# WangSimiao2000/MinecraftSkin_Raytracer

Hardware: NVIDIA B200
Metric: Mrays/s (higher is better)
Workload: dtype f32

## Files before the change

### include/mcskin_cuda.h

```cpp
#ifndef MCSKIN_CUDA_H
#define MCSKIN_CUDA_H

#include <stdint.h>

#ifdef __cplusplus
extern "C" {
#endif

#define MCSKIN_ABI_VERSION 2

enum {
    MC_OK = 0,
    MC_ERR_INVALID = -1,
    MC_ERR_NO_DEVICE = -2,
    MC_ERR_CUDA = -3,
    MC_ERR_LIMIT = -4
};

typedef struct McFaceTex {
    int32_t texel_offset;
    int32_t width;
    int32_t height;
} McFaceTex;

// ... 53 lines not shown
    x ^= x >> 16; x *= 0x7feb352du; x ^= x >> 15; x *= 0x846ca68bu; x ^= x >> 16;
    return x;
}
static inline uint32_t mc_rng_counter_key(uint32_t seed) { return mc_rng_lowbias32(seed ^ 0x9e3779b9u); }
static inline uint32_t mc_rng_counter_word(uint32_t seed, uint32_t k) { return mc_rng_lowbias32(mc_rng_counter_key(seed) + k); }
uint32_t mcskin_counter_word(uint32_t seed, uint32_t k);

void mcskin_config_defaults(McConfig* cfg);

typedef struct McTile {
    int32_t x, y, width, height;
} McTile;

int32_t mcskin_generate_tiles(int32_t image_width, int32_t image_height, int32_t tile_size,
                              McTile* out, int32_t capacity);

typedef void (*McProgressFn)(int32_t done, int32_t total, void* user);

typedef struct McRenderStats {
    int32_t n_tiles;
    int32_t n_active_pixels;
    int64_t n_samples;
    float ms_device;
    int32_t n_kernel_launches;
    float ms_primary;
    float ms_shade;
} McRenderStats;

int32_t mcskin_cuda_device_count(void);
const char* mcskin_cuda_last_error(void);
int32_t mcskin_cuda_abi_version(void);
void mcskin_cuda_abi_sizes(int32_t* out8);

int32_t mcskin_cuda_render(const McScene* scene, const McConfig* cfg, int32_t device,
                           float* out_rgba_f32, uint8_t* out_rgba_u8,
                           McProgressFn progress, void* user, McRenderStats* stats);

typedef struct McAovTargets {
    float* coverage;
    float* depth;
    int32_t* tri_id;
} McAovTargets;

int32_t mcskin_cuda_render_aovs(const McScene* scene, const McConfig* cfg, int32_t device,
                                float* out_rgba_f32, uint8_t* out_rgba_u8, const McAovTargets* aov,
                                McRenderStats* stats);

int32_t mcskin_cuda_render_tile(const McScene* scene, const McConfig* cfg, int32_t device,
                                const McTile* tile, float* image_rgba_f32, uint8_t* image_rgba_u8);

int32_t mcskin_cuda_render_multi(const McScene* scene, const McConfig* cfg, int32_t n_devices,
                                 float* out_rgba_f32, uint8_t* out_rgba_u8, McRenderStats* stats);

typedef struct McContext McContext;

int32_t mcskin_cuda_context_create(int32_t device, McContext** out);
void mcskin_cuda_context_destroy(McContext* ctx);
int32_t mcskin_cuda_context_set_scene(McContext* ctx, const McScene* scene, const McConfig* cfg);
int32_t mcskin_cuda_context_render_bands(McContext* ctx, int32_t first_tile_row, int32_t tile_row_stride,
                                         void* d_out_f32, void* d_out_u8, void* stream);
int32_t mcskin_cuda_band_rows(const McConfig* cfg, int32_t first_tile_row, int32_t tile_row_stride);
int32_t mcskin_cuda_context_render_rows_into_frame(McContext* ctx, int32_t first_tile_row, int32_t stride,
                                                    void* d_frame_f32, void* d_frame_u8, void* stream);
int32_t mcskin_cuda_context_render_tiles_into_frame(McContext* ctx, const int32_t* tiles, int32_t n_tiles,
                                                     void* d_frame_f32, void* d_frame_u8, void* stream);
int32_t mcskin_cuda_context_render_scene_tiles(McContext* ctx, const McScene* scene, const McConfig* cfg,
                                                const int32_t* tiles, int32_t n_tiles, float* host_frame_f32,
                                                uint8_t* host_frame_u8, float* ms_device);
int32_t mcskin_partition_tiles(const McScene* scene, const McConfig* cfg, int32_t n_parts, int32_t part,
                               int32_t root_part, int32_t* out_tiles, int32_t capacity);
int32_t mcskin_host_copy_rows(void* dst, const void* src, uint64_t dst_pitch, uint64_t src_pitch, uint64_t row_bytes,
                              uint64_t rows, int32_t pieces);
int32_t mcskin_cuda_host_register(void* host_ptr, uint64_t bytes, void** d_ptr);
int32_t mcskin_cuda_host_unregister(void* host_ptr);
int32_t mcskin_cuda_device_alloc(int32_t device, uint64_t bytes, void** out_ptr);
int32_t mcskin_cuda_device_free(int32_t device, void* ptr);
int32_t mcskin_cuda_ipc_export(int32_t device, void* ptr, uint8_t handle_out[64]);
int32_t mcskin_cuda_ipc_open(int32_t device, const uint8_t handle[64], void** out_ptr);
int32_t mcskin_cuda_ipc_close(int32_t device, void* ptr);
int32_t mcskin_cuda_peer_signal(int32_t device, void* d_flag, uint32_t value, void* stream);
int32_t mcskin_cuda_enable_peer_access(int32_t device, int32_t peer);
int32_t mcskin_cuda_peer_wait(int32_t device, const void* d_flags, int32_t n, uint32_t value, void* d_timeout, void* stream);
int32_t mcskin_cuda_context_debug_block_times(McContext* ctx, uint64_t* out, int32_t capacity);
int32_t mcskin_cuda_context_set_aov_targets(McContext* ctx, const McAovTargets* d_targets);
int32_t mcskin_cuda_context_sync(McContext* ctx, McRenderStats* stats);
int32_t mcskin_cuda_context_set_option(McContext* ctx, const char* name, int64_t value);

int32_t mcskin_cuda_context_render_batch(McContext* ctx, const McScene* scenes, int32_t n_scenes,
                                         const McConfig* cfg, void* d_out_f32, void* d_out_u8, void* stream);
int32_t mcskin_skin_layout(const uint8_t* atlas_rgba8, int32_t atlas_w, int32_t atlas_h, const float* pose12, McBox* boxes_out,
                           int32_t* faces_out, int32_t* n_faces_out, uint8_t* box_opaque_out, McScene* scene_out);
int32_t mcskin_cuda_context_render_skin_batch(McContext* ctx, const uint8_t* atlases_rgba8, int32_t atlas_w, int32_t atlas_h,
                                              int32_t n_skins, const float* poses12, int32_t pose_stride, const McConfig* cfg,
                                              void* d_out_f32, void* d_out_u8, void* stream);
int32_t mcskin_cuda_render_batch_multi(const McScene* scenes, int32_t n_scenes, const McConfig* cfg, int32_t n_devices,
                                       float* out_rgba_f32, uint8_t* out_rgba_u8);

typedef struct McRay {
    float origin[3];
    float dir[3];
} McRay;

typedef struct McHit {
    int32_t hit;
    float t;
    float point[3];
    float normal[3];
    float tex_color[4];
    int32_t is_outer_layer;
    int32_t box;
    int32_t face;
} McHit;

int32_t mcskin_cuda_intersect(const McScene* scene, int32_t device, int32_t box,
                              const McRay* rays, int32_t n, McHit* out);
int32_t mcskin_cuda_trace(const McScene* scene, const McConfig* cfg, int32_t device, int32_t use_config,
                          int32_t depth, const McRay* rays, int32_t n, float* out_rgba);
int32_t mcskin_cuda_shade(const McScene* scene, const McConfig* cfg, int32_t device,
                          const McHit* hits, const float* view_dirs , const float* shadow_factors ,
                          int32_t n, float* out_rgba);
int32_t mcskin_cuda_in_shadow(const McScene* scene, int32_t device, const float* points, const float* normals,
                              const float* light_positions, int32_t n, int32_t* out);
int32_t mcskin_cuda_soft_shadow(const McScene* scene, int32_t device, const float* points, const float* normals,
                                const uint32_t* seeds, int32_t samples, int32_t n, float* out);
int32_t mcskin_cuda_ambient_occlusion(const McScene* scene, int32_t device, const float* points,
                                      const float* normals, const uint32_t* seeds, int32_t samples,
                                      float radius, int32_t n, float* out);
int32_t mcskin_cuda_generate_rays(const McScene* scene, int32_t device, float aspect, const float* uv,
                                  int32_t n, McRay* out);
int32_t mcskin_cuda_background(const McScene* scene, const McConfig* cfg, int32_t device, int32_t use_config,
                               const float* uv, int32_t n, float* out_rgba);
int32_t mcskin_cuda_sincos(int32_t device, const float* angles, int32_t n, float* out_sin, float* out_cos);
void mcskin_sincos_model(const float* angles, int32_t n, float* out_sin, float* out_cos);
int32_t mcskin_cuda_powf(int32_t device, const float* x, const float* y, int32_t n, float* out);
void mcskin_powf_model(const float* x, const float* y, int32_t n, float* out);
int32_t mcskin_primary_launch_order(const McScene* scene, const McConfig* cfg, int32_t first_tile_row, int32_t stride,
                                    int32_t parts_heavy, int32_t parts_light, int32_t* out_tile, int32_t* out_part,
                                    int32_t* out_parts, int32_t capacity);
int32_t mcskin_cuda_fp32_issue_peak(int32_t device, double* out_lane_ops_per_second);
int32_t mcskin_cuda_aov(const McScene* scene, const McConfig* cfg, int32_t device, int32_t* out_tri_id);

#define MCSKIN_MAX_SKIN_BOXES 12
#define MCSKIN_MAX_SKIN_TEXELS 4096
int32_t mcskin_build_skin_scene(const uint8_t* atlas_rgba8, int32_t atlas_w, int32_t atlas_h,
                                const float* pose12, McBox* boxes_out, float* texels_out,
                                McScene* scene_out);

#ifdef __cplusplus
}
#endif
#endif
```

### minecraftskin_raytracer_b200/csrc/batch.cu

```cuda
#include <cstring>
#include <thread>
#include "capi_internal.hpp"

namespace {

struct SkinBatchSrc {
    const uint8_t* atlases;
    int w, h;
    const float* poses;
    int poseStride;
};

int render_batch_grouped(McContext* ctx, const McScene* scenes, const SkinBatchSrc* skins, int nScenes, const McConfig* cfg,
                         float4* outF32, uchar4* outU8, cudaStream_t stream, bool* handled) {
    *handled = false;
    if (!ctx->batchMode || ctx->shadeMode != 0 || ctx->forceAllActive || nScenes < 2) return MC_OK;
    if (cfg->width <= 0 || cfg->height <= 0 || cfg->tile_size <= 0 || cfg->width > 65535 || cfg->height > 65535) return MC_OK;
    const int spp = std::max(1, cfg->samples_per_pixel);
    if (spp > kBlockThreads) return MC_OK;
    const size_t pixels = static_cast<size_t>(cfg->width) * cfg->height;
    std::string err;
    for (int i = 0; i < 2; ++i)
        if (!ctx->evStage[i]) CU_TRY(cudaEventCreateWithFlags(&ctx->evStage[i], cudaEventDisableTiming));

// ... 123 lines not shown
                    groupOf[i] = static_cast<int>(g);
            }
            if (groupOf[i] < 0) {
                groupOf[i] = static_cast<int>(groups.size());
                groups.emplace_back();
            }
            groups[groupOf[i]].push_back(i);
        }
        unsigned char* stage = static_cast<unsigned char*>(ctx->batchStage[stageSlot].p);
        BatchSlice* stageSlices = reinterpret_cast<BatchSlice*>(stage + sliceOffset);
        AovView* stageAovs = reinterpret_cast<AovView*>(stage + aovOffset);
        int sliceAt = 0;
        std::vector<int> groupFirstSlice(groups.size(), 0);
        for (size_t g = 0; g < groups.size(); ++g) {
            groupFirstSlice[g] = sliceAt;
            for (int i : groups[g]) {
                const PreparedFrame& pf = ctx->batchPreps[i];
                unsigned char* dst = stage + static_cast<size_t>(i) * sceneStride;
                const size_t blobBytes = (pf.blob.size() + 255) & ~size_t(255);
                std::memcpy(dst, pf.blob.data(), pf.blob.size());
                if (!skins) std::memcpy(dst + blobBytes, pf.texels.data(), pf.texels.size() * sizeof(float4h));
                BatchSlice sl{};
                sl.fp.blob = devScenes + static_cast<size_t>(i) * sceneStride;
                sl.fp.texels = reinterpret_cast<const float4*>(devScenes + static_cast<size_t>(i) * sceneStride + blobBytes);
                sl.fp.blob_bytes = static_cast<unsigned int>(pf.blob.size());
                sl.band.first_tile_row = 0;
                sl.band.tile_row_stride = 1;
                sl.band.n_tile_rows = pf.frame.tiles_y;
                sl.band.out_first_row = 0;
                sl.band.out_row_stride = 1;
                sl.band.out_f32 = outF32 ? outF32 + static_cast<size_t>(c0 + i) * pixels : nullptr;
                sl.band.out_u8 = outU8 ? outU8 + static_cast<size_t>(c0 + i) * pixels : nullptr;
                AovView av{};
                av.planes = aov_at(ctx->aov, static_cast<size_t>(c0 + i) * pixels);
                sl.list.count = static_cast<unsigned int*>(ctx->batchCounts.p) + i;
                sl.list.slot_pixel = static_cast<uint2*>(ctx->batchSlots.p) + static_cast<size_t>(i) * slotCap;
                sl.list.records = reinterpret_cast<float*>(static_cast<unsigned char*>(ctx->batchRecords.p) + static_cast<size_t>(i) * recordBytes);
                sl.list.capacity = static_cast<unsigned int>(slotCap);
                sl.list.count_host = nullptr;
                const int gridX = std::max(2, (ctx->smCount * ctx->shadeBlocksPerSm + nC - 1) / nC);
                if (!wavefront_carve(pf.frame, static_cast<unsigned char*>(ctx->batchWave.p) + static_cast<size_t>(i) * waveBytes,
                                     waveBytes, static_cast<unsigned int>(paths), static_cast<unsigned int>(entries), gridX, &sl.wave, aov ? &av : nullptr))
                    return MC_OK;
                sl.wave.seedMemo = batchSeedMemo;
                stageAovs[sliceAt] = av;
                stageSlices[sliceAt++] = sl;
            }
        }
        const size_t usedScenes = static_cast<size_t>(nC) * sceneStride;
        if (skins) {
            const size_t blobMax = (SceneBlobLayout(kSkinMaxBoxes).bytes() + 255) & ~size_t(255);
            CU_TRY(cudaMemcpy2DAsync(devScenes, sceneStride, stage, sceneStride, blobMax, nC, cudaMemcpyHostToDevice, stream));
            CU_TRY(cudaMemcpyAsync(devSkin, skinStage, static_cast<size_t>(nC) * skinRecord, cudaMemcpyHostToDevice, stream));
            launch_slice_skins(devSkin, skinRecord, atlasBytes + kSkinMaxFaces * sizeof(SkinFaceSource), nC, stream);
        } else {
            CU_TRY(cudaMemcpyAsync(devScenes, stage, usedScenes, cudaMemcpyHostToDevice, stream));
        }
        CU_TRY(cudaMemcpyAsync(devScenes + sliceOffset, stage + sliceOffset, static_cast<size_t>(nC) * sizeof(BatchSlice),
                               cudaMemcpyHostToDevice, stream));
        if (aov)
            CU_TRY(cudaMemcpyAsync(devScenes + aovOffset, stage + aovOffset, static_cast<size_t>(nC) * sizeof(AovView),
                                   cudaMemcpyHostToDevice, stream));
        CU_TRY(cudaEventRecord(ctx->evStage[stageSlot], stream));
        stageSlot ^= 1;
        const BatchSlice* devSlices = reinterpret_cast<const BatchSlice*>(devScenes + sliceOffset);
        const AovView* devAovs = aov ? reinterpret_cast<const AovView*>(devScenes + aovOffset) : nullptr;
        for (size_t g = 0; g < groups.size(); ++g) {
            const int nS = static_cast<int>(groups[g].size());
            const BatchSlice* gs = devSlices + groupFirstSlice[g];
            const AovView* gAov = devAovs ? devAovs + groupFirstSlice[g] : nullptr;
            const BatchSlice& first = stageSlices[groupFirstSlice[g]];
            const DevFrame& f = ctx->batchPreps[groups[g][0]].frame;
            launch_batch_reset(gs, nS, stream);
            if (gAov) launch_aov_defaults(f, first.band, McAovTargets{}, gAov, nS, stream);
            const KernelBuild& build = kernels_for(f);
            const int primaryTarget = ctx->smCount * ctx->primaryBlocksPerSm;
            const int statesPerTile = primary_states_per_tile(f, f.tiles_x * f.tiles_y, nS, primaryTarget, 0);
            const bool seedNow = !seeded || statesPerTile != seededStatesPerTile;
            uint32_t* const states = static_cast<uint32_t*>(ctx->tileStates.p);
            if (!build.launch_primary_batch(f, first.band, states, seedNow, gs, nS, first.fp.blob_bytes, primaryTarget, stream)) return MC_OK;
            seeded = true;
            seededStatesPerTile = statesPerTile;
            int launches = 0;
            build.launch_wavefront(f, first.fp, first.band, first.list, first.wave, nullptr, stream, &launches, gs, nS, nullptr, gAov);
        }
        CU_TRY(cudaGetLastError());
    }
    *handled = true;
    return MC_OK;
}

}

extern "C" {

int32_t mcskin_cuda_context_render_batch(McContext* ctx, const McScene* scenes, int32_t nScenes, const McConfig* cfg,
                                         void* dOutF32, void* dOutU8, void* stream) {
    if (!ctx || !scenes || !cfg || nScenes < 0) return fail(MC_ERR_INVALID, "render_batch: bad argument");
    if (nScenes == 0) return MC_OK;
    CU_TRY(cudaSetDevice(ctx->device));
    const size_t pixels = static_cast<size_t>(std::max(cfg->width, 0)) * std::max(cfg->height, 0);
    cudaStream_t caller = stream ? static_cast<cudaStream_t>(stream) : ctx->stream;
    {
        bool handled = false;
        const int rc = render_batch_grouped(ctx, scenes, nullptr, nScenes, cfg, static_cast<float4*>(dOutF32), static_cast<uchar4*>(dOutU8),
                                            caller, &handled);
        if (rc != MC_OK) return rc;
        if (handled) {
            ctx->stats = McRenderStats{};
            ctx->statsPending = false;
            return MC_OK;
        }
    }
    const int nLanes = std::min<int>(ctx->batchLanes, nScenes);
    {
        const int rc = ensure_lanes(ctx, nLanes);
        if (rc != MC_OK) return rc;
    }
    CU_TRY(cudaEventRecord(ctx->evCopy, caller));
    for (int k = 0; k < nLanes; ++k) {
        McContext* lane = ctx->lanes[k];
        inherit_options(lane, ctx);
        lane->shadeBlocksPerSm = std::max(1, ctx->shadeBlocksPerSm / 2);
        CU_TRY(cudaStreamWaitEvent(lane->stream, ctx->evCopy, 0));
    }
    for (int i = 0; i < nScenes; ++i) {
        McContext* lane = ctx->lanes[i % nLanes];
        int rc = mcskin_cuda_context_set_scene(lane, &scenes[i], cfg);
        if (rc != MC_OK) return rc;
        lane->aov = aov_at(ctx->aov, static_cast<size_t>(i) * pixels);
        rc = render_bands(lane, 0, 1, dOutF32 ? static_cast<float4*>(dOutF32) + i * pixels : nullptr,
                          dOutU8 ? static_cast<uchar4*>(dOutU8) + i * pixels : nullptr, lane->stream);
        if (rc != MC_OK) return rc;
    }
    for (int k = 0; k < nLanes; ++k) {
        CU_TRY(cudaEventRecord(ctx->lanes[k]->evCopy, ctx->lanes[k]->stream));
        CU_TRY(cudaStreamWaitEvent(caller, ctx->lanes[k]->evCopy, 0));
    }
    ctx->stats = McRenderStats{};
    ctx->statsPending = false;
    return MC_OK;
}

int32_t mcskin_cuda_context_render_skin_batch(McContext* ctx, const uint8_t* atlases, int32_t atlasW, int32_t atlasH,
                                              int32_t nSkins, const float* poses12, int32_t poseStride, const McConfig* cfg,
                                              void* dOutF32, void* dOutU8, void* stream) {
    if (!ctx || !atlases || !cfg || nSkins < 0 || poseStride < 0) return fail(MC_ERR_INVALID, "render_skin_batch: bad argument");
    if (!((atlasW == 64 && atlasH == 64) || (atlasW == 64 && atlasH == 32)))
        return fail(MC_ERR_INVALID, "Invalid skin dimensions: " + std::to_string(atlasW) + "x" + std::to_string(atlasH) +
                                        " (expected 64x64 or 64x32)");
    if (nSkins == 0) return MC_OK;
    CU_TRY(cudaSetDevice(ctx->device));
    cudaStream_t caller = stream ? static_cast<cudaStream_t>(stream) : ctx->stream;
    const SkinBatchSrc src{atlases, atlasW, atlasH, poses12, poses12 ? poseStride : 0};
    bool handled = false;
    int rc = render_batch_grouped(ctx, nullptr, &src, nSkins, cfg, static_cast<float4*>(dOutF32), static_cast<uchar4*>(dOutU8),
                                  caller, &handled);
    if (rc != MC_OK) return rc;
    if (handled) {
        ctx->stats = McRenderStats{};
        ctx->statsPending = false;
        return MC_OK;
    }
    const size_t atlasBytes = static_cast<size_t>(atlasW) * atlasH * 4;
    const int chunk = 64;
    std::vector<McBox> boxes(static_cast<size_t>(chunk) * kSkinMaxBoxes);
    std::vector<float> texels(static_cast<size_t>(chunk) * (kSkinMaxTexels + 16) * 4);
// ... 99 lines not shown
```

### minecraftskin_raytracer_b200/csrc/capi.cu

```cuda
#include <cstring>
#include "capi_internal.hpp"

namespace {

struct Staged {
    McContext* ctx;
    std::vector<void*> temps;
    ~Staged() {
        for (void* p : temps) cudaFree(p);
    }
    int up(const void* host, size_t bytes, void** dev) {
        *dev = nullptr;
        if (bytes == 0) return MC_OK;
        CU_TRY(cudaMalloc(dev, bytes));
        temps.push_back(*dev);
        if (host) CU_TRY(cudaMemcpyAsync(*dev, host, bytes, cudaMemcpyHostToDevice, ctx->stream));
        return MC_OK;
    }
    int down(void* host, const void* dev, size_t bytes) {
        if (bytes == 0) return MC_OK;
        CU_TRY(cudaMemcpyAsync(host, dev, bytes, cudaMemcpyDeviceToHost, ctx->stream));
        CU_TRY(cudaStreamSynchronize(ctx->stream));
        CU_TRY(cudaGetLastError());
        return MC_OK;
// ... 251 lines not shown
    if (rc != MC_OK) return rc;
    Staged st{ctx, {}};
    void *dU, *dO;
    if ((rc = st.up(uv, sizeof(float) * 2 * n, &dU)) != MC_OK) return rc;
    if ((rc = st.up(nullptr, sizeof(float4) * n, &dO)) != MC_OK) return rc;
    launch_background(ctx->prep.frame, static_cast<float*>(dU), n, static_cast<float4*>(dO), ctx->stream);
    return st.down(out, dO, sizeof(float4) * n);
}

int32_t mcskin_primary_launch_order(const McScene* scene, const McConfig* cfg, int32_t first, int32_t stride,
                                    int32_t partsHeavy, int32_t partsLight, int32_t* outTile, int32_t* outPart,
                                    int32_t* outParts, int32_t capacity) {
    if (!scene || !cfg || capacity < 0) return fail(MC_ERR_INVALID, "primary_launch_order: bad argument");
    PreparedFrame pf;
    std::string err;
    const int rc = prepare_frame(scene, cfg, 1, 0.0f, pf, err);
    if (rc != MC_OK) return fail(rc, err);
    return primary_launch_order(pf.frame, first, stride, partsHeavy, partsLight, outTile, outPart, outParts, capacity);
}

int32_t mcskin_cuda_fp32_issue_peak(int32_t device, double* out) {
    if (!out) return fail(MC_ERR_INVALID, "fp32_issue_peak: out is null");
    *out = 0.0;
    std::lock_guard<std::mutex> lock(g_ctxMutex);
    McContext* ctx = nullptr;
    int rc = shared_context(device, &ctx);
    if (rc != MC_OK) return rc;
    float* sink = nullptr;
    CU_TRY(cudaMalloc(&sink, sizeof(float)));
    const int blocks = ctx->smCount * 8, iters = 1 << 15;
    cudaEvent_t e0, e1;
    CU_TRY(cudaEventCreate(&e0));
    CU_TRY(cudaEventCreate(&e1));
    double best = 0.0;
    for (int rep = 0; rep < 6; ++rep) {
        CU_TRY(cudaEventRecord(e0, ctx->stream));
        launch_fp32_peak(blocks, iters, sink, ctx->stream);
        CU_TRY(cudaEventRecord(e1, ctx->stream));
        CU_TRY(cudaEventSynchronize(e1));
        float ms = 0.0f;
        CU_TRY(cudaEventElapsedTime(&ms, e0, e1));
        const double ops = static_cast<double>(blocks) * kBlockThreads * iters * 16.0;
        if (ms > 0.0f) best = std::max(best, ops / (ms * 1e-3));
    }
    cudaEventDestroy(e0);
    cudaEventDestroy(e1);
    cudaFree(sink);
    CU_TRY(cudaGetLastError());
    *out = best;
    return MC_OK;
}

int32_t mcskin_cuda_powf(int32_t device, const float* x, const float* y, int32_t n, float* out) {
    if (n < 0 || (n > 0 && (!x || !y || !out))) return fail(MC_ERR_INVALID, "powf: bad argument");
    std::lock_guard<std::mutex> lock(g_ctxMutex);
    McContext* ctx = nullptr;
    int rc = shared_context(device, &ctx);
    if (rc != MC_OK) return rc;
    Staged st{ctx, {}};
    void *dX, *dY, *dO;
    if ((rc = st.up(x, sizeof(float) * n, &dX)) != MC_OK) return rc;
    if ((rc = st.up(y, sizeof(float) * n, &dY)) != MC_OK) return rc;
    if ((rc = st.up(nullptr, sizeof(float) * n, &dO)) != MC_OK) return rc;
    launch_powf(static_cast<float*>(dX), static_cast<float*>(dY), n, static_cast<float*>(dO), ctx->stream);
    return st.down(out, dO, sizeof(float) * n);
}

int32_t mcskin_cuda_sincos(int32_t device, const float* angles, int32_t n, float* outSin, float* outCos) {
    if (n < 0 || (n > 0 && (!angles || !outSin || !outCos))) return fail(MC_ERR_INVALID, "sincos: bad argument");
    std::lock_guard<std::mutex> lock(g_ctxMutex);
    McContext* ctx = nullptr;
    int rc = shared_context(device, &ctx);
    if (rc != MC_OK) return rc;
    Staged st{ctx, {}};
    void *dA, *dS, *dC;
    if ((rc = st.up(angles, sizeof(float) * n, &dA)) != MC_OK) return rc;
    if ((rc = st.up(nullptr, sizeof(float) * n, &dS)) != MC_OK) return rc;
    if ((rc = st.up(nullptr, sizeof(float) * n, &dC)) != MC_OK) return rc;
    launch_sincos(static_cast<float*>(dA), n, static_cast<float*>(dS), static_cast<float*>(dC), ctx->stream);
    if ((rc = st.down(outSin, dS, sizeof(float) * n)) != MC_OK) return rc;
    return st.down(outCos, dC, sizeof(float) * n);
}

int32_t mcskin_cuda_aov(const McScene* scene, const McConfig* cfg, int32_t device, int32_t* outTriId) {
    if (!cfg || !outTriId) return fail(MC_ERR_INVALID, "aov: bad argument");
    if (cfg->width <= 0 || cfg->height <= 0) return MC_OK;
    std::lock_guard<std::mutex> lock(g_ctxMutex);
    McContext* ctx = nullptr;
    int rc = query_setup(scene, cfg, device, 1, 0.0f, &ctx);
    if (rc != MC_OK) return rc;
    Staged st{ctx, {}};
    void* dO;
    const size_t bytes = sizeof(int32_t) * static_cast<size_t>(cfg->width) * cfg->height;
    if ((rc = st.up(nullptr, bytes, &dO)) != MC_OK) return rc;
    launch_aov(ctx->prep.frame, frame_pointers(ctx), static_cast<int*>(dO), ctx->stream);
    return st.down(outTriId, dO, bytes);
}

void mcskin_cuda_abi_sizes(int32_t* out8) {
    if (!out8) return;
    out8[0] = sizeof(McFaceTex);
    out8[1] = sizeof(McBox);
    out8[2] = sizeof(McScene);
    out8[3] = sizeof(McConfig);
    out8[4] = sizeof(McTile);
    out8[5] = sizeof(McRenderStats);
    out8[6] = sizeof(McRay);
    out8[7] = sizeof(McHit);
}

}
```

### minecraftskin_raytracer_b200/csrc/capi_internal.hpp

```cpp
#pragma once
#include <algorithm>
#include <atomic>
#include <cstdlib>
#include <cstring>
#include <memory>
#include <mutex>
#include <string>
#include <thread>
#include <vector>

#include <cuda_runtime.h>

#include "host_copy.hpp"
#include "host_prep.hpp"
#include "kernels.cuh"
#include "wavefront.cuh"
#include "mcskin_cuda.h"

using namespace mcskin;

inline int fail(int code, const std::string& msg) {
    set_last_error(msg);
    return code;
}
inline int cuda_fail(cudaError_t e, const char* what) {
    return fail(e == cudaErrorNoDevice || e == cudaErrorInsufficientDriver ? MC_ERR_NO_DEVICE : MC_ERR_CUDA,
                std::string(what) + ": " + cudaGetErrorString(e));
}
#define CU_TRY(expr)                                     \
    do {                                                 \
        cudaError_t e__ = (expr);                        \
        if (e__ != cudaSuccess) return cuda_fail(e__, #expr); \
    } while (0)

extern std::atomic<unsigned long long> g_allocEpoch;

template <bool kPinned>
struct GrowBuf {
    void* p = nullptr;
    size_t cap = 0;
    GrowBuf() = default;
    GrowBuf(const GrowBuf&) = delete;
    GrowBuf& operator=(const GrowBuf&) = delete;
    ~GrowBuf() { release(); }
    cudaError_t reserve(size_t bytes) {
        if (bytes <= cap) return cudaSuccess;
        if (!kPinned) g_allocEpoch.fetch_add(1);
        release();
        cudaError_t e = kPinned ? cudaMallocHost(&p, bytes) : cudaMalloc(&p, bytes);
        if (e == cudaSuccess) cap = bytes;
        return e;
    }
    void release() {
        if (p) (kPinned ? cudaFreeHost : cudaFree)(p);
        p = nullptr;
        cap = 0;
    }
};
using DevBuf = GrowBuf<false>;
using PinnedBuf = GrowBuf<true>;

struct PixelRect {
    int x, y, w, h;
};

struct McOptions {
    int forceAllActive = 0;
    long long recordBudgetBytes = 1ll << 31;
    int shadeBlocksPerSm = 8;
    int softBlocksPerSm = 4;
    int heavyTilesPerSm = 16;
    int primaryBlocksPerSm = 8;
    int waveQueuePct = 0;
    int frameLanes = 2;
    int cacheTileSeeds = 1;
    int overlapCopyOut = 2;
    int useGraphs = 1;
    int shadeMode = 0;
    long long waveBudgetBytes = 12ll << 30;
    int shadowSeedMemo = 1;
    int stagedCopyOut = 1;
    int batchLanes = 4;
    int batchGroup = 128;
    int batchMode = 1;
    int debugPrimaryTiming = 0;
};
constexpr size_t kOptionCount = 19;

struct McContext : McOptions {
    int device = 0;
    int smCount = 148;
    cudaStream_t stream = nullptr;
    cudaEvent_t ev0 = nullptr, ev1 = nullptr, evCopy = nullptr;
    std::vector<cudaEvent_t> passEvents;
    bool hasScene = false;
    PreparedFrame prep;
    DevBuf boxes, texels;
    DevBuf slotPixel, records;
    DevBuf imgF32, imgU8;
    DevBuf tileStates;
    DevBuf blockTimes;
    int blockTimesCount = 0;
    DevBuf tileMap;
    std::vector<int32_t> tileMapHost, tileMapOrdered;
    std::vector<PixelRect> tileMapLightRects;
    unsigned long long tileMapVersion = 0;
    int tileMapHeavy = 0;
    DevFrame tileMapFrame{};
    DevBuf wave;
    PinnedBuf pinned;
    bool isChild = false;
    struct TileSeedKey {
        int width = 0, tile_size = 0, first = 0, stride = 0, rows = 0;
        const void* buf = nullptr;
        cudaStream_t stream = nullptr;
        const void* map = nullptr;
        unsigned long long mapVersion = 0;
        int wordsPerPixel = 0, statesPerTile = 0;
        bool operator==(const TileSeedKey& o) const {
            return width == o.width && tile_size == o.tile_size && first == o.first && stride == o.stride &&
                   rows == o.rows && buf == o.buf && stream == o.stream && map == o.map && mapVersion == o.mapVersion &&
                   wordsPerPixel == o.wordsPerPixel && statesPerTile == o.statesPerTile;
        }
    } tileSeedKey;
    bool tileSeedValid = false;
    int splitLastRender = 0;
    cudaEvent_t evPrimaryDone = nullptr;
    cudaStream_t copyStream = nullptr;
    cudaEvent_t evFrameDone = nullptr;
    cudaEvent_t evUpload = nullptr;
    unsigned long long seedGen = 0;
    bool capturing = false;
    struct GraphKey {
        DevFrame frame;
        const void *blob, *texels, *outF32, *outU8;
        unsigned int blobBytes;
        int first, stride, lanes;
        const void* tileMap;
        unsigned long long mapVersion;
        int nTiles, nHeavy;
        const void *hotF32, *hotU8;
        const void *aovCoverage, *aovDepth, *aovTriId;
        long long optionBits[kOptionCount];
        unsigned long long allocEpoch;
        bool operator==(const GraphKey& o) const { return std::memcmp(this, &o, sizeof(GraphKey)) == 0; }
    };
    GraphKey graphKey{}, graphCandidate{};
    bool hasCandidate = false;
    cudaGraph_t graph = nullptr;
    cudaGraphExec_t graphExec = nullptr;
    std::vector<unsigned long long> graphSeedGens;
    std::vector<int> graphLaneLaunches, graphLaneChunks, graphLaneTiles;
    bool graphLastRender = false;
    McRenderStats stats{};
    bool statsPending = false;
    bool uploadQueued = false;
    DevBuf countLog;
    PinnedBuf countHost;
    unsigned int* countAlias = nullptr;
    PinnedBuf sceneStage;
    DevBuf seedMemo;
    PinnedBuf stageF32, stageU8;
    std::vector<cudaEvent_t> pieceEvents;
    std::vector<std::pair<const void*, bool>> farCache;
    int chunksLastRender = 0;
    DevBuf batchScenes, batchSlots, batchRecords, batchWave, batchCounts;
    DevBuf batchSkinSrc;
    PinnedBuf batchSkinStage[2];
    std::vector<McBox> batchSkinBoxes;
    PinnedBuf batchStage[2];
    cudaEvent_t evStage[2] = {nullptr, nullptr};
    std::vector<PreparedFrame> batchPreps;
    std::vector<McContext*> lanes;
    McAovTargets aov{};
    DevBuf aovPlanes;
};

struct KernelBuild {
    decltype(&mcskin::launch_primary) launch_primary;
    decltype(&mcskin::launch_shade) launch_shade;
    decltype(&mcskin::launch_wavefront) launch_wavefront;
    decltype(&mcskin::launch_primary_batch) launch_primary_batch;
};
constexpr KernelBuild kGeneralBuild{&launch_primary, &launch_shade, &launch_wavefront, &launch_primary_batch};
constexpr KernelBuild kPlainBuild{&plain::launch_primary, &plain::launch_shade, &plain::launch_wavefront, &plain::launch_primary_batch};
// ... 50 lines not shown
```

### minecraftskin_raytracer_b200/csrc/context.cu

```cuda
#include <cstdlib>
#include "capi_internal.hpp"

std::atomic<unsigned long long> g_allocEpoch{1};

namespace {

using IntOption = int McOptions::*;
using LongOption = long long McOptions::*;
struct OptionSpec {
    const char* name;
    const char* env;
    IntOption i;
    LongOption ll;
    long long lo, hi;
    bool inherited, launch;
};
constexpr OptionSpec kOptions[] = {
    {"force_all_active", "MCSKIN_FORCE_ALL_ACTIVE", &McOptions::forceAllActive, nullptr, 0, 1, true, true},
    {"record_budget_bytes", nullptr, nullptr, &McOptions::recordBudgetBytes, 1, INT64_MAX, true, true},
    {"shade_blocks_per_sm", "MCSKIN_SHADE_BLOCKS", &McOptions::shadeBlocksPerSm, nullptr, 1, INT32_MAX, true, true},
    {"soft_blocks_per_sm", "MCSKIN_SOFT_BLOCKS", &McOptions::softBlocksPerSm, nullptr, 1, INT32_MAX, true, true},
    {"primary_blocks_per_sm", "MCSKIN_PRIMARY_BLOCKS", &McOptions::primaryBlocksPerSm, nullptr, 0, INT32_MAX, true, true},
    {"heavy_tiles_per_sm", "MCSKIN_HEAVY_TILES", &McOptions::heavyTilesPerSm, nullptr, 0, INT32_MAX, true, true},
    {"batch_lanes", nullptr, &McOptions::batchLanes, nullptr, 1, 16, false, false},
    {"batch_group", "MCSKIN_BATCH_GROUP", &McOptions::batchGroup, nullptr, 1, 4096, false, false},
    {"batch_mode", "MCSKIN_BATCH_MODE", &McOptions::batchMode, nullptr, 0, 1, false, false},
    {"shade_mode", "MCSKIN_SHADE_MODE", &McOptions::shadeMode, nullptr, 0, 2, true, true},
    {"debug_primary_timing", nullptr, &McOptions::debugPrimaryTiming, nullptr, 0, 1, false, true},
    {"wave_queue_pct", "MCSKIN_WAVE_QUEUE_PCT", &McOptions::waveQueuePct, nullptr, 0, 100000, true, true},
    {"frame_lanes", "MCSKIN_FRAME_LANES", &McOptions::frameLanes, nullptr, 1, 8, false, true},
    {"cache_tile_seeds", "MCSKIN_CACHE_TILE_SEEDS", &McOptions::cacheTileSeeds, nullptr, 0, 1, true, true},
    {"use_graphs", "MCSKIN_GRAPHS", &McOptions::useGraphs, nullptr, 0, 1, false, false},
    {"overlap_copy_out", "MCSKIN_OVERLAP_COPY", &McOptions::overlapCopyOut, nullptr, 0, 2, false, false},
    {"wave_budget_bytes", nullptr, nullptr, &McOptions::waveBudgetBytes, 1 << 20, INT64_MAX, true, true},
    {"staged_copy_out", "MCSKIN_STAGED_COPY", &McOptions::stagedCopyOut, nullptr, 0, 1, false, false},
    {"shadow_seed_memo", "MCSKIN_SEED_MEMO", &McOptions::shadowSeedMemo, nullptr, 0, 1, false, true},
};
static_assert(sizeof(kOptions) / sizeof(kOptions[0]) == kOptionCount, "kOptionCount counts the rows of kOptions");

long long option_value(const McOptions& o, const OptionSpec& spec) { return spec.i ? o.*spec.i : o.*spec.ll; }

void set_option_value(McOptions& o, const OptionSpec& spec, long long value) {
    const long long v = spec.lo == 0 && spec.hi == 1 ? value != 0 : std::min(spec.hi, std::max(spec.lo, value));
    if (spec.i) o.*spec.i = static_cast<int>(v);
    else o.*spec.ll = v;
}

}

void inherit_options(McContext* lane, const McContext* ctx) {
    for (const OptionSpec& spec : kOptions)
        if (spec.inherited) set_option_value(*lane, spec, option_value(*ctx, spec));
    lane->aov = ctx->aov;
    lane->useGraphs = 0;
}

void launch_option_bits(const McContext* ctx, long long* bits) {
    for (size_t i = 0; i < kOptionCount; ++i) bits[i] = kOptions[i].launch ? option_value(*ctx, kOptions[i]) : 0;
}

int upload_scene(McContext* ctx) {
    const PreparedFrame& pf = ctx->prep;
    if (pf.blob.size() > kMaxSceneSmemBytes)
        return fail(MC_ERR_LIMIT, "scene has too many meshes for the shared-memory staging area (" +
                                      std::to_string(pf.boxes.size()) + " boxes)");
    CU_TRY(ctx->boxes.reserve(pf.blob.size()));
    CU_TRY(ctx->texels.reserve(pf.texels.size() * sizeof(float4h)));
    const size_t blobBytes = (pf.blob.size() + 255) & ~size_t(255), texelBytes = pf.texels.size() * sizeof(float4h);
    if (ctx->uploadQueued) CU_TRY(cudaEventSynchronize(ctx->evUpload));
    CU_TRY(ctx->sceneStage.reserve(blobBytes + texelBytes + 256));
    unsigned char* stage = static_cast<unsigned char*>(ctx->sceneStage.p);
    std::memcpy(stage, pf.blob.data(), pf.blob.size());
    if (texelBytes) std::memcpy(stage + blobBytes, pf.texels.data(), texelBytes);
    CU_TRY(cudaMemcpyAsync(ctx->boxes.p, stage, pf.blob.size(), cudaMemcpyHostToDevice, ctx->stream));
    if (texelBytes) CU_TRY(cudaMemcpyAsync(ctx->texels.p, stage + blobBytes, texelBytes, cudaMemcpyHostToDevice, ctx->stream));
    CU_TRY(cudaEventRecord(ctx->evUpload, ctx->stream));
    ctx->uploadQueued = true;
    return MC_OK;
}

int finish_stats(McContext* ctx, McRenderStats* out) {
    if (ctx->statsPending) {
        float ms = 0.0f;
        if (!(ctx->isChild && ctx->graphLastRender)) {
            CU_TRY(cudaEventSynchronize(ctx->ev1));
            CU_TRY(cudaEventElapsedTime(&ms, ctx->ev0, ctx->ev1));
        }
        ctx->stats.ms_device = ms;
        ctx->stats.ms_primary = ctx->stats.ms_shade = 0.0f;
        for (int c = 0; c < ctx->chunksLastRender && !ctx->graphLastRender; ++c) {
            float a = 0.0f, b = 0.0f;
            CU_TRY(cudaEventElapsedTime(&a, ctx->passEvents[3 * c], ctx->passEvents[3 * c + 1]));
            CU_TRY(cudaEventElapsedTime(&b, ctx->passEvents[3 * c + 1], ctx->passEvents[3 * c + 2]));
            ctx->stats.ms_primary += a;
            ctx->stats.ms_shade += b;
        }
        long long active = 0;
        const unsigned int* counts = static_cast<const unsigned int*>(ctx->countHost.p);
        for (int c = 0; c < ctx->chunksLastRender && counts; ++c) active += counts[c];
        ctx->stats.n_active_pixels = static_cast<int32_t>(std::min<long long>(active, 0x7fffffff));
        ctx->statsPending = false;
        for (int k = 0; k < ctx->splitLastRender; ++k) {
            McRenderStats s{};
            const int rc = finish_stats(ctx->lanes[k], &s);
            if (rc != MC_OK) return rc;
            ctx->stats.n_tiles += s.n_tiles;
            ctx->stats.n_active_pixels += s.n_active_pixels;
            ctx->stats.n_kernel_launches += s.n_kernel_launches;
            ctx->stats.ms_primary = std::max(ctx->stats.ms_primary, s.ms_primary);
            ctx->stats.ms_shade = std::max(ctx->stats.ms_shade, s.ms_shade);
        }
    }
    if (out) *out = ctx->stats;
    return MC_OK;
}

std::mutex g_ctxMutex;
std::vector<McContext*> g_ctxByDevice;

// ... 116 lines not shown
```

### minecraftskin_raytracer_b200/csrc/dev_intersect.cuh

```cuda
#pragma once
#include "dev_math.cuh"
#include "dev_types.cuh"

namespace mcskin {

struct Ray {
    V3 o, d;
};

struct Hit {
    float t;
    V3 p;
    int box;
    int face;
    int texel;
    bool flip;
};

struct SceneView {
    const float4* __restrict__ lo;
    const float4* __restrict__ hi;
    const int4* __restrict__ rect;
    const DevBox* __restrict__ boxes;
    const float4* __restrict__ texels;
// ... 73 lines not shown
}
__device__ __forceinline__ int face_texel(const DevBox& bx, V3 p, int axis, bool negSide, int face) {
    const float pa = (axis == 0) ? p.z : p.x;
    const float la0 = (axis == 0) ? bx.lo[2] : bx.lo[0];
    const float sa = (axis == 0) ? bx.size[2] : bx.size[0];
    const float ra = (axis == 0) ? bx.inv_size_z : bx.inv_size_x;
    const float pb = (axis == 1) ? p.z : p.y;
    const float lb0 = (axis == 1) ? bx.lo[2] : bx.lo[1];
    const float sb = (axis == 1) ? bx.size[2] : bx.size[1];
    const float rb = (axis == 1) ? bx.inv_size_z : bx.inv_size_y;
    float la, lb;
    if (bx.flags & kBoxRecip) {
        la = div_exact(pa - la0, sa, ra);
        lb = div_exact(pb - lb0, sb, rb);
    } else {
        la = (pa - la0) / sa;
        lb = (pb - lb0) / sb;
    }
    float u, v;
    if (axis == 2) {
        u = negSide ? 1.0f - la : la;
        v = 1.0f - lb;
    } else if (axis == 0) {
        u = !negSide ? 1.0f - la : la;
        v = 1.0f - lb;
    } else {
        u = la;
        v = !negSide ? lb : 1.0f - lb;
    }
    u = clamp01(u);
    v = clamp01(v);
    const int2 ft = bx.face[face];
    const int w = ft.y & 0xffff;
    const int h = ft.y >> 16;
    int x = __float2int_rz(u * static_cast<float>(w));
    int y = __float2int_rz(v * static_cast<float>(h));
    x = max(0, min(x, w - 1));
    y = max(0, min(y, h - 1));
    return ft.x + y * w + x;
}

struct RayPre {
    V3 inv;
    bool parallel;
};
__device__ __forceinline__ RayPre ray_pre(const Ray& r) {
    RayPre p;
    p.parallel = fabsf(r.d.x) < 1e-8f || fabsf(r.d.y) < 1e-8f || fabsf(r.d.z) < 1e-8f;
    p.inv = mk3(1.0f / r.d.x, 1.0f / r.d.y, 1.0f / r.d.z);
    return p;
}

struct BoxHit {
    float t;
    V3 p;
    int face, texel;
    bool flip;
};

__device__ __forceinline__ float rcp_fast(float x) {
    float r;
    asm("rcp.approx.ftz.f32 %0, %1;" : "=f"(r) : "f"(x));
    return r;
}

__device__ __forceinline__ V3 to_box_space(const DevBox& bx, V3 p, bool isPoint) {
    const V3 pivot = isPoint ? ld3(bx.pivot) : mk3(0.0f, 0.0f, 0.0f);
    V3 q = p - pivot;
    if (bx.flags & kBoxRotZ) {
        const float nx = q.x * bx.inv_cz - q.y * bx.inv_sz, ny = q.x * bx.inv_sz + q.y * bx.inv_cz;
        q.x = nx;
        q.y = ny;
    }
    if (bx.flags & kBoxRotX) {
        const float ny = q.y * bx.inv_cx - q.z * bx.inv_sx, nz = q.y * bx.inv_sx + q.z * bx.inv_cx;
        q.y = ny;
        q.z = nz;
    }
    return q + pivot;
}

enum : int { kPosedUnknown = 0, kPosedMissed = 1, kPosedHitBeforeLimit = 2 };
template <bool LIMITED>
__device__ __forceinline__ int posed_box_verdict(const DevBox& bx, const Ray& ray, float limit, bool opaque) {
    constexpr float kPad = 1e-2f;
    const V3 o = to_box_space(bx, ray.o, true);
    const V3 d = to_box_space(bx, ray.d, false);
    float tmin = -FLT_MAX, tmax = FLT_MAX;
    float smin = -FLT_MAX, smax = FLT_MAX;
    bool sure = LIMITED && opaque;
    const float os[3] = {o.x, o.y, o.z}, ds[3] = {d.x, d.y, d.z};
#pragma unroll
    for (int k = 0; k < 3; ++k) {
        const float lo = bx.lo[k] - kPad, hi = bx.hi[k] + kPad;
        if (fabsf(ds[k]) < 1e-6f) {
            if (os[k] < lo || os[k] > hi) return kPosedMissed;
            sure = sure && os[k] > lo + 2.0f * kPad && os[k] < hi - 2.0f * kPad;
            continue;
        }
        const float inv = rcp_fast(ds[k]);
        const float a = (lo - os[k]) * inv, b = (hi - os[k]) * inv;
        tmin = fmaxf(tmin, fminf(a, b));
        tmax = fminf(tmax, fmaxf(a, b));
        if (LIMITED) {
            const float shift = 2.0f * kPad * fabsf(inv);
            smin = fmaxf(smin, fminf(a, b) + shift);
            smax = fminf(smax, fmaxf(a, b) - shift);
        }
    }
    const float slack = 1e-4f * (fabsf(tmin) + fabsf(tmax)) + 1e-3f;
    if (fmaxf(tmin, 0.0f) > tmax + slack) return kPosedMissed;
    if (LIMITED && !(tmin - slack < limit)) return kPosedMissed;
    if (LIMITED && sure && fmaxf(smin, 0.0f) + slack < smax && tmax + slack < limit) return kPosedHitBeforeLimit;
    return kPosedUnknown;
}
template <bool LIMITED>
__device__ __forceinline__ bool posed_box_missed(const DevBox& bx, const Ray& ray, float limit) {
    return posed_box_verdict<LIMITED>(bx, ray, limit, false) == kPosedMissed;
}

template <bool LIMITED>
__device__ __forceinline__ uint32_t drop_missed_posed(const SceneView& sc, const Ray& ray, uint32_t mask, float limit) {
    if (!kPosedScenes) return mask;
    uint32_t todo = mask & sc.rotated_mask;
    while (todo) {
        const int i = __ffs(todo) - 1;
        todo &= todo - 1u;
        if (posed_box_missed<LIMITED>(sc.boxes[i], ray, limit)) mask &= ~(1u << i);
    }
    return mask;
}


__device__ __forceinline__ bool box_test(const SceneView& sc, const DevBox& bx, V3 o, V3 d, V3 inv, BoxHit& out) {
    Slab s;
    s.tmin = -FLT_MAX;
    s.tmax = FLT_MAX;
    s.axis = 0;
    s.exitAxis = 0;
    s.neg = false;
    s.exitNeg = false;
    if (!slab_axis<0>(s, o.x, d.x, inv.x, bx.lo[0], bx.hi[0])) return false;
    if (!slab_axis<1>(s, o.y, d.y, inv.y, bx.lo[1], bx.hi[1])) return false;
    if (!slab_axis<2>(s, o.z, d.z, inv.z, bx.lo[2], bx.hi[2])) return false;
    if (s.tmin > s.tmax || s.tmax < 0.0f) return false;

    float tHit = s.tmin;
    int axis = s.axis;
    bool negSide = s.neg;
    if (tHit < 0.0f) {
        tHit = s.tmax;
        axis = s.exitAxis;
        negSide = s.exitNeg;
    }
    bool flip = false;
    for (;;) {
        const V3 p = o + d * tHit;
        const int face = face_index(axis, negSide);
        const int texel = face_texel(bx, p, axis, negSide, face);
        const float alpha = __ldg(&sc.texels[texel].w);
        const bool opaque = flip ? (alpha > 0.0f) : !(alpha == 0.0f);
        if (opaque) {
            out.t = tHit;
            out.p = p;
            out.face = face;
            out.texel = texel;
            out.flip = flip;
            return true;
// ... 177 lines not shown
    best.p = mk3(0.0f, 0.0f, 0.0f);
    BoxHit h;
    const RayPre pre = ray_pre(ray);
    if (b >= 0 && b < sc.n_boxes && mesh_test(sc, b, ray, pre, h)) {
        best.t = h.t;
        best.p = h.p;
        best.box = b;
        best.face = h.face;
        best.texel = h.texel;
        best.flip = h.flip;
    }
    return best;
}

__device__ __forceinline__ bool any_hit(const SceneView& sc, const Ray& ray) {
    const RayPre pre = ray_pre(ray);
    for (int base = 0; base < sc.n_boxes; base += 32) {
        uint32_t mask = candidate_mask<false>(sc, ray, pre, base, FLT_MAX);
        while (mask) {
            const int b = base + __ffs(mask) - 1;
            mask &= mask - 1u;
            BoxHit h;
            if (mesh_test(sc, b, ray, pre, h)) return true;
        }
    }
    return false;
}

__device__ __forceinline__ bool occluded_among(const SceneView& sc, const Ray& ray, const float dist, const uint32_t allow) {
    const RayPre pre = ray_pre(ray);
    for (int base = 0; base < sc.n_boxes; base += 32) {
        uint32_t mask;
        if (base == 0 && allow != 0xffffffffu) {
            uint32_t todo = allow & sc.usable_mask;
            if (sc.n_boxes < 32) todo &= (1u << sc.n_boxes) - 1u;
            mask = todo;
            if (!pre.parallel) {
                uint32_t rejected = 0u;
                while (todo) {
                    const int i = __ffs(todo) - 1;
                    todo &= todo - 1u;
                    const float4 L = sc.lo[i];
                    const float4 H = sc.hi[i];
                    const float ax = (L.x - ray.o.x) * pre.inv.x, bx = (H.x - ray.o.x) * pre.inv.x;
                    const float ay = (L.y - ray.o.y) * pre.inv.y, by = (H.y - ray.o.y) * pre.inv.y;
                    const float az = (L.z - ray.o.z) * pre.inv.z, bz = (H.z - ray.o.z) * pre.inv.z;
                    const float tmin = fmaxf(fmaxf(fminf(ax, bx), fminf(ay, by)), fminf(az, bz));
                    const float tmax = fminf(fminf(fmaxf(ax, bx), fmaxf(ay, by)), fmaxf(az, bz));
                    if (fmaxf(tmin, 0.0f) > tmax || !(tmin < dist)) {
                        rejected |= 1u << i;
                    } else if ((sc.opaque_mask >> i) & 1u) {
                        if ((tmin < 0.0f ? tmax : tmin) < dist) return true;
                        rejected |= 1u << i;
                    }
                }
                mask &= ~rejected | sc.posed_mask;
                if (kPosedScenes) {
                    uint32_t posedTodo = mask & sc.rotated_mask;
                    while (posedTodo) {
                        const int i = __ffs(posedTodo) - 1;
                        posedTodo &= posedTodo - 1u;
                        const int verdict = posed_box_verdict<true>(sc.boxes[i], ray, dist, (sc.opaque_posed_mask >> i) & 1u);
                        if (verdict == kPosedHitBeforeLimit) return true;
                        if (verdict == kPosedMissed) mask &= ~(1u << i);
                    }
                }
            }
        } else {
            mask = candidate_mask<true>(sc, ray, pre, base, dist);
        }
        while (mask) {
            const int b = base + __ffs(mask) - 1;
            mask &= mask - 1u;
            BoxHit h;
            if (mesh_test(sc, b, ray, pre, h) && h.t < dist) return true;
        }
    }
    return false;
}
__device__ __forceinline__ bool occluded(const SceneView& sc, const Ray& ray, float dist) {
    return occluded_among(sc, ray, dist, 0xffffffffu);
}

__device__ __forceinline__ bool bundle_clip(V3 a, V3 d, V3 inv, V3 lo, V3 hi, float grow, float* sEnd) {
    const float ax0 = (lo.x - grow - a.x) * inv.x, ax1 = (hi.x + grow - a.x) * inv.x;
    const float ay0 = (lo.y - grow - a.y) * inv.y, ay1 = (hi.y + grow - a.y) * inv.y;
    const float az0 = (lo.z - grow - a.z) * inv.z, az1 = (hi.z + grow - a.z) * inv.z;
    const bool px = fabsf(d.x) < 1e-6f, py = fabsf(d.y) < 1e-6f, pz = fabsf(d.z) < 1e-6f;
    const bool outX = px && (a.x < lo.x - grow || a.x > hi.x + grow);
    const bool outY = py && (a.y < lo.y - grow || a.y > hi.y + grow);
    const bool outZ = pz && (a.z < lo.z - grow || a.z > hi.z + grow);
    float s0 = 0.0f, s1 = 1.0f;
    if (!px) { s0 = fmaxf(s0, fminf(ax0, ax1)); s1 = fminf(s1, fmaxf(ax0, ax1)); }
    if (!py) { s0 = fmaxf(s0, fminf(ay0, ay1)); s1 = fminf(s1, fmaxf(ay0, ay1)); }
    if (!pz) { s0 = fmaxf(s0, fminf(az0, az1)); s1 = fminf(s1, fmaxf(az0, az1)); }
    *sEnd = s1;
    return !(outX || outY || outZ) && s0 <= s1 + 1e-3f;
}

__device__ __forceinline__ bool bundle_reaches(V3 from, V3 d, V3 lo, V3 hi, float radius, float pad) {
    const float growFull = radius * 1.01f + 0.01f + pad;
    const V3 inv = mk3(rcp_fast(d.x), rcp_fast(d.y), rcp_fast(d.z));
    if (fabsf(d.x) < 1e-6f || fabsf(d.y) < 1e-6f || fabsf(d.z) < 1e-6f) {
        float sEnd;
        if (!bundle_clip(from, d, inv, lo, hi, growFull, &sEnd)) return false;
        const float reach = fminf(fmaxf(sEnd + 1e-3f, 0.0f), 1.0f);
        float unused;
        return bundle_clip(from, d, inv, lo, hi, reach * radius * 1.01f + 0.01f + pad, &unused);
    }
    if ((from.x > hi.x + pad && d.x > growFull) || (from.x < lo.x - pad && d.x < -growFull) ||
        (from.y > hi.y + pad && d.y > growFull) || (from.y < lo.y - pad && d.y < -growFull) ||
        (from.z > hi.z + pad && d.z > growFull) || (from.z < lo.z - pad && d.z < -growFull))
        return false;
    const V3 ainv = mk3(fabsf(inv.x), fabsf(inv.y), fabsf(inv.z));
    const V3 g1 = ainv * growFull;
    const float ax = (lo.x - from.x) * inv.x, bx = (hi.x - from.x) * inv.x;
    const float ay = (lo.y - from.y) * inv.y, by = (hi.y - from.y) * inv.y;
    const float az = (lo.z - from.z) * inv.z, bz = (hi.z - from.z) * inv.z;
    const float nx = fminf(ax, bx), fx = fmaxf(ax, bx);
    const float ny = fminf(ay, by), fy = fmaxf(ay, by);
    const float nz = fminf(az, bz), fz = fmaxf(az, bz);
    const float s0 = fmaxf(fmaxf(nx - g1.x, ny - g1.y), fmaxf(nz - g1.z, 0.0f));
    const float s1 = fminf(fminf(fx + g1.x, fy + g1.y), fminf(fz + g1.z, 1.0f));
    if (!(s0 <= s1 + 1e-3f)) return false;
    const float reach = fminf(fmaxf(s1 + 1e-3f, 0.0f), 1.0f);
    const V3 g2 = ainv * (reach * radius * 1.01f + 0.01f + pad);
    const float t0 = fmaxf(fmaxf(nx - g2.x, ny - g2.y), fmaxf(nz - g2.z, 0.0f));
    const float t1 = fminf(fminf(fx + g2.x, fy + g2.y), fminf(fz + g2.z, 1.0f));
    return t0 <= t1 + 1e-3f;
}

__device__ __forceinline__ bool posed_bundle_reaches(const DevBox& pb, V3 from, V3 d, float radius) {
    return bundle_reaches(to_box_space(pb, from, true), to_box_space(pb, d, false), ld3(pb.lo), ld3(pb.hi), radius, 1e-4f);
}

__device__ __forceinline__ uint32_t drop_unreached_posed(const SceneView& sc, V3 from, V3 d, float radius, uint32_t mask) {
    if (!kPosedScenes) return mask;
    uint32_t todo = mask & sc.rotated_mask;
    while (todo) {
        const int i = __ffs(todo) - 1;
        todo &= todo - 1u;
        if (!posed_bundle_reaches(sc.boxes[i], from, d, radius)) mask &= ~(1u << i);
    }
    return mask;
}


__device__ __forceinline__ uint32_t bundle_box_mask(const SceneView& sc, V3 from, V3 to, float radius) {
    const int n = min(32, sc.n_boxes);
    const V3 d = to - from;
    const V3 inv = mk3(rcp_fast(d.x), rcp_fast(d.y), rcp_fast(d.z));
    const float growFull = radius * 1.01f + 0.01f;
    uint32_t mask = 0u;
    if (fabsf(d.x) < 1e-6f || fabsf(d.y) < 1e-6f || fabsf(d.z) < 1e-6f) {
        for (int i = 0; i < n; ++i) {
            const float4 L = sc.lo[i];
            const float4 H = sc.hi[i];
            if (__float_as_uint(L.w) & kBoxEmpty) continue;
            const V3 lo = mk3(L.x, L.y, L.z), hi = mk3(H.x, H.y, H.z);
            float sEnd;
            if (!bundle_clip(from, d, inv, lo, hi, growFull, &sEnd)) continue;
            const float reach = fminf(fmaxf(sEnd + 1e-3f, 0.0f), 1.0f);
            float unused;
            if (!bundle_clip(from, d, inv, lo, hi, reach * radius * 1.01f + 0.01f, &unused)) continue;
            mask |= 1u << i;
        }
// ... 85 lines not shown
```

### minecraftskin_raytracer_b200/csrc/dev_shade.cuh

```cuda
#pragma once
#include "dev_intersect.cuh"
#include "dev_mt19937.cuh"

namespace mcskin {

constexpr float kShadowEpsilon = 1e-3f;
constexpr float kReflectEpsilon = 1e-3f;
constexpr float kReflectivity = 0.1f;
constexpr int kMaxStackDepth = 64;
#define MCSKIN_TWO_PI_F (2.0f * 3.14159274101257324219f)

__device__ __forceinline__ Ray camera_ray(const DevFrame& fr, float u, float v) {
    const float su = (2.0f * u - 1.0f) * fr.half_w;
    const float sv = (2.0f * (1.0f - v) - 1.0f) * fr.half_h;
    const V3 fwd = ld3(fr.cam_fwd), right = ld3(fr.cam_right), up = ld3(fr.cam_up);
    Ray r;
    r.o = ld3(fr.cam_pos);
    r.d = normalize3((fwd + right * su) + up * sv);
    return r;
}

__device__ __forceinline__ void sincos_ref(float a, float* sn, float* cs) {
    const uint32_t top12 = (__float_as_uint(a) >> 20) & 0x7ffu;
    if (top12 > 0x42eu) {
// ... 171 lines not shown
}

static __device__ __noinline__ float soft_shadow_large(const SceneView& sc, const DevFrame& fr, V3 point, V3 normal,
                                                int samples, uint32_t seed) {
    if (samples <= 1 || fr.light_radius < 1e-4f) return in_shadow(sc, point, normal, ld3(fr.light_pos)) ? 0.0f : 1.0f;
    LocalEngine rng;
    rng.seed(seed);
    return static_cast<float>(soft_shadow_count(sc, fr, point, normal, samples, rng, 0xffffffffu)) / static_cast<float>(samples);
}
__device__ __forceinline__ float soft_shadow(const SceneView& sc, const DevFrame& fr, V3 point, V3 normal,
                                             int samples, uint32_t seed) {
    if (samples <= 1 || fr.light_radius < 1e-4f || 2 * samples > kFreshStreamMaxDraws)
        return soft_shadow_large(sc, fr, point, normal, samples, seed);
    const uint32_t allow = bundle_box_mask(sc, point + normal * kShadowEpsilon, ld3(fr.light_pos), fr.light_radius);
    if (allow == 0u && sc.n_boxes <= 32) return 1.0f;
    FreshStream rng;
    rng.seed(seed);
    return static_cast<float>(soft_shadow_count(sc, fr, point, normal, samples, rng, allow)) / static_cast<float>(samples);
}

template <class Engine>
__device__ __forceinline__ int ao_count(const SceneView& sc, V3 point, V3 normal, int samples, float radius,
                                        Engine& rng) {
    const V3 N = normalize3(normal);
    V3 T, B;
    frame_about(N, &T, &B);
    Ray r;
    r.o = point + N * 1e-3f;
    int occludedCount = 0;
    for (int i = 0; i < samples; ++i) {
        const float r1 = rng.next();
        const float r2 = rng.next();
        const float sinT = sqrtf(1.0f - r1);
        const float cosT = sqrtf(r1);
        const float phi = MCSKIN_TWO_PI_F * r2;
        float sn, cs;
        sincos_ref(phi, &sn, &cs);
        const V3 l = mk3(sinT * cs, cosT, sinT * sn);
        r.d = normalize3((T * l.x + N * l.y) + B * l.z);
        if (occluded(sc, r, radius)) ++occludedCount;
    }
    return occludedCount;
}
static __device__ __noinline__ float ambient_occlusion_large(const SceneView& sc, V3 point, V3 normal, int samples,
                                                      float radius, uint32_t seed) {
    LocalEngine rng;
    rng.seed(seed);
    return 1.0f - static_cast<float>(ao_count(sc, point, normal, samples, radius, rng)) / static_cast<float>(samples);
}
static __device__ __noinline__ float ambient_occlusion(const SceneView& sc, V3 point, V3 normal, int samples,
                                                   float radius, uint32_t seed) {
    if (2 * samples > kFreshStreamMaxDraws) return ambient_occlusion_large(sc, point, normal, samples, radius, seed);
    FreshStream rng;
    rng.seed(seed);
    return 1.0f - static_cast<float>(ao_count(sc, point, normal, samples, radius, rng)) / static_cast<float>(samples);
}

__device__ __forceinline__ float4 shade_lit(const DevFrame& fr, V3 P, V3 normal, float4 tex, V3 viewDir, float vis) {
    const V3 lp = ld3(fr.light_pos);
    const V3 L = normalize3(lp - P);
    const V3 N = normalize3(normal);
    const V3 V = normalize3(viewDir);
    const float ndl = fmaxf(0.0f, dot3(N, L));
    const float kdiff = fr.kd * ndl * vis;
    const V3 H = normalize3(L + V);
    const float ndh = fmaxf(0.0f, dot3(N, H));
    const float spec = powf_ref(ndh, fr.shininess);
    const float kspec = fr.ks * spec * vis;
    float4 out;
    out.x = (tex.x * fr.ambient + tex.x * fr.light_color[0] * kdiff) + fr.light_color[0] * kspec;
    out.y = (tex.y * fr.ambient + tex.y * fr.light_color[1] * kdiff) + fr.light_color[1] * kspec;
    out.z = (tex.z * fr.ambient + tex.z * fr.light_color[2] * kdiff) + fr.light_color[2] * kspec;
    out.w = tex.w;
    return clamp4(out);
}

__device__ __forceinline__ float4 shade_hit(const SceneView& sc, const DevFrame& fr, V3 P, V3 normal, float4 tex,
                                            V3 viewDir, float shadowFactor) {
    float vis = shadowFactor;
    if (vis < 0.0f) vis = in_shadow(sc, P, normalize3(normal), ld3(fr.light_pos)) ? 0.0f : 1.0f;
    return shade_lit(fr, P, normal, tex, viewDir, vis);
}

template <class Engine>
__device__ __forceinline__ void soft_shadow_positions(const DevFrame& fr, V3 point, int samples, Engine& rng,
                                                      float* out ) {
    const V3 lp = ld3(fr.light_pos);
    const V3 toPoint = normalize3(point - lp);
    V3 tangent, bitangent;
    frame_about(toPoint, &tangent, &bitangent);
    for (int i = 0; i < samples; ++i) {
        const float angle = MCSKIN_TWO_PI_F * rng.next();
        const float r = fr.light_radius * sqrtf(rng.next());
        float sn, cs;
        sincos_ref(angle, &sn, &cs);
        const V3 offset = tangent * (r * cs) + bitangent * (r * sn);
        const V3 samplePos = lp + offset;
        out[3 * i] = samplePos.x;
        out[3 * i + 1] = samplePos.y;
        out[3 * i + 2] = samplePos.z;
    }
}

__device__ __forceinline__ uint32_t shadow_seed(V3 P, int depth) {
    return seed_cast(P.x * 12345.0f + P.y * 67890.0f + P.z * 11111.0f + static_cast<float>(depth) * 99999.0f);
}
__device__ __forceinline__ uint32_t ao_seed(V3 P) {
    return seed_cast(P.x * 73856093.0f + P.y * 19349663.0f + P.z * 83492791.0f);
}

struct TraceOptions {
    int start_depth;
    bool primary_uv;
    float u, v;
};

__device__ __forceinline__ float4 trace_path(const SceneView& sc, const DevFrame& fr, Ray ray,
                                             const TraceOptions& opt) {
    const bool cfg = fr.use_config != 0;
    const int maxB = fr.max_bounces;
    int depth = opt.start_depth;

    if (depth > maxB) {
        float4 c = cfg ? config_background(fr, 0.5f, 0.5f) : flat_background(fr);
        if (opt.primary_uv && closest_hit(sc, ray).box < 0) c = config_background(fr, opt.u, opt.v);
        return c;
    }

    float stack[kMaxStackDepth][3];
    float alpha0 = 1.0f;
    int top = 0;
    float4 tail;
    for (;;) {
        const Hit hit = closest_hit(sc, ray);
        if (hit.box < 0) {
            if (depth == 0 && opt.primary_uv) tail = config_background(fr, opt.u, opt.v);
            else if (depth == 0 && cfg) tail = config_background(fr, 0.5f, 0.5f);
            else tail = flat_background(fr);
            break;
        }
        const V3 P = hit.p;
        const V3 nrm = hit_normal(sc, hit);
        const float4 tex = hit_texel(sc, hit);
        const V3 viewDir = normalize3(ray.o - P);
        float shadowFactor = -1.0f;
        if (cfg && fr.soft_on) {
            const uint32_t seed = shadow_seed(P, depth);
            shadowFactor = soft_shadow(sc, fr, P, nrm, fr.shadow_samples, seed);
        }
        float4 shaded = shade_hit(sc, fr, P, nrm, tex, viewDir, shadowFactor);
        const float alpha = shaded.w;
        if (cfg && fr.ao_on && depth == 0) {
            const uint32_t seed = ao_seed(P);
            const float ao = ambient_occlusion(sc, P, nrm, fr.ao_samples, fr.ao_radius, seed);
            const float f = 1.0f - fr.ao_intensity * (1.0f - ao);
            shaded.x *= f;
            shaded.y *= f;
            shaded.z *= f;
        }
        if (depth < maxB && top < kMaxStackDepth) {
            stack[top][0] = shaded.x;
            stack[top][1] = shaded.y;
            stack[top][2] = shaded.z;
            if (top == 0) alpha0 = alpha;
            ++top;
            const V3 N = normalize3(nrm);
            const V3 D = normalize3(ray.d);
            V3 R = D - N * (2.0f * dot3(D, N));
            R = normalize3(R);
            ray.o = P + N * kReflectEpsilon;
            ray.d = R;
            ++depth;
            continue;
        }
        shaded.w = alpha;
        tail = clamp4(shaded);
        break;
    }
    const float keep = 1.0f - kReflectivity;
    while (top > 0) {
        --top;
        float4 c;
        c.x = stack[top][0] * keep + tail.x * kReflectivity;
        c.y = stack[top][1] * keep + tail.y * kReflectivity;
// ... 9 lines not shown
```

### minecraftskin_raytracer_b200/csrc/frame.cu

```cuda
#include <cstring>
#include "capi_internal.hpp"

FramePointers frame_pointers(const McContext* ctx) {
    return FramePointers{static_cast<const unsigned char*>(ctx->boxes.p), static_cast<const float4*>(ctx->texels.p),
                         static_cast<unsigned int>(ctx->prep.blob.size())};
}

namespace {

int local_tile_rows(const DevFrame& f, int first, int stride) {
    if (f.tiles_y <= 0 || first < 0 || stride <= 0 || first >= f.tiles_y) return 0;
    return (f.tiles_y - first + stride - 1) / stride;
}

int band_pixel_rows(const DevFrame& f, int first, int stride) {
    const int n = local_tile_rows(f, first, stride);
    if (n == 0) return 0;
    const int lastTileRow = first + (n - 1) * stride;
    const int lastHeight = std::min(f.tile_size, f.height - lastTileRow * f.tile_size);
    return (n - 1) * f.tile_size + lastHeight;
}

}

// ... 81 lines not shown
        paths = std::max<size_t>(paths, static_cast<size_t>(f.spp));
        size_t entries = paths * hitsMax;
        if (ctx.waveQueuePct > 0) entries = std::min(entries, std::max<size_t>(32, paths * static_cast<size_t>(ctx.waveQueuePct) / 100));
        const size_t room = budget > paths * perPath ? (budget - paths * perPath) / perEntry : 0;
        entries = std::min(entries, std::max(room, paths + paths / 4));
        entries = std::min<size_t>(entries, 0xffffff00u);
        p.wavePaths = paths;
        p.waveEntries = entries;
        p.waveBytes = paths * perPath + entries * perEntry + wavefront_fixed_bytes(f) + 16 * 256;
    }
    return p;
}

int render_bands_lane(McContext* ctx, const McContext* scn, const BandSpec& spec, float4* outF32, uchar4* outU8,
                      cudaStream_t stream, int lanesInFlight = 1) {
    const DevFrame& f = scn->prep.frame;
    const long long nTilesAll = band_tiles(f, spec);
    ctx->chunksLastRender = 0;
    ctx->graphLastRender = false;
    ctx->stats = McRenderStats{};
    ctx->stats.n_samples = static_cast<int64_t>(std::max(f.width, 0)) * std::max(f.height, 0) * f.spp;
    ctx->stats.n_tiles = nTilesAll;
    if (nTilesAll == 0) return MC_OK;
    if (f.width > 65535 || f.height > 65535) return fail(MC_ERR_LIMIT, "image larger than 65535 pixels on a side");
    if (static_cast<long long>(f.tile_size) * f.tile_size > (1ll << 30))
        return fail(MC_ERR_LIMIT, "tile_size too large");
    const BandPlan plan = plan_band(f, spec, *ctx, lanesInFlight);
    if (plan.slotCap > 0x7fffffffull) return fail(MC_ERR_LIMIT, "one tile row holds more than 2^31 pixels");
    const int nChunks = plan.nChunks;

    CU_TRY(ctx->countLog.reserve(sizeof(unsigned int) * 2 * nChunks));
    if (ctx->countHost.cap < sizeof(unsigned int) * nChunks) {
        g_allocEpoch.fetch_add(1);
        CU_TRY(ctx->countHost.reserve(sizeof(unsigned int) * std::max(1024, 2 * nChunks)));
        void* alias = nullptr;
        if (cudaHostGetDevicePointer(&alias, ctx->countHost.p, 0) != cudaSuccess) {
            cudaGetLastError();
            alias = nullptr;
        }
        ctx->countAlias = static_cast<unsigned int*>(alias);
    }
    unsigned int* const countAlias = ctx->countAlias;
    CU_TRY(ctx->slotPixel.reserve(plan.slotCap * sizeof(uint2)));
    CU_TRY(ctx->records.reserve(std::max<size_t>(16, plan.slotCap * plan.recordBytesPerSlot)));
    CU_TRY(ctx->tileStates.reserve(
        std::max<size_t>(16, plan.unitsPerChunk * plan.tilesPerUnit * plan.statesPerTile * 624 * sizeof(uint32_t))));
    CU_TRY(cudaMemsetAsync(ctx->countLog.p, 0, sizeof(unsigned int) * 2 * nChunks, stream));

    while (ctx->passEvents.size() < static_cast<size_t>(3 * nChunks)) {
        cudaEvent_t e;
        CU_TRY(cudaEventCreate(&e));
        ctx->passEvents.push_back(e);
    }
    WaveView wave{};
    const bool aov = aov_on(ctx);
    AovView aovView{};
    aovView.planes = ctx->aov;
    if (ctx->shadeMode == 0) {
        CU_TRY(ctx->wave.reserve(plan.waveBytes));
        if (!wavefront_carve(f, ctx->wave.p, ctx->wave.cap, static_cast<unsigned int>(plan.wavePaths),
                             static_cast<unsigned int>(plan.waveEntries), ctx->smCount * ctx->shadeBlocksPerSm, &wave,
                             aov ? &aovView : nullptr))
            return fail(MC_ERR_CUDA, "wavefront buffer carve failed");
        wave.softGrid = ctx->smCount * ctx->softBlocksPerSm;
        wave.seedMemo = static_cast<uint2*>(scn->seedMemo.p);
        if (!scn->shadowSeedMemo) wave.seedMemo = nullptr;
    }
    if (!ctx->capturing) CU_TRY(cudaEventRecord(ctx->ev0, stream));
    const FramePointers fp = frame_pointers(scn);
    const KernelBuild& build = kernels_for(f);
    const bool mapped = spec.map != nullptr, classify = plan.classify;
    int launches = 0;
    McContext::TileSeedKey seedKey;
    seedKey.width = f.width; seedKey.tile_size = f.tile_size; seedKey.first = spec.first; seedKey.stride = spec.stride;
    seedKey.rows = static_cast<int>(plan.nUnits); seedKey.buf = ctx->tileStates.p; seedKey.stream = stream;
    seedKey.map = spec.map; seedKey.mapVersion = spec.mapVersion;
    seedKey.wordsPerPixel = f.spp * f.draws_per_sample; seedKey.statesPerTile = static_cast<int>(plan.statesPerTile) | (f.rng_mode << 16);
    const bool seedsCacheable = ctx->cacheTileSeeds && nChunks == 1 && f.draws_per_sample > 0;
    const bool seedTiles = !(seedsCacheable && ctx->tileSeedValid && seedKey == ctx->tileSeedKey);
    ctx->tileSeedKey = seedKey;
    ctx->tileSeedValid = false;
    if (seedTiles) ++ctx->seedGen;
    const bool farOutput = spec.hotF32 || spec.hotU8 || is_far_memory(ctx, outF32) || is_far_memory(ctx, outU8);
    for (int c = 0; c < nChunks; ++c) {
        const size_t unit0 = static_cast<size_t>(c) * plan.unitsPerChunk;
        const size_t units = std::min<size_t>(plan.unitsPerChunk, plan.nUnits - unit0);
        BandView band{};
        band.out_f32 = outF32;
        band.out_u8 = outU8;
        band.hot_f32 = spec.hotF32;
        band.hot_u8 = spec.hotU8;
        band.far_output = farOutput ? 1 : 0;
        if (ctx->debugPrimaryTiming && nChunks == 1) {
            const size_t tilePixels = static_cast<size_t>(f.tile_size) * f.tile_size;
            const size_t blocks = static_cast<size_t>(nTilesAll) * ((tilePixels + kBlockThreads - 1) / kBlockThreads);
            CU_TRY(ctx->blockTimes.reserve(blocks * 4 * sizeof(unsigned long long)));
            CU_TRY(cudaMemsetAsync(ctx->blockTimes.p, 0, blocks * 4 * sizeof(unsigned long long), stream));
            band.block_times = static_cast<unsigned long long*>(ctx->blockTimes.p);
            ctx->blockTimesCount = static_cast<int>(blocks);
        }
        size_t listing = units;
        if (mapped) {
            band.tile_map = spec.map + unit0;
            band.n_tiles = static_cast<int>(units);
            band.n_heavy = static_cast<int>(unit0 >= static_cast<size_t>(spec.nHeavy) ? 0 : std::min<size_t>(units, spec.nHeavy - unit0));
            if (classify && f.rect_valid) listing = static_cast<size_t>(band.n_heavy);
        } else {
            band.first_tile_row = spec.first + static_cast<int>(unit0) * spec.stride;
            band.tile_row_stride = spec.stride;
            band.n_tile_rows = static_cast<int>(units);
            band.out_first_row = spec.outFirst + static_cast<int>(unit0) * spec.outStride;
            band.out_row_stride = spec.outStride;
        }
        ActiveList list;
        list.count = static_cast<unsigned int*>(ctx->countLog.p) + c;
        list.slot_pixel = static_cast<uint2*>(ctx->slotPixel.p);
        list.records = static_cast<float*>(ctx->records.p);
        list.capacity = static_cast<unsigned int>(std::min(plan.slotCap, std::max<size_t>(1, listing * plan.slotsPerUnit)));
        list.count_host = (ctx->shadeMode == 0 && countAlias) ? countAlias + c : nullptr;
        if (!classify) {
            CU_TRY(cudaMemsetAsync(list.slot_pixel, 0xff, static_cast<size_t>(list.capacity) * sizeof(uint2), stream));
            CU_TRY(cudaMemcpyAsync(list.count, &list.capacity, sizeof(unsigned int), cudaMemcpyHostToDevice, stream));
        }
        if (!ctx->capturing) CU_TRY(cudaEventRecord(ctx->passEvents[3 * c], stream));
        if (aov) {
            launch_aov_defaults(f, band, ctx->aov, nullptr, 1, stream);
            ++launches;
        }
        const bool seeded = build.launch_primary(f, fp, band, list, classify ? 1 : 0, static_cast<uint32_t*>(ctx->tileStates.p),
                                                 seedTiles, plan.primaryTarget, plan.heavyTarget, stream);
        ctx->tileSeedValid = seedsCacheable && seeded;
        if (c == nChunks - 1)
            CU_TRY(cudaEventRecordWithFlags(ctx->evPrimaryDone, stream, ctx->capturing ? cudaEventRecordExternal : cudaEventRecordDefault));
        if (!ctx->capturing) CU_TRY(cudaEventRecord(ctx->passEvents[3 * c + 1], stream));
        unsigned int* groupCounter = static_cast<unsigned int*>(ctx->countLog.p) + nChunks + c;
        const int shadeGrid = ctx->smCount * ctx->shadeBlocksPerSm;
        if (ctx->shadeMode == 0)
            build.launch_wavefront(f, fp, band, list, wave, groupCounter, stream, &launches, nullptr, 1, aov ? &aovView : nullptr, nullptr);
        else
            launches += build.launch_shade(f, fp, band, list, shadeGrid, groupCounter, 0u, stream, ctx->shadeMode, &ctx->aov);
        if (!ctx->capturing) CU_TRY(cudaEventRecord(ctx->passEvents[3 * c + 2], stream));
        ++launches;
    }
    if (!(ctx->shadeMode == 0 && countAlias))
        CU_TRY(cudaMemcpyAsync(ctx->countHost.p, ctx->countLog.p, sizeof(unsigned int) * nChunks, cudaMemcpyDeviceToHost, stream));
    if (!ctx->capturing) CU_TRY(cudaEventRecord(ctx->ev1, stream));
    CU_TRY(cudaGetLastError());
    ctx->chunksLastRender = nChunks;
    ctx->stats.n_kernel_launches = launches;
    ctx->statsPending = true;
    return MC_OK;
}

}

int ensure_lanes(McContext* ctx, int n) {
    while (static_cast<int>(ctx->lanes.size()) < n) {
        McContext* lane = nullptr;
        const int rc = mcskin_cuda_context_create(ctx->device, &lane);
        if (rc != MC_OK) return rc;
        lane->isChild = true;
        ctx->lanes.push_back(lane);
    }
    return MC_OK;
}

namespace {

int launch_frame_lanes(McContext* ctx, int first, int stride, int L, float4* outF32, uchar4* outU8, cudaStream_t stream,
                       bool frameLayout, const BandSpec* tiles, float4* hotF32, uchar4* hotU8) {
    if (tiles) {
        BandSpec t = *tiles;
        t.hotF32 = hotF32; t.hotU8 = hotU8;
        return render_bands_lane(ctx, ctx, t, outF32, outU8, stream);
    }
    auto rows = [&](int f0, int st, int out0, int outSt) {
        BandSpec b;
        b.first = f0; b.stride = st; b.outFirst = out0; b.outStride = outSt;
        b.hotF32 = hotF32; b.hotU8 = hotU8;
        return b;
    };
    if (L <= 1)
        return render_bands_lane(ctx, ctx, rows(first, stride, frameLayout ? first : 0, frameLayout ? stride : 1), outF32, outU8, stream);
    CU_TRY(cudaEventRecord(ctx->evCopy, stream));
    int rc = render_bands_lane(ctx, ctx, rows(first, stride * L, frameLayout ? first : 0, frameLayout ? stride * L : L), outF32, outU8, stream, L);
    if (rc != MC_OK) return rc;
    for (int k = 1; k < L; ++k) {
        McContext* lane = ctx->lanes[k - 1];
        CU_TRY(cudaStreamWaitEvent(lane->stream, ctx->evCopy, 0));
        rc = render_bands_lane(lane, ctx, rows(first + k * stride, stride * L, frameLayout ? first + k * stride : k,
                                               frameLayout ? stride * L : L), outF32, outU8, lane->stream, L);
        if (rc != MC_OK) return rc;
        CU_TRY(cudaEventRecord(lane->evCopy, lane->stream));
    }
    for (int k = 1; k < L; ++k) CU_TRY(cudaStreamWaitEvent(stream, ctx->lanes[k - 1]->evCopy, 0));
    return MC_OK;
}

void drop_graph(McContext* ctx) {
    if (ctx->graphExec) cudaGraphExecDestroy(ctx->graphExec);
    if (ctx->graph) cudaGraphDestroy(ctx->graph);
    ctx->graphExec = nullptr;
    ctx->graph = nullptr;
}

}

int render_bands(McContext* ctx, int first, int stride, float4* outF32, uchar4* outU8, cudaStream_t stream,
                 bool frameLayout, const BandSpec* tiles, float4* hotF32, uchar4* hotU8) {
    const DevFrame& f = ctx->prep.frame;
    const int nRows = tiles ? (tiles->nTiles > 0 ? 1 : 0) : local_tile_rows(f, first, stride);
    const int L = (ctx->isChild || tiles) ? 1 : std::max(1, std::min(ctx->frameLanes, nRows / 2));
    ctx->splitLastRender = 0;
    ctx->graphLastRender = false;
    if (!ctx->isChild && f.soft_on) seed_memo_of(ctx);
    if (stream != ctx->stream && ctx->evUpload) CU_TRY(cudaStreamWaitEvent(stream, ctx->evUpload, 0));
    if (L > 1) {
        const int rc = ensure_lanes(ctx, L - 1);
        if (rc != MC_OK) return rc;
        for (int k = 1; k < L; ++k) inherit_options(ctx->lanes[k - 1], ctx);
    }
// ... 143 lines not shown
            const int x = tx * f.tile_size, y = ty * f.tile_size;
            const int w = std::min(f.tile_size, f.width - x), h = std::min(f.tile_size, f.height - y);
            const bool canHit = !f.rect_valid || !(x > f.rect_x1 || x + w - 1 < f.rect_x0 || y > f.rect_y1 || y + h - 1 < f.rect_y0);
            (canHit ? heavy : light).push_back(id);
        }
        ctx->tileMapHost.assign(tiles, tiles + nTiles);
        ctx->tileMapHeavy = static_cast<int>(heavy.size());
        ctx->tileMapOrdered = heavy;
        ctx->tileMapOrdered.insert(ctx->tileMapOrdered.end(), light.begin(), light.end());
        ctx->tileMapLightRects = tile_rects(f, light);
        ctx->tileMapFrame = f;
        if (nTiles > 0) {
            CU_TRY(ctx->tileMap.reserve(sizeof(int32_t) * static_cast<size_t>(nTiles)));
            CU_TRY(cudaMemcpyAsync(ctx->tileMap.p, ctx->tileMapOrdered.data(), sizeof(int32_t) * nTiles, cudaMemcpyHostToDevice, s));
        }
        ++ctx->tileMapVersion;
    }
    *empty = nTiles == 0;
    if (nTiles == 0) {
        ctx->stats = McRenderStats{};
        ctx->statsPending = false;
        return MC_OK;
    }
    spec->map = static_cast<const int*>(ctx->tileMap.p);
    spec->nTiles = nTiles;
    spec->nHeavy = ctx->tileMapHeavy;
    spec->mapVersion = ctx->tileMapVersion;
    return MC_OK;
}

extern "C" {

int32_t mcskin_cuda_band_rows(const McConfig* cfg, int32_t first, int32_t stride) {
    if (!cfg || cfg->width <= 0 || cfg->height <= 0 || cfg->tile_size <= 0) return 0;
    DevFrame f{};
    f.width = cfg->width;
    f.height = cfg->height;
    f.tile_size = cfg->tile_size;
    f.tiles_x = (cfg->width + cfg->tile_size - 1) / cfg->tile_size;
    f.tiles_y = (cfg->height + cfg->tile_size - 1) / cfg->tile_size;
    return band_pixel_rows(f, first, stride);
}

int32_t mcskin_cuda_context_render_bands(McContext* ctx, int32_t first, int32_t stride, void* dOutF32, void* dOutU8,
                                         void* stream) {
    if (!ctx || !ctx->hasScene) return fail(MC_ERR_INVALID, "render_bands: no scene set");
    if (stride <= 0 || first < 0) return fail(MC_ERR_INVALID, "render_bands: bad partition");
    CU_TRY(cudaSetDevice(ctx->device));
    cudaStream_t s = stream ? static_cast<cudaStream_t>(stream) : ctx->stream;
    return render_bands(ctx, first, stride, static_cast<float4*>(dOutF32), static_cast<uchar4*>(dOutU8), s);
}

int32_t mcskin_cuda_context_render_rows_into_frame(McContext* ctx, int32_t first, int32_t stride, void* dFrameF32,
                                                    void* dFrameU8, void* stream) {
    if (!ctx || !ctx->hasScene) return fail(MC_ERR_INVALID, "render_rows_into_frame: no scene set");
    if (stride <= 0 || first < 0) return fail(MC_ERR_INVALID, "render_rows_into_frame: bad partition");
    CU_TRY(cudaSetDevice(ctx->device));
    cudaStream_t s = stream ? static_cast<cudaStream_t>(stream) : ctx->stream;
    return render_bands(ctx, first, stride, static_cast<float4*>(dFrameF32), static_cast<uchar4*>(dFrameU8), s, true);
}

int32_t mcskin_cuda_context_render_tiles_into_frame(McContext* ctx, const int32_t* tiles, int32_t nTiles, void* dFrameF32,
                                                     void* dFrameU8, void* stream) {
    if (!ctx || !ctx->hasScene) return fail(MC_ERR_INVALID, "render_tiles_into_frame: no scene set");
    if (nTiles < 0 || (nTiles > 0 && !tiles)) return fail(MC_ERR_INVALID, "render_tiles_into_frame: bad tile list");
    CU_TRY(cudaSetDevice(ctx->device));
    cudaStream_t s = stream ? static_cast<cudaStream_t>(stream) : ctx->stream;
    BandSpec spec;
    bool empty = false;
    const int rc = prepare_tile_map(ctx, tiles, nTiles, s, &spec, &empty);
    if (rc != MC_OK || empty) return rc;
    return render_bands(ctx, 0, 1, static_cast<float4*>(dFrameF32), static_cast<uchar4*>(dFrameU8), s, true, &spec);
}

int32_t mcskin_cuda_context_debug_block_times(McContext* ctx, uint64_t* out, int32_t capacity) {
    if (!ctx || capacity < 0) return fail(MC_ERR_INVALID, "debug_block_times: bad argument");
    CU_TRY(cudaSetDevice(ctx->device));
    CU_TRY(cudaDeviceSynchronize());
    const int n = std::min(ctx->blockTimesCount, capacity);
    if (out && n > 0) CU_TRY(cudaMemcpy(out, ctx->blockTimes.p, static_cast<size_t>(n) * 4 * sizeof(uint64_t), cudaMemcpyDeviceToHost));
    return ctx->blockTimesCount;
}

}
```

### minecraftskin_raytracer_b200/csrc/kernels.cu

```cuda
#include "kernels.cuh"
#include "wavefront.cuh"

#include "dev_shade.cuh"
#include "dev_stage.cuh"
#include "dev_sample.cuh"

namespace mcskin {
MCSKIN_VARIANT_BEGIN

namespace {

struct TileGeom {
    int x, y, w, h;
    int bandRow0;
    int localIndex;
};

__device__ __forceinline__ TileGeom tile_geom(const DevFrame& fr, const BandView& band, int localTile) {
    TileGeom g;
    int tx, ty, outRow;
    if (band.tile_map) {
        const int id = __ldg(band.tile_map + localTile);
        ty = id / fr.tiles_x;
        tx = id - ty * fr.tiles_x;
// ... 1043 lines not shown

__global__ void k_soft_shadow(const DevFrame fr, const FramePointers fp, const float* points, const float* normals,
                              const uint32_t* seeds, int samples, int n, float* out) {
    const int i = blockIdx.x * blockDim.x + threadIdx.x;
    if (i >= n) return;
    const SceneView sc = scene_view(fp.blob, fp.texels, fr);
    out[i] = soft_shadow(sc, fr, ld3(points + 3 * i), ld3(normals + 3 * i), samples, seeds[i]);
}

__global__ void k_ambient_occlusion(const DevFrame fr, const FramePointers fp, const float* points,
                                    const float* normals, const uint32_t* seeds, int samples, float radius, int n,
                                    float* out) {
    const int i = blockIdx.x * blockDim.x + threadIdx.x;
    if (i >= n) return;
    const SceneView sc = scene_view(fp.blob, fp.texels, fr);
    out[i] = ambient_occlusion(sc, ld3(points + 3 * i), ld3(normals + 3 * i), samples, radius, seeds[i]);
}

__global__ void k_generate_rays(const DevFrame fr, const float* uv, int n, McRay* out) {
    const int i = blockIdx.x * blockDim.x + threadIdx.x;
    if (i >= n) return;
    const Ray r = camera_ray(fr, uv[2 * i], uv[2 * i + 1]);
    out[i].origin[0] = r.o.x; out[i].origin[1] = r.o.y; out[i].origin[2] = r.o.z;
    out[i].dir[0] = r.d.x; out[i].dir[1] = r.d.y; out[i].dir[2] = r.d.z;
}

__global__ void k_background(const DevFrame fr, const float* uv, int n, float4* out) {
    const int i = blockIdx.x * blockDim.x + threadIdx.x;
    if (i >= n) return;
    out[i] = fr.use_config ? config_background(fr, uv[2 * i], uv[2 * i + 1]) : flat_background(fr);
}

__global__ void k_peer_signal(unsigned int* flag, const unsigned int value) {
    __threadfence_system();
    asm volatile("st.release.sys.global.u32 [%0], %1;" ::"l"(flag), "r"(value) : "memory");
}
__global__ void k_peer_wait(const unsigned int* flags, const int n, const unsigned int value, unsigned int* timedOut) {
    const int i = threadIdx.x;
    if (i < n) {
        const long long t0 = clock64();
        for (;;) {
            unsigned int v;
            asm volatile("ld.relaxed.sys.global.u32 %0, [%1];" : "=r"(v) : "l"(flags + i) : "memory");
            if (static_cast<int>(v - value) >= 0) {
                asm volatile("ld.acquire.sys.global.u32 %0, [%1];" : "=r"(v) : "l"(flags + i) : "memory");
                break;
            }
            if (clock64() - t0 > 4000000000ll) {
                if (timedOut) *timedOut = 1u;
                break;
            }
            __nanosleep(100);
        }
    }
}

__global__ void __launch_bounds__(kBlockThreads) k_fp32_peak(const int iters, float* sink) {
    float x0 = threadIdx.x * 1e-3f, x1 = x0 + 0.1f, x2 = x0 + 0.2f, x3 = x0 + 0.3f;
    float x4 = x0 + 0.4f, x5 = x0 + 0.5f, x6 = x0 + 0.6f, x7 = x0 + 0.7f;
    const float a = 0.999f + blockIdx.x * 1e-9f, b = 1e-3f;
#pragma unroll 4
    for (int i = 0; i < iters; ++i) {
        x0 = x0 * a + b; x1 = x1 * a + b; x2 = x2 * a + b; x3 = x3 * a + b;
        x4 = x4 * a + b; x5 = x5 * a + b; x6 = x6 * a + b; x7 = x7 * a + b;
    }
    const float s = ((x0 + x1) + (x2 + x3)) + ((x4 + x5) + (x6 + x7));
    if (s == 123.456f) sink[0] = s;
}

__global__ void k_powf(const float* x, const float* y, int n, float* out) {
    const int i = blockIdx.x * blockDim.x + threadIdx.x;
    if (i < n) out[i] = powf_ref(x[i], y[i]);
}

__global__ void k_sincos(const float* angles, int n, float* outSin, float* outCos) {
    const int i = blockIdx.x * blockDim.x + threadIdx.x;
    if (i >= n) return;
    float sn, cs;
    sincos_ref(angles[i], &sn, &cs);
    outSin[i] = sn;
    outCos[i] = cs;
}

__global__ void k_aov(const DevFrame fr, const FramePointers fp, int* outTriId) {
    const int px = blockIdx.x * blockDim.x + threadIdx.x;
    const int py = blockIdx.y * blockDim.y + threadIdx.y;
    if (px >= fr.width || py >= fr.height) return;
    const SceneView sc = scene_view(fp.blob, fp.texels, fr);
    const float u = (static_cast<float>(px) + 0.5f) / fr.width_f;
    const float v = (static_cast<float>(py) + 0.5f) / fr.height_f;
    const Hit h = closest_hit(sc, camera_ray(fr, u, v));
    outTriId[py * fr.width + px] = h.box >= 0 ? h.box * 12 + h.face * 2 : -1;
}

__global__ void k_slice_skins(const unsigned char* records, const size_t recordStride, const size_t jobOffset) {
    const SkinSliceJob job = *reinterpret_cast<const SkinSliceJob*>(records + blockIdx.y * recordStride + jobOffset);
    const int f = blockIdx.x;
    if (f == 0 && threadIdx.x == 0) {
        job.texels[job.nTexels] = make_float4(1.0f, 0.0f, 1.0f, 1.0f);
        job.texels[job.nTexels + 1] = make_float4(0.0f, 0.0f, 0.0f, 1.0f);
    }
    if (f >= job.nFaces) return;
    const SkinFaceSource src = job.faces[f];
    const int n = src.w * src.h;
    for (int i = threadIdx.x; i < n; i += blockDim.x) {
        const int row = i / src.w, col = i - row * src.w;
        const int sx = src.x + (src.mirror ? src.w - 1 - col : col), sy = src.y + row;
        float4 t = make_float4(0.0f, 0.0f, 0.0f, 1.0f);
        if (sx >= 0 && sx < job.atlasW && sy >= 0 && sy < job.atlasH) {
            const uchar4 b = job.atlas[sy * job.atlasW + sx];
            t = make_float4(static_cast<float>(b.x) / 255.0f, static_cast<float>(b.y) / 255.0f, static_cast<float>(b.z) / 255.0f,
                            static_cast<float>(b.w) / 255.0f);
        }
        job.texels[src.dst + i] = t;
    }
}

inline int blocks_for(int n) { return (n + kBlockThreads - 1) / kBlockThreads; }

}

static int log2_if_warp_spp(int spp) {
    for (int lg = 0; lg <= 5; ++lg)
        if (spp == (1 << lg)) return lg;
    return -1;
}

static size_t pix_smem_limit() {
    static SmemOptIn optIn;
    static const void* const fns[] = {
        reinterpret_cast<const void*>(k_primary_pix<false>), reinterpret_cast<const void*>(k_primary_pix<true>),
        reinterpret_cast<const void*>(k_primary_pix_fixed<16, true, false>), reinterpret_cast<const void*>(k_primary_pix_fixed<16, false, false>),
        reinterpret_cast<const void*>(k_primary_pix_fixed<4, true, false>), reinterpret_cast<const void*>(k_primary_pix_fixed<4, false, false>),
        reinterpret_cast<const void*>(k_primary_pix_fixed<16, true, true>), reinterpret_cast<const void*>(k_primary_pix_fixed<16, false, true>),
        reinterpret_cast<const void*>(k_primary_pix_fixed<4, true, true>), reinterpret_cast<const void*>(k_primary_pix_fixed<4, false, true>)};
    return optIn.limit(fns, static_cast<int>(sizeof(fns) / sizeof(fns[0])));
}

static void launch_primary_pix(const DevFrame& fr, const FramePointers& fp, const BandView& band, const ActiveList& list,
                               uint32_t* tileStates, bool seedTiles, int primaryTargetBlocks, int heavyTargetTiles,
                               const BatchSlice* batch, int nScenes, unsigned int blobBytes, cudaStream_t stream) {
    const int nTiles = band_tile_count(band, fr.tiles_x);
    const size_t pixSmem = ((sizeof(PixStreamSmem) + 15) & ~size_t(15)) + blobBytes;
    const int roundsPerTile = (fr.tile_size * fr.tile_size + kBlockThreads - 1) / kBlockThreads;
    const int allTiles = nTiles * (batch ? nScenes : 1);
    int parts = (primaryTargetBlocks + allTiles - 1) / allTiles;
    parts = parts < 1 ? 1 : (parts > roundsPerTile ? roundsPerTile : parts);
    while (roundsPerTile % parts) --parts;
    int partsHeavy = (heavyTargetTiles + allTiles - 1) / allTiles;
    partsHeavy = partsHeavy < parts ? parts : (partsHeavy > roundsPerTile ? roundsPerTile : partsHeavy);
    while (roundsPerTile % partsHeavy) --partsHeavy;
    TileOrder order = make_tile_order(fr, band, partsHeavy, parts);
    const int statesPerTile = primary_states_per_tile(fr, nTiles, batch ? nScenes : 1, primaryTargetBlocks, heavyTargetTiles);
    order.round_states = statesPerTile > 1 ? statesPerTile : 0;
    if (fr.draws_per_sample > 0 && seedTiles) {
        k_tile_seed<<<(nTiles + 63) / 64, 64, 0, stream>>>(fr, band, tileStates, statesPerTile);
        if (statesPerTile > 1)
            k_tile_rounds<<<nTiles, kBlockThreads, 0, stream>>>(tileStates, statesPerTile,
                                                                static_cast<unsigned int>(kBlockThreads * fr.spp * fr.draws_per_sample));
    }
    const dim3 grid(order.n_heavy * order.parts_heavy + (nTiles - order.n_heavy) * order.parts_light, batch ? nScenes : 1);
    const bool fixedForm = fr.draws_per_sample == 2 && fr.spp > 1 && !fr.dof_on && fr.uv_recip;
#define MCSKIN_LAUNCH_PIX(KERNEL)                                                                                \
    do {                                                                                                        \
        if (batch) KERNEL<true><<<grid, kBlockThreads, pixSmem, stream>>>(fr, fp, band, list, tileStates, order, batch);   \
        else KERNEL<false><<<grid, kBlockThreads, pixSmem, stream>>>(fr, fp, band, list, tileStates, order, batch);        \
// ... 59 lines not shown
    else
        k_shade_cta<<<gridBlocks, kBlockThreads, fp.blob_bytes, stream>>>(fr, fp, band, list, firstSlot);
    if (!aov_any(aov)) return 1;
    k_aov_listed<<<gridBlocks, kBlockThreads, 0, stream>>>(fr, fp, list, firstSlot, *aov);
    return 2;
}

void launch_aov_defaults(const DevFrame& fr, const BandView& band, const McAovTargets& planes, const AovView* aovBatch, int nScenes,
                         cudaStream_t stream) {
    const int nTiles = band_tile_count(band, fr.tiles_x);
    if (nTiles <= 0 || nScenes <= 0) return;
    if (aovBatch) k_aov_defaults<true><<<dim3(nTiles, nScenes), kBlockThreads, 0, stream>>>(fr, band, planes, aovBatch);
    else k_aov_defaults<false><<<nTiles, kBlockThreads, 0, stream>>>(fr, band, planes, aovBatch);
}

void launch_intersect(const DevFrame& fr, const FramePointers& fp, int box, const McRay* rays, int n, McHit* out,
                      cudaStream_t stream) {
    if (n > 0) k_intersect<<<blocks_for(n), kBlockThreads, 0, stream>>>(fr, fp, box, rays, n, out);
}
void launch_trace(const DevFrame& fr, const FramePointers& fp, int depth, const McRay* rays, int n, float4* out,
                  cudaStream_t stream) {
    if (n > 0) k_trace<<<blocks_for(n), kBlockThreads, 0, stream>>>(fr, fp, depth, rays, n, out);
}
void launch_shade_hits(const DevFrame& fr, const FramePointers& fp, const McHit* hits, const float* viewDirs,
                       const float* shadowFactors, int n, float4* out, cudaStream_t stream) {
    if (n > 0) k_shade_hits<<<blocks_for(n), kBlockThreads, 0, stream>>>(fr, fp, hits, viewDirs, shadowFactors, n, out);
}
void launch_in_shadow(const DevFrame& fr, const FramePointers& fp, const float* points, const float* normals,
                      const float* lights, int n, int* out, cudaStream_t stream) {
    if (n > 0) k_in_shadow<<<blocks_for(n), kBlockThreads, 0, stream>>>(fr, fp, points, normals, lights, n, out);
}
void launch_soft_shadow(const DevFrame& fr, const FramePointers& fp, const float* points, const float* normals,
                        const uint32_t* seeds, int samples, int n, float* out, cudaStream_t stream) {
    if (n > 0)
        k_soft_shadow<<<blocks_for(n), kBlockThreads, 0, stream>>>(fr, fp, points, normals, seeds, samples, n, out);
}
void launch_ambient_occlusion(const DevFrame& fr, const FramePointers& fp, const float* points, const float* normals,
                              const uint32_t* seeds, int samples, float radius, int n, float* out,
                              cudaStream_t stream) {
    if (n > 0)
        k_ambient_occlusion<<<blocks_for(n), kBlockThreads, 0, stream>>>(fr, fp, points, normals, seeds, samples,
                                                                         radius, n, out);
}
void launch_generate_rays(const DevFrame& fr, const float* uv, int n, McRay* out, cudaStream_t stream) {
    if (n > 0) k_generate_rays<<<blocks_for(n), kBlockThreads, 0, stream>>>(fr, uv, n, out);
}
void launch_background(const DevFrame& fr, const float* uv, int n, float4* out, cudaStream_t stream) {
    if (n > 0) k_background<<<blocks_for(n), kBlockThreads, 0, stream>>>(fr, uv, n, out);
}
int primary_launch_order(const DevFrame& fr, int first, int stride, int partsHeavy, int partsLight, int* outTile,
                         int* outPart, int* outParts, int capacity) {
    BandView band{};
    band.first_tile_row = first;
    band.tile_row_stride = stride;
    band.n_tile_rows = (fr.tiles_y <= 0 || first < 0 || stride <= 0 || first >= fr.tiles_y) ? 0 : (fr.tiles_y - first + stride - 1) / stride;
    const int nTiles = band.n_tile_rows * fr.tiles_x;
    if (nTiles <= 0) return 0;
    partsLight = partsLight < 1 ? 1 : partsLight;
    partsHeavy = partsHeavy < partsLight ? partsLight : partsHeavy;
    const TileOrder order = make_tile_order(fr, band, partsHeavy, partsLight);
    const int blocks = order.n_heavy * order.parts_heavy + (nTiles - order.n_heavy) * order.parts_light;
    for (int b = 0; b < blocks && b < capacity; ++b) {
        int slot, part, parts;
        block_to_slot(order, b, &slot, &part, &parts);
        if (outTile) outTile[b] = ordered_tile(order, fr.tiles_x, slot);
        if (outPart) outPart[b] = part;
        if (outParts) outParts[b] = parts;
    }
    return blocks;
}

void launch_fp32_peak(int blocks, int iters, float* sink, cudaStream_t stream) {
    k_fp32_peak<<<blocks, kBlockThreads, 0, stream>>>(iters, sink);
}
void launch_peer_signal(unsigned int* flag, unsigned int value, cudaStream_t stream) {
    k_peer_signal<<<1, 1, 0, stream>>>(flag, value);
}
void launch_peer_wait(const unsigned int* flags, int n, unsigned int value, unsigned int* timedOut, cudaStream_t stream) {
    if (n > 0) k_peer_wait<<<1, ((n + 31) / 32) * 32, 0, stream>>>(flags, n, value, timedOut);
}
void launch_powf(const float* x, const float* y, int n, float* out, cudaStream_t stream) {
    if (n > 0) k_powf<<<blocks_for(n), kBlockThreads, 0, stream>>>(x, y, n, out);
}
void launch_sincos(const float* angles, int n, float* outSin, float* outCos, cudaStream_t stream) {
    if (n > 0) k_sincos<<<blocks_for(n), kBlockThreads, 0, stream>>>(angles, n, outSin, outCos);
}
void launch_slice_skins(const unsigned char* records, size_t recordStride, size_t jobOffset, int nSkins, cudaStream_t stream) {
    if (nSkins > 0) k_slice_skins<<<dim3(kSkinMaxFaces, nSkins), 96, 0, stream>>>(records, recordStride, jobOffset);
}
void launch_aov(const DevFrame& fr, const FramePointers& fp, int* outTriId, cudaStream_t stream) {
    if (fr.width <= 0 || fr.height <= 0) return;
    dim3 block(32, 8);
    dim3 grid((fr.width + 31) / 32, (fr.height + 7) / 8);
    k_aov<<<grid, block, 0, stream>>>(fr, fp, outTriId);
}

MCSKIN_VARIANT_END
}
```

### minecraftskin_raytracer_b200/csrc/kernels.cuh

```cuda
#pragma once
#include <cuda_runtime.h>
#include <stdint.h>

#include <algorithm>
#include <mutex>

#include "dev_types.cuh"
#include "host_prep.hpp"
#include "mcskin_cuda.h"

namespace mcskin {

constexpr int kBlockThreads = 256;
constexpr unsigned int kMaxSceneSmemBytes = 40u * 1024u;

class SmemOptIn {
public:
    size_t limit(const void* const* fns, int nFns) {
        int dev = 0;
        if (cudaGetDevice(&dev) != cudaSuccess || dev < 0 || dev >= kMaxDevices) return 0;
        std::lock_guard<std::mutex> lock(mu_);
        if (known_[dev]) return limit_[dev];
        int optin = 0;
        if (cudaDeviceGetAttribute(&optin, cudaDevAttrMaxSharedMemoryPerBlockOptin, dev) != cudaSuccess) optin = 0;
// ... 16 lines not shown
private:
    static constexpr int kMaxDevices = 64;
    std::mutex mu_;
    size_t limit_[kMaxDevices] = {};
    bool known_[kMaxDevices] = {};
};

struct BandView {
    int first_tile_row, tile_row_stride, n_tile_rows;
    int out_first_row, out_row_stride;
    float4* out_f32;
    uchar4* out_u8;
    float4* hot_f32;
    uchar4* hot_u8;
    const int* tile_map;
    int n_tiles, n_heavy;
    int far_output;
    unsigned long long* block_times;
};
__host__ __device__ inline int band_tile_count(const BandView& band, int tilesX) {
    return band.tile_map ? band.n_tiles : band.n_tile_rows * tilesX;
}
__host__ __device__ inline bool aov_any(const McAovTargets* a) { return a && (a->coverage || a->depth || a->tri_id); }

struct ActiveList {
    unsigned int* count;
    uint2* slot_pixel;
    float* records;
    unsigned int capacity;
    unsigned int* count_host;
};

struct FramePointers {
    const unsigned char* blob;
    const float4* texels;
    unsigned int blob_bytes;
};

#define MCSKIN_HOT_KERNEL_LAUNCHERS                                                                                      \
    bool launch_primary(const DevFrame& fr, const FramePointers& fp, const BandView& band, const ActiveList& list,      \
                        int classify, uint32_t* tileStates, bool seedTiles, int primaryTargetBlocks, int heavyTargetTiles, \
                        cudaStream_t stream);                                                                           \
    int launch_shade(const DevFrame& fr, const FramePointers& fp, const BandView& band, const ActiveList& list,         \
                     int gridBlocks, unsigned int* groupCounter, unsigned int firstSlot, cudaStream_t stream,           \
                     int variant = 1, const McAovTargets* aov = nullptr);
MCSKIN_HOT_KERNEL_LAUNCHERS
namespace plain {
MCSKIN_HOT_KERNEL_LAUNCHERS
}
namespace counter {
MCSKIN_HOT_KERNEL_LAUNCHERS
}

inline int primary_states_per_tile(const DevFrame& fr, int nTiles, int nScenes, int primaryTargetBlocks, int heavyTargetTiles) {
    if (nTiles <= 0 || fr.draws_per_sample <= 0) return 1;
    const int roundsPerTile = (fr.tile_size * fr.tile_size + kBlockThreads - 1) / kBlockThreads;
    const long long allTiles = static_cast<long long>(nTiles) * std::max(1, nScenes);
    const bool split = primaryTargetBlocks > allTiles || heavyTargetTiles > allTiles;
    return split && roundsPerTile > 1 ? roundsPerTile : 1;
}

void launch_intersect(const DevFrame& fr, const FramePointers& fp, int box, const McRay* rays, int n, McHit* out,
                      cudaStream_t stream);
void launch_trace(const DevFrame& fr, const FramePointers& fp, int depth, const McRay* rays, int n, float4* out,
                  cudaStream_t stream);
void launch_shade_hits(const DevFrame& fr, const FramePointers& fp, const McHit* hits, const float* viewDirs,
                       const float* shadowFactors, int n, float4* out, cudaStream_t stream);
void launch_in_shadow(const DevFrame& fr, const FramePointers& fp, const float* points, const float* normals,
                      const float* lights, int n, int* out, cudaStream_t stream);
void launch_soft_shadow(const DevFrame& fr, const FramePointers& fp, const float* points, const float* normals,
                        const uint32_t* seeds, int samples, int n, float* out, cudaStream_t stream);
void launch_ambient_occlusion(const DevFrame& fr, const FramePointers& fp, const float* points, const float* normals,
                              const uint32_t* seeds, int samples, float radius, int n, float* out,
                              cudaStream_t stream);
void launch_generate_rays(const DevFrame& fr, const float* uv, int n, McRay* out, cudaStream_t stream);
void launch_background(const DevFrame& fr, const float* uv, int n, float4* out, cudaStream_t stream);
int primary_launch_order(const DevFrame& fr, int first, int stride, int partsHeavy, int partsLight, int* outTile,
                         int* outPart, int* outParts, int capacity);
void launch_fp32_peak(int blocks, int iters, float* sink, cudaStream_t stream);
void launch_peer_signal(unsigned int* flag, unsigned int value, cudaStream_t stream);
void launch_peer_wait(const unsigned int* flags, int n, unsigned int value, unsigned int* timedOut, cudaStream_t stream);
void launch_powf(const float* x, const float* y, int n, float* out, cudaStream_t stream);
void launch_sincos(const float* angles, int n, float* outSin, float* outCos, cudaStream_t stream);
void launch_aov(const DevFrame& fr, const FramePointers& fp, int* outTriId, cudaStream_t stream);

struct SkinSliceJob {
    const uchar4* atlas;
    const SkinFaceSource* faces;
    float4* texels;
    int atlasW, atlasH, nFaces, nTexels;
};
void launch_slice_skins(const unsigned char* records, size_t recordStride, size_t jobOffset, int nSkins, cudaStream_t stream);

}
```

### minecraftskin_raytracer_b200/csrc/wavefront.cu

```cuda
#include "wavefront.cuh"

#include <algorithm>

#include "dev_sample.cuh"

namespace mcskin {
MCSKIN_VARIANT_BEGIN

namespace {

constexpr int kWfThreads = 256;
#ifndef MCSKIN_WF_HIT0_MIN_BLOCKS
#define MCSKIN_WF_HIT0_MIN_BLOCKS 3
#endif
#ifndef MCSKIN_WF_SHADE_MIN_BLOCKS
#define MCSKIN_WF_SHADE_MIN_BLOCKS 4
#endif
#define WF_HIT0_BOUNDS __launch_bounds__(kWfThreads, MCSKIN_WF_HIT0_MIN_BLOCKS)
#ifdef MCSKIN_WF_SHADOW_MIN_BLOCKS
#define WF_SHADOW_BOUNDS __launch_bounds__(kWfThreads, MCSKIN_WF_SHADOW_MIN_BLOCKS)
#else
#define WF_SHADOW_BOUNDS __launch_bounds__(kWfThreads)
#endif
#define WF_SHADE_BOUNDS __launch_bounds__(kWfThreads, QUEUED ? MCSKIN_WF_SHADE_MIN_BLOCKS : 2)
// ... 92 lines not shown
                }
                if (fr.max_bounces < 0) {
                    wv.tail[p] = hit.box < 0 ? config_background(fr, u, v) : config_background(fr, 0.5f, 0.5f);
                    wv.top[p] = 0;
                } else if (hit.box < 0) {
                    wv.tail[p] = config_background(fr, u, v);
                    wv.top[p] = 0;
                } else {
                    alive = true;
                }
            } else {
                wv.top[p] = -1;
            }
        }
        for (int depth = 0; __any_sync(0xffffffffu, alive); ++depth) {
            const bool queued = enqueue_hit(wv.q, &wv.qCount[0], wv.qCapacity, alive, hit, ray, static_cast<unsigned int>(p), depth);
            if (!alive) continue;
            if (!queued) {
                wv.top[p] = kPathOverflow;
                alive = false;
            } else if (depth < lastBounce) {
                const V3 N = normalize3(hit_normal(sc, hit));
                const V3 D = normalize3(ray.d);
                V3 Rd = D - N * (2.0f * dot3(D, N));
                Rd = normalize3(Rd);
                ray.o = hit.p + N * kReflectEpsilon;
                ray.d = Rd;
                hit = closest_hit(sc, ray);
                if (hit.box < 0) {
                    wv.tail[p] = flat_background(fr);
                    wv.top[p] = depth + 1;
                    alive = false;
                }
            } else {
                alive = false;
            }
        }
    }
}

template <bool BATCH>
__global__ void __launch_bounds__(kWfThreads)
k_wf_overflow(const DevFrame fr, const FramePointers fp_, const ActiveList list_, const WaveView wv_,
              const BatchSlice* __restrict__ batch) {
    __shared__ __align__(8) uint64_t stageBar;
    const FramePointers& fp = BATCH ? batch[blockIdx.y].fp : fp_;
    const ActiveList& list = BATCH ? batch[blockIdx.y].list : list_;
    const WaveView& wv = BATCH ? batch[blockIdx.y].wave : wv_;
    if (wv.qCount[0] <= wv.qCapacity) return;
    unsigned int count = *list.count;
    if (count > list.capacity) count = list.capacity;
    if (count > wv.slotCapacity) count = wv.slotCapacity;
    const unsigned long long nPaths = static_cast<unsigned long long>(count) * fr.spp;
    stage_bulk(g_sceneSmem, fp.blob, fp.blob_bytes, &stageBar);
    const SceneView sc = scene_view(g_sceneSmem, fp.texels, fr);
    const int spp = fr.spp, dps = fr.draws_per_sample;
    for (unsigned long long p = static_cast<unsigned long long>(blockIdx.x) * kWfThreads + threadIdx.x; p < nPaths;
         p += static_cast<unsigned long long>(gridDim.x) * kWfThreads) {
        if (wv.top[p] != kPathOverflow) continue;
        const unsigned int slot = static_cast<unsigned int>(p / spp);
        const int s = static_cast<int>(p - static_cast<unsigned long long>(slot) * spp);
        const uint2 sp = list.slot_pixel[slot];
        const int px = static_cast<int>(sp.y & 0xffffu), py = static_cast<int>(sp.y >> 16);
        float d0 = 0.0f, d1 = 0.0f, d2 = 0.0f, d3 = 0.0f;
        const float* rec = list.records + (static_cast<size_t>(slot) * spp + s) * dps;
        if (dps == 2) {
            const float2 r = *reinterpret_cast<const float2*>(rec);
            d0 = r.x; d1 = r.y;
        } else if (dps == 4) {
            const float4 r = *reinterpret_cast<const float4*>(rec);
            d0 = r.x; d1 = r.y; d2 = r.z; d3 = r.w;
        }
        const SampleDraws sd = assign_draws(fr, d0, d1, d2, d3);
        TraceOptions opt;
        opt.start_depth = 0;
        opt.primary_uv = true;
        sample_uv(fr, px, py, sd, &opt.u, &opt.v);
        wv.tail[p] = trace_path(sc, fr, primary_ray(fr, opt.u, opt.v, sd), opt);
        wv.top[p] = 0;
    }
}

constexpr int kPendCap = 2 * kWfThreads;
constexpr int kShadowRound = 8;
constexpr int kPtStride = kShadowRound * 3 + 1;
struct ShadowSmem {
    float4 pendP[kPendCap];
    float4 pendO[kPendCap];
    unsigned int pendI[kPendCap];
    float pts[kWfThreads * kPtStride];
    uint4 engine[kWfThreads];
    unsigned int lit[kWfThreads];
    unsigned int head, tail;
    unsigned int chunk;
};
static_assert((kPendCap & (kPendCap - 1)) == 0, "ring size must be a power of two");

#ifndef MCSKIN_WF_SOFT_MIN_BLOCKS
#define MCSKIN_WF_SOFT_MIN_BLOCKS 4
#endif
template <bool BATCH>
__global__ void __launch_bounds__(kWfThreads, MCSKIN_WF_SOFT_MIN_BLOCKS)
k_wf_softshadow(const DevFrame fr, const FramePointers fp_, const WaveView wv_, const BatchSlice* __restrict__ batch) {
    __shared__ __align__(8) uint64_t stageBar;
    const FramePointers& fp = BATCH ? batch[blockIdx.y].fp : fp_;
    const WaveView& wv = BATCH ? batch[blockIdx.y].wave : wv_;
    unsigned int n = wv.qCount[0];
    if (n > wv.qCapacity) n = wv.qCapacity;
    const unsigned int nChunks = (n + kWfThreads - 1) / kWfThreads;
    if (blockIdx.x >= nChunks) return;
    stage_bulk(g_sceneSmem, fp.blob, fp.blob_bytes, &stageBar);
    const SceneView sc = scene_view(g_sceneSmem, fp.texels, fr);
    ShadowSmem* sm = reinterpret_cast<ShadowSmem*>(g_sceneSmem + ((fp.blob_bytes + 15u) & ~15u));
    const int tid = threadIdx.x, lane = tid & 31;
    const HitQueueView q = wv.q;
    const int N = fr.shadow_samples;
    const int rounds = (N + kShadowRound - 1) / kShadowRound;
    const V3 lightCentre = ld3(fr.light_pos);
    const uint32_t one = fr.spp > 0 ? 1u : 0u;
    unsigned int* chunkCounter = wv.qCount + 1;
    if (tid == 0) {
        sm->head = 0u;
        sm->tail = 0u;
    }
    for (;;) {
        __syncthreads();
        if (tid == 0) sm->chunk = atomicAdd(chunkCounter, 1u);
        __syncthreads();
        const unsigned int c = sm->chunk;
        const bool last = c >= nChunks;
        if (!last) {
            const unsigned int i = c * kWfThreads + tid;
            bool pend = false;
            float4 eP = make_float4(0.f, 0.f, 0.f, 0.f), eO = eP;
            if (i < n) {
                const float4 g = q.geo[i];
                const Hit h = unpack_hit(g, make_float4(0.f, 0.f, 0.f, 0.f));
                const V3 origin = h.p + hit_normal(sc, h) * kShadowEpsilon;
                const uint32_t allow = bundle_box_mask(sc, origin, lightCentre, fr.light_radius);
                if (allow == 0u && sc.n_boxes <= 32) {
                    wv.lit[i] = static_cast<unsigned int>(N);
                } else {
                    pend = true;
                    eP = make_float4(h.p.x, h.p.y, h.p.z, __uint_as_float(shadow_seed(h.p, unpack_depth(g))));
                    eO = make_float4(origin.x, origin.y, origin.z, __uint_as_float(allow));
                }
            }
            const unsigned int m = __ballot_sync(0xffffffffu, pend);
            if (m) {
                unsigned int base = 0u;
                if (lane == 0) base = atomicAdd(&sm->tail, static_cast<unsigned int>(__popc(m)));
                base = __shfl_sync(0xffffffffu, base, 0);
                if (pend) {
                    const unsigned int pos = (base + __popc(m & ((1u << lane) - 1u))) & (kPendCap - 1);
                    sm->pendP[pos] = eP;
                    sm->pendO[pos] = eO;
                    sm->pendI[pos] = i;
                }
            }
            __syncthreads();
        }
        for (;;) {
            const unsigned int head = sm->head;
            const unsigned int avail = sm->tail - head;
            if (avail == 0u || (!last && avail < static_cast<unsigned int>(kWfThreads))) break;
            const unsigned int cnt = avail < static_cast<unsigned int>(kWfThreads) ? avail : static_cast<unsigned int>(kWfThreads);
            const bool mine = static_cast<unsigned int>(tid) < cnt;
            if (mine) sm->lit[tid] = 0u;
            for (int round = 0; round < rounds; ++round) {
                const int ns = min(kShadowRound, N - round * kShadowRound);
                if (mine) {
                    const float4 eP = sm->pendP[(head + tid) & (kPendCap - 1)];
                    const V3 P = mk3(eP.x, eP.y, eP.z);
                    FreshStream rng;
                    if (round == 0) {
                        rng.seed_memo(__float_as_uint(eP.w), one, wv.seedMemo);
                    } else {
                        const uint4 e = sm->engine[tid];
                        rng.cur = e.x; rng.nxt = e.y; rng.far = e.z; rng.j = e.w;
                    }
                    soft_shadow_positions(fr, P, ns, rng, sm->pts + tid * kPtStride);
                    if (round + 1 < rounds) sm->engine[tid] = make_uint4(rng.cur, rng.nxt, rng.far, rng.j);
                }
                __syncthreads();
                const unsigned int nRays = cnt * static_cast<unsigned int>(ns);
                for (unsigned int r = tid; r < nRays; r += kWfThreads) {
                    const unsigned int e = ns == kShadowRound ? r >> 3 : r / static_cast<unsigned int>(ns);
                    const unsigned int k = r - e * static_cast<unsigned int>(ns);
                    const float4 eO = sm->pendO[(head + e) & (kPendCap - 1)];
                    const float* pt = sm->pts + e * kPtStride + k * 3u;
                    if (!in_shadow_from(sc, mk3(eO.x, eO.y, eO.z), mk3(pt[0], pt[1], pt[2]), __float_as_uint(eO.w)))
                        atomicAdd(&sm->lit[e], 1u);
                }
                __syncthreads();
            }
            if (mine) wv.lit[sm->pendI[(head + tid) & (kPendCap - 1)]] = sm->lit[tid];
            __syncthreads();
            if (tid == 0) sm->head = head + cnt;
            __syncthreads();
        }
        if (last) break;
    }
}

template <bool BATCH>
__global__ void __launch_bounds__(kWfThreads)
k_wf_hardshadow(const DevFrame fr, const FramePointers fp_, const WaveView wv_, const BatchSlice* __restrict__ batch) {
    __shared__ __align__(8) uint64_t stageBar;
    const FramePointers& fp = BATCH ? batch[blockIdx.y].fp : fp_;
    const WaveView& wv = BATCH ? batch[blockIdx.y].wave : wv_;
    unsigned int n = wv.qCount[0];
    if (n > wv.qCapacity) n = wv.qCapacity;
    if (blockIdx.x * kWfThreads >= n) return;
    stage_bulk(g_sceneSmem, fp.blob, fp.blob_bytes, &stageBar);
    const SceneView sc = scene_view(g_sceneSmem, fp.texels, fr);
    const HitQueueView q = wv.q;
    const V3 lightCentre = ld3(fr.light_pos);
    for (unsigned int i = blockIdx.x * kWfThreads + threadIdx.x; i < n; i += gridDim.x * kWfThreads) {
        const Hit h = unpack_hit(q.geo[i], make_float4(0.f, 0.f, 0.f, 0.f));
        wv.lit[i] = in_shadow(sc, h.p, normalize3(hit_normal(sc, h)), lightCentre) ? 0u : 1u;
    }
}

template <bool QUEUED, bool BATCH>
__global__ void WF_SHADE_BOUNDS
k_wf_shade(const DevFrame fr, const FramePointers fp_, const WaveView wv_, const BatchSlice* __restrict__ batch) {
    const FramePointers& fp = BATCH ? batch[blockIdx.y].fp : fp_;
    const WaveView& wv = BATCH ? batch[blockIdx.y].wave : wv_;
    __shared__ __align__(8) uint64_t stageBar;
    unsigned int n = wv.qCount[0];
    if (n > wv.qCapacity) n = wv.qCapacity;
    if (blockIdx.x * kWfThreads >= n) return;
    stage_bulk(g_sceneSmem, fp.blob, fp.blob_bytes, &stageBar);
    const SceneView sc = scene_view(g_sceneSmem, fp.texels, fr);
    const HitQueueView q = wv.q;
    const bool cfg = fr.use_config != 0;
    const size_t cap = wv.pathCapacity;
    const int lastBounce = min(fr.max_bounces, wv.levels);

    for (unsigned int i = blockIdx.x * kWfThreads + threadIdx.x; i < n; i += gridDim.x * kWfThreads) {
        const float4 g = q.geo[i], o = q.org[i], dd = q.dir[i];
        const Hit h = unpack_hit(g, o);
        const int d = unpack_depth(g);
        const unsigned int path = __float_as_uint(dd.w);
        const V3 P = h.p;
        const V3 nrm = hit_normal(sc, h);
        const float4 tex = hit_texel(sc, h);
        const V3 viewDir = normalize3(mk3(o.x, o.y, o.z) - P);
        float vis;
        if (QUEUED) {
            vis = static_cast<float>(wv.lit[i]) / static_cast<float>(wv.shadowRays);
            if (wv.shadowMode == kShadowHard) vis = wv.lit[i] ? 1.0f : 0.0f;
        } else if (cfg && fr.soft_on) {
            vis = soft_shadow(sc, fr, P, nrm, fr.shadow_samples, shadow_seed(P, d));
        } else {
            vis = in_shadow(sc, P, normalize3(nrm), ld3(fr.light_pos)) ? 0.0f : 1.0f;
        }
        float4 shaded = shade_lit(fr, P, nrm, tex, viewDir, vis);
        const float alpha = shaded.w;
        if (cfg && fr.ao_on && d == 0) {
            const float ao = ambient_occlusion(sc, P, nrm, fr.ao_samples, fr.ao_radius, ao_seed(P));
            const float f = 1.0f - fr.ao_intensity * (1.0f - ao);
            shaded.x *= f;
            shaded.y *= f;
            shaded.z *= f;
        }
        if (d < lastBounce) {
            wv.stack[static_cast<size_t>(d) * cap + path] = make_float4(shaded.x, shaded.y, shaded.z, alpha);
        } else {
            shaded.w = alpha;
            wv.tail[path] = clamp4(shaded);
            wv.top[path] = d;
        }
    }
}

__device__ __forceinline__ float4 fold_path(const WaveView& wv, size_t path) {
    float4 c = wv.tail[path];
    const int top = wv.top[path];
    if (top > 0) {
        const size_t cap = wv.pathCapacity;
        const float alpha0 = wv.stack[path].w;
        const float keep = 1.0f - kReflectivity;
        for (int k = top - 1; k >= 0; --k) {
// ... 104 lines not shown
    }
}

__global__ void k_batch_reset(const BatchSlice* __restrict__ batch, const int nScenes, const int nQueueCounters) {
    const int s = blockIdx.x * blockDim.x + threadIdx.x;
    if (s >= nScenes) return;
    *batch[s].list.count = 0u;
    for (int i = 0; i < nQueueCounters; ++i) batch[s].wave.qCount[i] = 0u;
}

int log2_pow2_le32(int v) {
    for (int lg = 0; lg <= 5; ++lg)
        if (v == (1 << lg)) return lg;
    return -1;
}

size_t align256(size_t v) { return (v + 255) & ~static_cast<size_t>(255); }

int shadow_mode_of(const DevFrame& fr) {
    if (!(fr.use_config && fr.soft_on)) return kShadowHard;
    if (fr.shadow_samples <= 1 || fr.light_radius < 1e-4f || 2 * fr.shadow_samples > kFreshStreamMaxDraws)
        return kShadowInThread;
    return kShadowSoft;
}
int stack_levels_of(const DevFrame& fr) {
    return fr.max_bounces < 0 ? 0 : (fr.max_bounces > kMaxStackDepth ? kMaxStackDepth : fr.max_bounces);
}
constexpr size_t kEntryBytes = 3 * sizeof(float4) + sizeof(unsigned int);
constexpr int kQueueCounters = 4;

}

int wavefront_max_hits_per_path(const DevFrame& fr) { return stack_levels_of(fr) + 1; }
size_t wavefront_bytes_per_path(const DevFrame& fr, bool aov) {
    return sizeof(float4) + sizeof(int) + sizeof(float4) * stack_levels_of(fr) + (aov ? sizeof(float) + sizeof(int) : 0);
}
size_t wavefront_bytes_per_entry() { return kEntryBytes; }
size_t wavefront_fixed_bytes(const DevFrame&) { return 256 * 16 + sizeof(unsigned int) * kQueueCounters; }

bool wavefront_carve(const DevFrame& fr, void* base, size_t bytes, unsigned int pathCapacity, unsigned int entryCapacity,
                     int gridBlocks, WaveView* out, AovView* aov) {
    WaveView w{};
    w.pathCapacity = pathCapacity;
    w.slotCapacity = pathCapacity / static_cast<unsigned int>(fr.spp);
    w.qCapacity = entryCapacity;
    w.levels = stack_levels_of(fr);
    w.shadowMode = shadow_mode_of(fr);
    w.shadowRays = w.shadowMode == kShadowSoft ? fr.shadow_samples : (w.shadowMode == kShadowHard ? 1 : 0);
    w.gridBlocks = gridBlocks;
    w.softGrid = gridBlocks;
    unsigned char* p = static_cast<unsigned char*>(base);
    size_t off = 0;
    auto take = [&](size_t n) {
        void* r = p + off;
        off = align256(off + n);
        return r;
    };
    const size_t cap = pathCapacity, ents = entryCapacity;
    w.q.geo = static_cast<float4*>(take(ents * sizeof(float4)));
    w.q.org = static_cast<float4*>(take(ents * sizeof(float4)));
    w.q.dir = static_cast<float4*>(take(ents * sizeof(float4)));
    w.lit = static_cast<unsigned int*>(take(ents * sizeof(unsigned int)));
    w.tail = static_cast<float4*>(take(cap * sizeof(float4)));
    w.top = static_cast<int*>(take(cap * sizeof(int)));
    w.stack = static_cast<float4*>(take(std::max<size_t>(16, cap * sizeof(float4) * w.levels)));
    w.qCount = static_cast<unsigned int*>(take(sizeof(unsigned int) * kQueueCounters));
    float* aovT = aov ? static_cast<float*>(take(cap * sizeof(float))) : nullptr;
    int* aovId = aov ? static_cast<int*>(take(cap * sizeof(int))) : nullptr;
    if (off > bytes) return false;
    if (aov) {
        aov->t = aovT;
        aov->id = aovId;
    }
    *out = w;
    return true;
}

void launch_batch_reset(const BatchSlice* batch, int nScenes, cudaStream_t stream) {
    if (nScenes > 0) k_batch_reset<<<(nScenes + 127) / 128, 128, 0, stream>>>(batch, nScenes, kQueueCounters);
}

void launch_wavefront(const DevFrame& fr, const FramePointers& fp, const BandView& band, const ActiveList& list,
                      const WaveView& wv, unsigned int* groupCounter, cudaStream_t stream, int* launches,
                      const BatchSlice* batch, int nScenes, const AovView* aovView, const AovView* aovBatch) {
    int n = 0;
    const AovView av = aovView ? *aovView : AovView{};
    const int grid = wv.gridBlocks;
    const unsigned int ny = batch ? static_cast<unsigned int>(nScenes) : 1u;
    const dim3 g(grid, ny);
    const size_t blob = fp.blob_bytes;
#define MCSKIN_WF_LAUNCH(KERNEL, GRID, SMEM, ...)                                                   \
    do {                                                                                            \
        if (batch) KERNEL<true><<<GRID, kWfThreads, SMEM, stream>>>(__VA_ARGS__, batch);            \
        else KERNEL<false><<<GRID, kWfThreads, SMEM, stream>>>(__VA_ARGS__, batch);                 \
        ++n;                                                                                        \
    } while (0)
    if (wv.shadowMode == kShadowSoft) {
        static SmemOptIn optIn;
        static const void* const fns[] = {reinterpret_cast<const void*>(k_wf_softshadow<false>),
                                          reinterpret_cast<const void*>(k_wf_softshadow<true>)};
        optIn.limit(fns, 2);
    }
    if (!batch) cudaMemsetAsync(wv.qCount, 0, sizeof(unsigned int) * kQueueCounters, stream);
    const bool aov = batch ? aovBatch != nullptr : av.t != nullptr;
    if (batch) {
        if (aov) k_wf_trace<true, true><<<g, kWfThreads, blob, stream>>>(fr, fp, list, wv, av, aovBatch, batch);
        else k_wf_trace<true, false><<<g, kWfThreads, blob, stream>>>(fr, fp, list, wv, av, aovBatch, batch);
    } else {
        if (aov) k_wf_trace<false, true><<<g, kWfThreads, blob, stream>>>(fr, fp, list, wv, av, aovBatch, batch);
        else k_wf_trace<false, false><<<g, kWfThreads, blob, stream>>>(fr, fp, list, wv, av, aovBatch, batch);
    }
    ++n;
    if (fr.max_bounces >= 0) {
        if (wv.shadowMode == kShadowSoft) {
            const dim3 gs(std::max(1, std::min<int>(grid, wv.softGrid)), ny);
            const size_t smem = ((blob + 15u) & ~size_t(15)) + sizeof(ShadowSmem);
            MCSKIN_WF_LAUNCH(k_wf_softshadow, gs, smem, fr, fp, wv);
        } else if (wv.shadowMode == kShadowHard) {
            MCSKIN_WF_LAUNCH(k_wf_hardshadow, g, blob, fr, fp, wv);
        }
        if (wv.shadowMode != kShadowInThread) {
            if (batch) k_wf_shade<true, true><<<g, kWfThreads, blob, stream>>>(fr, fp, wv, batch);
            else k_wf_shade<true, false><<<g, kWfThreads, blob, stream>>>(fr, fp, wv, batch);
        } else {
            if (batch) k_wf_shade<false, true><<<g, kWfThreads, blob, stream>>>(fr, fp, wv, batch);
            else k_wf_shade<false, false><<<g, kWfThreads, blob, stream>>>(fr, fp, wv, batch);
        }
        ++n;
        if (static_cast<unsigned long long>(wv.qCapacity) < static_cast<unsigned long long>(wv.pathCapacity) * (wv.levels + 1))
            MCSKIN_WF_LAUNCH(k_wf_overflow, g, blob, fr, fp, list, wv);
    }
    const int lg = log2_pow2_le32(fr.spp);
    if (lg >= 0) {
        const bool farImage = !batch && band.far_output != 0;
        if (aov) {
            if (batch) k_wf_resolve_warp<true, false, true><<<g, kWfThreads, 0, stream>>>(fr, band, list, wv, lg, av, aovBatch, batch);
            else if (farImage) k_wf_resolve_warp<false, true, true><<<g, kWfThreads, 0, stream>>>(fr, band, list, wv, lg, av, aovBatch, batch);
            else k_wf_resolve_warp<false, false, true><<<g, kWfThreads, 0, stream>>>(fr, band, list, wv, lg, av, aovBatch, batch);
        } else {
            if (batch) k_wf_resolve_warp<true, false, false><<<g, kWfThreads, 0, stream>>>(fr, band, list, wv, lg, av, aovBatch, batch);
            else if (farImage) k_wf_resolve_warp<false, true, false><<<g, kWfThreads, 0, stream>>>(fr, band, list, wv, lg, av, aovBatch, batch);
            else k_wf_resolve_warp<false, false, false><<<g, kWfThreads, 0, stream>>>(fr, band, list, wv, lg, av, aovBatch, batch);
        }
        ++n;
    } else {
        if (batch && aov) k_wf_resolve_pixel<true, true><<<g, kWfThreads, 0, stream>>>(fr, band, list, wv, av, aovBatch, batch);
        else if (batch) k_wf_resolve_pixel<true, false><<<g, kWfThreads, 0, stream>>>(fr, band, list, wv, av, aovBatch, batch);
        else if (aov) k_wf_resolve_pixel<false, true><<<g, kWfThreads, 0, stream>>>(fr, band, list, wv, av, aovBatch, batch);
        else k_wf_resolve_pixel<false, false><<<g, kWfThreads, 0, stream>>>(fr, band, list, wv, av, aovBatch, batch);
        ++n;
    }
#undef MCSKIN_WF_LAUNCH
    if (!batch && wv.slotCapacity < list.capacity) {
        n += MCSKIN_VARIANT_NS::launch_shade(fr, fp, band, list, grid, groupCounter, wv.slotCapacity, stream, 1, aov ? &av.planes : nullptr);
    }
    if (launches) *launches += n;
}

MCSKIN_VARIANT_END
}
```

### minecraftskin_raytracer_b200/csrc/wavefront.cuh

```cuda
#pragma once
#include "kernels.cuh"

namespace mcskin {

struct HitQueueView {
    float4* geo;
    float4* org;
    float4* dir;
};

struct WaveView {
    HitQueueView q;
    unsigned int* lit;
    float4* tail;
    float4* stack;
    int* top;
    unsigned int* qCount;
    unsigned int pathCapacity;
    unsigned int slotCapacity;
    unsigned int qCapacity;
    int levels;
    int shadowMode;
    int shadowRays;
    int gridBlocks;
    int softGrid;
    uint2* seedMemo;
};

struct AovView {
    McAovTargets planes;
    float* t;
    int* id;
};

enum : int {
    kShadowHard = 0,
    kShadowSoft = 1,
    kShadowInThread = 2
};

struct BatchSlice {
    FramePointers fp;
    BandView band;
    ActiveList list;
    WaveView wave;
};
static_assert(sizeof(BatchSlice) == 256, "a BatchSlice is indexed by blockIdx.y: keep its stride a power of two");

size_t wavefront_bytes_per_path(const DevFrame& fr, bool aov = false);
size_t wavefront_bytes_per_entry();
size_t wavefront_fixed_bytes(const DevFrame& fr);
int wavefront_max_hits_per_path(const DevFrame& fr);
bool wavefront_carve(const DevFrame& fr, void* base, size_t bytes, unsigned int pathCapacity, unsigned int entryCapacity,
                     int gridBlocks, WaveView* out, AovView* aov = nullptr);

void launch_aov_defaults(const DevFrame& fr, const BandView& band, const McAovTargets& planes, const AovView* aovBatch, int nScenes,
                         cudaStream_t stream);

#define MCSKIN_HOT_WAVEFRONT_LAUNCHERS                                                                                   \
    void launch_wavefront(const DevFrame& fr, const FramePointers& fp, const BandView& band, const ActiveList& list,    \
                          const WaveView& wave, unsigned int* groupCounter, cudaStream_t stream, int* launches,         \
                          const BatchSlice* batch = nullptr, int nScenes = 1, const AovView* aov = nullptr,             \
                          const AovView* aovBatch = nullptr);                                                          \
    void launch_batch_reset(const BatchSlice* batch, int nScenes, cudaStream_t stream);                                 \
    bool launch_primary_batch(const DevFrame& fr, const BandView& band, uint32_t* tileStates, bool seedTiles,           \
                              const BatchSlice* batch, int nScenes, unsigned int blobBytes, int primaryTargetBlocks,    \
                              cudaStream_t stream);
MCSKIN_HOT_WAVEFRONT_LAUNCHERS
namespace plain {
MCSKIN_HOT_WAVEFRONT_LAUNCHERS
}
namespace counter {
MCSKIN_HOT_WAVEFRONT_LAUNCHERS
}

}
```

### minecraftskin_raytracer_b200/lib.py

```python
from __future__ import annotations

import ctypes as C
from pathlib import Path

import numpy as np

from . import _abi
from ._abi import McConfig, McContext_p, McHit, McRay, McRenderStats, McScene, McTile
from .scene import FlatScene, pose_array

import os

LIB_PATH = Path(os.environ.get("MCSKIN_LIB") or (Path(__file__).resolve().parent / "_lib" / "libmcskin_cuda.so"))

DEFAULT_FRAME_LANES = 2

EXPORTS = [
    "mcskin_config_defaults", "mcskin_counter_word", "mcskin_host_copy_rows", "mcskin_generate_tiles", "mcskin_cuda_device_count", "mcskin_cuda_last_error",
    "mcskin_cuda_abi_version", "mcskin_cuda_abi_sizes", "mcskin_cuda_render", "mcskin_cuda_render_tile",
    "mcskin_cuda_render_multi", "mcskin_cuda_context_create", "mcskin_cuda_context_destroy",
    "mcskin_cuda_context_set_scene", "mcskin_cuda_context_render_bands", "mcskin_cuda_band_rows",
    "mcskin_cuda_context_sync", "mcskin_cuda_context_set_option", "mcskin_cuda_context_render_batch",
    "mcskin_cuda_intersect", "mcskin_cuda_trace", "mcskin_cuda_shade", "mcskin_cuda_in_shadow",
    "mcskin_cuda_soft_shadow", "mcskin_cuda_ambient_occlusion", "mcskin_cuda_generate_rays",
    "mcskin_cuda_background", "mcskin_cuda_aov", "mcskin_build_skin_scene", "mcskin_cuda_sincos",
    "mcskin_sincos_model", "mcskin_cuda_powf", "mcskin_powf_model", "mcskin_cuda_context_render_rows_into_frame",
    "mcskin_cuda_device_alloc", "mcskin_cuda_device_free", "mcskin_cuda_ipc_export", "mcskin_cuda_ipc_open",
    "mcskin_cuda_ipc_close", "mcskin_cuda_fp32_issue_peak", "mcskin_cuda_peer_signal", "mcskin_cuda_peer_wait",
    "mcskin_primary_launch_order", "mcskin_cuda_context_render_tiles_into_frame", "mcskin_partition_tiles",
    "mcskin_cuda_host_register", "mcskin_cuda_host_unregister", "mcskin_cuda_render_batch_multi",
    "mcskin_cuda_enable_peer_access", "mcskin_cuda_context_render_scene_tiles",
    "mcskin_cuda_context_debug_block_times", "mcskin_cuda_context_render_skin_batch",
    "mcskin_skin_layout", "mcskin_cuda_render_aovs", "mcskin_cuda_context_set_aov_targets",
]


class McSkinError(RuntimeError):
    def __init__(self, code: int, message: str):
        super().__init__(f"mcskin_cuda error {code}: {message}")
        self.code = code
        self.message = message


def _load() -> C.CDLL:
    if not LIB_PATH.exists():
        raise ImportError(
            f"{LIB_PATH} is missing: build the CUDA extension first "
            "(python -c 'import __graft_entry__ as g; g.build()').  There is no CPU fallback.")
    lib = C.CDLL(str(LIB_PATH))
    lib.mcskin_cuda_last_error.restype = C.c_char_p
    for name in EXPORTS:
        fn = getattr(lib, name)
        if name not in ("mcskin_cuda_last_error", "mcskin_config_defaults", "mcskin_cuda_context_destroy",
                        "mcskin_cuda_abi_sizes"):
            fn.restype = C.c_int32
    lib.mcskin_config_defaults.restype = None
    lib.mcskin_cuda_context_destroy.restype = None
    lib.mcskin_cuda_abi_sizes.restype = None
    lib.mcskin_counter_word.restype = C.c_uint32
    lib.mcskin_counter_word.argtypes = [C.c_uint32, C.c_uint32]
    return lib


_lib = _load()


def raw() -> C.CDLL:
    return _lib


def last_error() -> str:
    return (_lib.mcskin_cuda_last_error() or b"").decode("utf-8", "replace")


def _check(rc: int):
    if rc != 0:
        raise McSkinError(rc, last_error())


def _ptr(a: np.ndarray, ctype):
    return a.ctypes.data_as(C.POINTER(ctype))


def _f32(a, shape=None):
    a = np.ascontiguousarray(a, dtype=np.float32)
    return a.reshape(shape) if shape is not None else a


def device_count() -> int:
    return int(_lib.mcskin_cuda_device_count())


def abi_sizes() -> list[int]:
    out = (C.c_int32 * 8)()
    _lib.mcskin_cuda_abi_sizes(out)
    return list(out)


def config_defaults() -> McConfig:
    cfg = McConfig()
    _lib.mcskin_config_defaults(C.byref(cfg))
    return cfg


def counter_word(seed: int, k: int) -> int:
    return int(_lib.mcskin_counter_word(seed & 0xFFFFFFFF, k & 0xFFFFFFFF))


def host_copy_rows(dst: np.ndarray, src: np.ndarray, row_bytes: int, rows: int, pieces: int = 8,
                   dst_pitch: int | None = None, src_pitch: int | None = None):
    _check(_lib.mcskin_host_copy_rows(C.c_void_p(dst.ctypes.data), C.c_void_p(src.ctypes.data),
                                      C.c_uint64(row_bytes if dst_pitch is None else dst_pitch),
                                      C.c_uint64(row_bytes if src_pitch is None else src_pitch),
                                      C.c_uint64(row_bytes), C.c_uint64(rows), C.c_int32(pieces)))

# ... 195 lines not shown
    def __del__(self):
        try:
            self.close()
        except Exception:
            pass

    def set_option(self, name: str, value: int):
        _check(_lib.mcskin_cuda_context_set_option(self._h, name.encode(), C.c_int64(value)))

    def set_aov_targets(self, coverage: int = 0, depth: int = 0, tri_id: int = 0):
        t = _abi.McAovTargets(coverage or None, depth or None, tri_id or None)
        _check(_lib.mcskin_cuda_context_set_aov_targets(self._h, C.byref(t)))

    def set_scene(self, scene: FlatScene, cfg: McConfig):
        cs = scene.as_c()
        _check(_lib.mcskin_cuda_context_set_scene(self._h, C.byref(cs), C.byref(cfg)))
        self.cfg = _abi.copy_config(cfg)

    def band_rows(self, first_tile_row: int = 0, stride: int = 1) -> int:
        return int(_lib.mcskin_cuda_band_rows(C.byref(self.cfg), C.c_int32(first_tile_row), C.c_int32(stride)))

    def render_bands(self, first_tile_row: int, stride: int, d_out_f32: int = 0, d_out_u8: int = 0, stream: int = 0):
        _check(_lib.mcskin_cuda_context_render_bands(self._h, C.c_int32(first_tile_row), C.c_int32(stride),
                                                     C.c_void_p(d_out_f32 or None), C.c_void_p(d_out_u8 or None),
                                                     C.c_void_p(stream or None)))

    def render_rows_into_frame(self, first_tile_row: int, stride: int, d_frame_f32: int = 0, d_frame_u8: int = 0, stream: int = 0):
        _check(_lib.mcskin_cuda_context_render_rows_into_frame(self._h, C.c_int32(first_tile_row), C.c_int32(stride),
                                                               C.c_void_p(d_frame_f32 or None), C.c_void_p(d_frame_u8 or None),
                                                               C.c_void_p(stream or None)))

    def render_tiles_into_frame(self, tiles: np.ndarray, d_frame_f32: int = 0, d_frame_u8: int = 0, stream: int = 0):
        tiles = np.ascontiguousarray(tiles, dtype=np.int32)
        _check(_lib.mcskin_cuda_context_render_tiles_into_frame(self._h, _ptr(tiles, C.c_int32), C.c_int32(len(tiles)),
                                                                C.c_void_p(d_frame_f32 or None), C.c_void_p(d_frame_u8 or None),
                                                                C.c_void_p(stream or None)))

    def render_scene_tiles(self, scene, cfg: McConfig, tiles: np.ndarray, host_f32: np.ndarray | None = None,
                           host_u8: np.ndarray | None = None) -> float:
        cs = scene.as_c() if isinstance(scene, FlatScene) else scene
        ms = C.c_float(0.0)
        _check(_lib.mcskin_cuda_context_render_scene_tiles(
            self._h, C.byref(cs), C.byref(cfg), _ptr(tiles, C.c_int32), C.c_int32(len(tiles)),
            None if host_f32 is None else C.cast(C.c_void_p(host_f32.ctypes.data), C.POINTER(C.c_float)),
            None if host_u8 is None else C.cast(C.c_void_p(host_u8.ctypes.data), C.POINTER(C.c_uint8)), C.byref(ms)))
        self.cfg = cfg
        return float(ms.value)

    def render_batch(self, scenes: list[FlatScene], cfg: McConfig, d_out_f32: int = 0, d_out_u8: int = 0, stream: int = 0):
        arr = (McScene * len(scenes))(*[s.as_c() for s in scenes])
        self._keep = (arr, scenes)
        _check(_lib.mcskin_cuda_context_render_batch(self._h, arr, C.c_int32(len(scenes)), C.byref(cfg),
                                                     C.c_void_p(d_out_f32 or None), C.c_void_p(d_out_u8 or None),
                                                     C.c_void_p(stream or None)))
        self.cfg = _abi.copy_config(cfg)

    def render_skin_batch(self, atlases: np.ndarray, cfg: McConfig, poses=None, d_out_f32: int = 0, d_out_u8: int = 0, stream: int = 0):
        atlases = np.ascontiguousarray(atlases, dtype=np.uint8)
        if atlases.ndim != 4 or atlases.shape[3] != 4:
            raise ValueError("atlases must be uint8 [n, H, W, 4]")
        n, h, w = atlases.shape[:3]
        p, stride = None, 0
        if poses is not None:
            arr = np.asarray(poses, dtype=np.float32) if not isinstance(poses, (str, int)) else None
            if arr is not None and arr.ndim == 2:
                p, stride = np.ascontiguousarray(arr.reshape(n, 12)), 12
            else:
                p = pose_array(poses)
        self._keep = (atlases, p)
        _check(_lib.mcskin_cuda_context_render_skin_batch(self._h, _ptr(atlases, C.c_uint8), C.c_int32(w), C.c_int32(h), C.c_int32(n),
                                                          None if p is None else _ptr(p, C.c_float), C.c_int32(stride), C.byref(cfg),
                                                          C.c_void_p(d_out_f32 or None), C.c_void_p(d_out_u8 or None),
                                                          C.c_void_p(stream or None)))
        self.cfg = _abi.copy_config(cfg)

    def debug_block_times(self) -> np.ndarray:
        n = _lib.mcskin_cuda_context_debug_block_times(self._h, None, C.c_int32(0))
        _check(min(n, 0))
        out = np.zeros((n, 4), dtype=np.uint64)
        if n:
            _check(min(_lib.mcskin_cuda_context_debug_block_times(self._h, _ptr(out, C.c_uint64), C.c_int32(n)), 0))
        return out

    def sync(self) -> dict:
        stats = McRenderStats()
        _check(_lib.mcskin_cuda_context_sync(self._h, C.byref(stats)))
        return {k: getattr(stats, k) for k, _ in McRenderStats._fields_}


def intersect(scene: FlatScene, rays: np.ndarray, box: int = -1, device: int = 0) -> np.ndarray:
    rays = np.ascontiguousarray(rays, dtype=_abi.RAY_DTYPE)
    out = np.zeros(len(rays), dtype=_abi.HIT_DTYPE)
    cs = scene.as_c()
    _check(_lib.mcskin_cuda_intersect(C.byref(cs), C.c_int32(device), C.c_int32(box), _ptr(rays, McRay),
                                      C.c_int32(len(rays)), _ptr(out, McHit)))
    return out


def trace(scene: FlatScene, cfg: McConfig, rays: np.ndarray, depth: int = 0, use_config: bool = True,
          device: int = 0) -> np.ndarray:
    rays = np.ascontiguousarray(rays, dtype=_abi.RAY_DTYPE)
    out = np.zeros((len(rays), 4), dtype=np.float32)
    cs = scene.as_c()
    _check(_lib.mcskin_cuda_trace(C.byref(cs), C.byref(cfg), C.c_int32(device), C.c_int32(int(use_config)),
                                  C.c_int32(depth), _ptr(rays, McRay), C.c_int32(len(rays)), _ptr(out, C.c_float)))
    return out


def shade(scene: FlatScene, cfg: McConfig, hits: np.ndarray, view_dirs, shadow_factors=None,
          device: int = 0) -> np.ndarray:
    hits = np.ascontiguousarray(hits, dtype=_abi.HIT_DTYPE)
    vd = _f32(view_dirs, (-1, 3))
    sf = None if shadow_factors is None else _f32(shadow_factors)
    out = np.zeros((len(hits), 4), dtype=np.float32)
    cs = scene.as_c()
    _check(_lib.mcskin_cuda_shade(C.byref(cs), C.byref(cfg), C.c_int32(device), _ptr(hits, McHit), _ptr(vd, C.c_float),
                                  None if sf is None else _ptr(sf, C.c_float), C.c_int32(len(hits)),
                                  _ptr(out, C.c_float)))
    return out


def in_shadow(scene: FlatScene, points, normals, lights, device: int = 0) -> np.ndarray:
    p, n, l = _f32(points, (-1, 3)), _f32(normals, (-1, 3)), _f32(lights, (-1, 3))
    out = np.zeros(len(p), dtype=np.int32)
    cs = scene.as_c()
    _check(_lib.mcskin_cuda_in_shadow(C.byref(cs), C.c_int32(device), _ptr(p, C.c_float), _ptr(n, C.c_float),
                                      _ptr(l, C.c_float), C.c_int32(len(p)), _ptr(out, C.c_int32)))
    return out


def soft_shadow(scene: FlatScene, points, normals, seeds, samples: int, device: int = 0) -> np.ndarray:
    p, n = _f32(points, (-1, 3)), _f32(normals, (-1, 3))
    s = np.ascontiguousarray(seeds, dtype=np.uint32)
    out = np.zeros(len(p), dtype=np.float32)
    cs = scene.as_c()
    _check(_lib.mcskin_cuda_soft_shadow(C.byref(cs), C.c_int32(device), _ptr(p, C.c_float), _ptr(n, C.c_float),
                                        _ptr(s, C.c_uint32), C.c_int32(samples), C.c_int32(len(p)),
                                        _ptr(out, C.c_float)))
    return out


def ambient_occlusion(scene: FlatScene, points, normals, seeds, samples: int, radius: float,
                      device: int = 0) -> np.ndarray:
    p, n = _f32(points, (-1, 3)), _f32(normals, (-1, 3))
    s = np.ascontiguousarray(seeds, dtype=np.uint32)
    out = np.zeros(len(p), dtype=np.float32)
    cs = scene.as_c()
    _check(_lib.mcskin_cuda_ambient_occlusion(C.byref(cs), C.c_int32(device), _ptr(p, C.c_float), _ptr(n, C.c_float),
                                              _ptr(s, C.c_uint32), C.c_int32(samples), C.c_float(radius),
                                              C.c_int32(len(p)), _ptr(out, C.c_float)))
    return out


def generate_rays(scene: FlatScene, aspect: float, uv, device: int = 0) -> np.ndarray:
    uv = _f32(uv, (-1, 2))
    out = np.zeros(len(uv), dtype=_abi.RAY_DTYPE)
    cs = scene.as_c()
    _check(_lib.mcskin_cuda_generate_rays(C.byref(cs), C.c_int32(device), C.c_float(aspect), _ptr(uv, C.c_float),
                                          C.c_int32(len(uv)), _ptr(out, McRay)))
    return out


def background(scene: FlatScene, cfg: McConfig, uv, use_config: bool = True, device: int = 0) -> np.ndarray:
    uv = _f32(uv, (-1, 2))
    out = np.zeros((len(uv), 4), dtype=np.float32)
    cs = scene.as_c()
    _check(_lib.mcskin_cuda_background(C.byref(cs), C.byref(cfg), C.c_int32(device), C.c_int32(int(use_config)),
                                       _ptr(uv, C.c_float), C.c_int32(len(uv)), _ptr(out, C.c_float)))
    return out


def sincos(angles, device: int = 0):
    a = _f32(angles, (-1,))
    sn = np.zeros(len(a), dtype=np.float32)
    cs = np.zeros(len(a), dtype=np.float32)
    _check(_lib.mcskin_cuda_sincos(C.c_int32(device), _ptr(a, C.c_float), C.c_int32(len(a)), _ptr(sn, C.c_float),
                                   _ptr(cs, C.c_float)))
    return sn, cs


def powf(x, y, device: int = 0) -> np.ndarray:
    x, y = _f32(x, (-1,)), _f32(y, (-1,))
    out = np.zeros(len(x), dtype=np.float32)
    _check(_lib.mcskin_cuda_powf(C.c_int32(device), _ptr(x, C.c_float), _ptr(y, C.c_float), C.c_int32(len(x)), _ptr(out, C.c_float)))
    return out


def powf_model(x, y) -> np.ndarray:
    x, y = _f32(x, (-1,)), _f32(y, (-1,))
    out = np.zeros(len(x), dtype=np.float32)
    _lib.mcskin_powf_model(_ptr(x, C.c_float), _ptr(y, C.c_float), C.c_int32(len(x)), _ptr(out, C.c_float))
    return out


def primary_launch_order(scene: FlatScene, cfg: McConfig, first_tile_row: int = 0, stride: int = 1, parts_heavy: int = 1,
                         parts_light: int = 1):
    cs = scene.as_c()
    n = _lib.mcskin_primary_launch_order(C.byref(cs), C.byref(cfg), C.c_int32(first_tile_row), C.c_int32(stride),
                                         C.c_int32(parts_heavy), C.c_int32(parts_light), None, None, None, C.c_int32(0))
    _check(min(n, 0))
    tile, part, parts = (np.zeros(n, dtype=np.int32) for _ in range(3))
    if n:
        _lib.mcskin_primary_launch_order(C.byref(cs), C.byref(cfg), C.c_int32(first_tile_row), C.c_int32(stride),
                                         C.c_int32(parts_heavy), C.c_int32(parts_light), _ptr(tile, C.c_int32),
                                         _ptr(part, C.c_int32), _ptr(parts, C.c_int32), C.c_int32(n))
    return tile, part, parts


def fp32_issue_peak(device: int = 0) -> float:
    out = C.c_double(0.0)
    _check(_lib.mcskin_cuda_fp32_issue_peak(C.c_int32(device), C.byref(out)))
    return float(out.value)


def sincos_model(angles):
    a = _f32(angles, (-1,))
    sn = np.zeros(len(a), dtype=np.float32)
    cs = np.zeros(len(a), dtype=np.float32)
    _lib.mcskin_sincos_model(_ptr(a, C.c_float), C.c_int32(len(a)), _ptr(sn, C.c_float), _ptr(cs, C.c_float))
    return sn, cs


def aov(scene: FlatScene, cfg: McConfig, device: int = 0) -> np.ndarray:
    out = np.full((max(cfg.height, 0), max(cfg.width, 0)), -1, dtype=np.int32)
    cs = scene.as_c()
    _check(_lib.mcskin_cuda_aov(C.byref(cs), C.byref(cfg), C.c_int32(device), _ptr(out, C.c_int32)))
    return out
```

Baseline: 77170.

## Add conservative fast shadow verdict with exact fallback for soft-shadow rays

Soft-shadow rays are first classified by a cheap conservative test. It computes light sample points with fast sincos/sqrt and adds error-padded slab tests against box bounds and texel alpha, yielding lit, blocked or unknown. Only the unknown rays are compacted into a shared-memory queue and traced exactly with the reference light point and occlusion test. This aims to skip most full occlusion traversals, at the cost of extra shared-memory queueing, ballots and syncs, plus the risk that the error bounds are not truly conservative.

```diff
diff --git a/include/mcskin_cuda.h b/include/mcskin_cuda.h
--- a/include/mcskin_cuda.h
+++ b/include/mcskin_cuda.h
@@ -159,6 +159,8 @@
 int32_t mcskin_cuda_enable_peer_access(int32_t device, int32_t peer);
 int32_t mcskin_cuda_peer_wait(int32_t device, const void* d_flags, int32_t n, uint32_t value, void* d_timeout, void* stream);
 int32_t mcskin_cuda_context_debug_block_times(McContext* ctx, uint64_t* out, int32_t capacity);
+int32_t mcskin_cuda_context_debug_shadow_verdicts(McContext* ctx, uint64_t* out);
+int32_t mcskin_cuda_light_draw_errors(int32_t device, float* out);
 int32_t mcskin_cuda_context_set_aov_targets(McContext* ctx, const McAovTargets* d_targets);
 int32_t mcskin_cuda_context_sync(McContext* ctx, McRenderStats* stats);
 int32_t mcskin_cuda_context_set_option(McContext* ctx, const char* name, int64_t value);
diff --git a/minecraftskin_raytracer_b200/csrc/batch.cu b/minecraftskin_raytracer_b200/csrc/batch.cu
--- a/minecraftskin_raytracer_b200/csrc/batch.cu
+++ b/minecraftskin_raytracer_b200/csrc/batch.cu
@@ -229,7 +229,10 @@
             seeded = true;
             seededStatesPerTile = statesPerTile;
             int launches = 0;
-            build.launch_wavefront(f, first.fp, first.band, first.list, first.wave, nullptr, stream, &launches, gs, nS, nullptr, gAov);
+            ShadowVerdicts verdicts;
+            verdicts.fast = ctx->shadowFastVerdict;
+            build.launch_wavefront(f, first.fp, first.band, first.list, first.wave, nullptr, stream, &launches, gs, nS, nullptr, gAov,
+                                   verdicts);
         }
         CU_TRY(cudaGetLastError());
     }
diff --git a/minecraftskin_raytracer_b200/csrc/capi.cu b/minecraftskin_raytracer_b200/csrc/capi.cu
--- a/minecraftskin_raytracer_b200/csrc/capi.cu
+++ b/minecraftskin_raytracer_b200/csrc/capi.cu
@@ -357,6 +357,22 @@
     return st.down(outCos, dC, sizeof(float) * n);
 }
 
+int32_t mcskin_cuda_light_draw_errors(int32_t device, float* out) {
+    if (!out) return fail(MC_ERR_INVALID, "light_draw_errors: out is null");
+    std::lock_guard<std::mutex> lock(g_ctxMutex);
+    McContext* ctx = nullptr;
+    int rc = shared_context(device, &ctx);
+    if (rc != MC_OK) return rc;
+    Staged st{ctx, {}};
+    const unsigned int zeros[3] = {0u, 0u, 0u};
+    void* dE;
+    if ((rc = st.up(zeros, sizeof(zeros), &dE)) != MC_OK) return rc;
+    const float bound = launch_light_draw_errors(static_cast<unsigned int*>(dE), ctx->stream);
+    if ((rc = st.down(out, dE, sizeof(zeros))) != MC_OK) return rc;
+    out[3] = bound;
+    return MC_OK;
+}
+
 int32_t mcskin_cuda_aov(const McScene* scene, const McConfig* cfg, int32_t device, int32_t* outTriId) {
     if (!cfg || !outTriId) return fail(MC_ERR_INVALID, "aov: bad argument");
     if (cfg->width <= 0 || cfg->height <= 0) return MC_OK;
diff --git a/minecraftskin_raytracer_b200/csrc/capi_internal.hpp b/minecraftskin_raytracer_b200/csrc/capi_internal.hpp
--- a/minecraftskin_raytracer_b200/csrc/capi_internal.hpp
+++ b/minecraftskin_raytracer_b200/csrc/capi_internal.hpp
@@ -84,8 +84,10 @@
     int batchGroup = 128;
     int batchMode = 1;
     int debugPrimaryTiming = 0;
-};
-constexpr size_t kOptionCount = 19;
+    int shadowFastVerdict = 1;
+    int debugShadowVerdicts = 0;
+};
+constexpr size_t kOptionCount = 21;
 
 struct McContext : McOptions {
     int device = 0;
@@ -101,6 +103,7 @@
     DevBuf tileStates;
     DevBuf blockTimes;
     int blockTimesCount = 0;
+    DevBuf verdictCounts;
     DevBuf tileMap;
     std::vector<int32_t> tileMapHost, tileMapOrdered;
     std::vector<PixelRect> tileMapLightRects;
diff --git a/minecraftskin_raytracer_b200/csrc/context.cu b/minecraftskin_raytracer_b200/csrc/context.cu
--- a/minecraftskin_raytracer_b200/csrc/context.cu
+++ b/minecraftskin_raytracer_b200/csrc/context.cu
@@ -35,6 +35,8 @@
     {"wave_budget_bytes", nullptr, nullptr, &McOptions::waveBudgetBytes, 1 << 20, INT64_MAX, true, true},
     {"staged_copy_out", "MCSKIN_STAGED_COPY", &McOptions::stagedCopyOut, nullptr, 0, 1, false, false},
     {"shadow_seed_memo", "MCSKIN_SEED_MEMO", &McOptions::shadowSeedMemo, nullptr, 0, 1, false, true},
+    {"shadow_fast_verdict", "MCSKIN_SHADOW_FAST", &McOptions::shadowFastVerdict, nullptr, 0, 1, true, true},
+    {"debug_shadow_verdicts", nullptr, &McOptions::debugShadowVerdicts, nullptr, 0, 1, true, true},
 };
 static_assert(sizeof(kOptions) / sizeof(kOptions[0]) == kOptionCount, "kOptionCount counts the rows of kOptions");
 
diff --git a/minecraftskin_raytracer_b200/csrc/dev_intersect.cuh b/minecraftskin_raytracer_b200/csrc/dev_intersect.cuh
--- a/minecraftskin_raytracer_b200/csrc/dev_intersect.cuh
+++ b/minecraftskin_raytracer_b200/csrc/dev_intersect.cuh
@@ -179,8 +179,9 @@
 
 enum : int { kPosedUnknown = 0, kPosedMissed = 1, kPosedHitBeforeLimit = 2 };
 template <bool LIMITED>
-__device__ __forceinline__ int posed_box_verdict(const DevBox& bx, const Ray& ray, float limit, bool opaque) {
-    constexpr float kPad = 1e-2f;
+__device__ __forceinline__ int posed_box_verdict(const DevBox& bx, const Ray& ray, float limit, bool opaque,
+                                                 float extraPad = 0.0f) {
+    const float kPad = 1e-2f + extraPad;
     const V3 o = to_box_space(bx, ray.o, true);
     const V3 d = to_box_space(bx, ray.d, false);
     float tmin = -FLT_MAX, tmax = FLT_MAX;
@@ -524,6 +525,104 @@
     return occluded_among(sc, ray, dist, 0xffffffffu);
 }
 
+enum : int { kShadowUnknown = 0, kShadowLit = 1, kShadowBlocked = 2 };
+__device__ __forceinline__ int sure_largest(float x, float y, float z, V3 g) {
+    if (x - g.x > y + g.y && x - g.x > z + g.z) return 0;
+    if (y - g.y > x + g.x && y - g.y > z + g.z) return 1;
+    if (z - g.z > x + g.x && z - g.z > y + g.y) return 2;
+    return -1;
+}
+__device__ __forceinline__ float pick3(V3 v, int k) { return k == 0 ? v.x : (k == 1 ? v.y : v.z); }
+__device__ __forceinline__ float sure_alpha(const DevBox& bx, const float4* __restrict__ texels, V3 o, V3 D, V3 gs,
+                                            float g, float s, int axis, bool neg) {
+    const V3 p = mk3(fmaf(D.x, s, o.x), fmaf(D.y, s, o.y), fmaf(D.z, s, o.z));
+    const float gk = pick3(gs, axis);
+    const int a = axis == 0 ? 2 : 0, b = axis == 1 ? 2 : 1;
+    const int face = face_index(axis, neg);
+    const int2 ft = bx.face[face];
+    const float ta = (pick3(p, a) - bx.lo[a]) * rcp_fast(bx.size[a]) * static_cast<float>(ft.y & 0xffff);
+    const float tb = (pick3(p, b) - bx.lo[b]) * rcp_fast(bx.size[b]) * static_cast<float>(ft.y >> 16);
+    const float ma = (g + fabsf(pick3(D, a)) * gk) * static_cast<float>(ft.y & 0xffff);
+    const float mb = (g + fabsf(pick3(D, b)) * gk) * static_cast<float>(ft.y >> 16);
+    if (fabsf(ta - rintf(ta)) * bx.size[a] <= ma || fabsf(tb - rintf(tb)) * bx.size[b] <= mb) return -1.0f;
+    return __ldg(&texels[face_texel(bx, p, axis, neg, face)].w);
+}
+__device__ __forceinline__ int see_through_verdict(const DevBox& bx, const float4* __restrict__ texels, V3 o, V3 D,
+                                                   V3 gs, float g, V3 n, V3 f) {
+    const int ea = sure_largest(n.x, n.y, n.z, gs), xa = sure_largest(-f.x, -f.y, -f.z, gs);
+    if (ea < 0 || xa < 0) return kShadowUnknown;
+    const float tn = pick3(n, ea), gn = pick3(gs, ea), tf = pick3(f, xa), gf = pick3(gs, xa);
+    const bool xneg = pick3(D, xa) < 0.0f;
+    auto hit_at_exit = [&](bool hit) {
+        if (!hit) return kShadowLit;
+        if (tf + gf < 1.0f) return kShadowBlocked;
+        return tf - gf >= 1.0f ? kShadowLit : kShadowUnknown;
+    };
+    if (tn - gn > 0.0f && tf - gf > tn + gn) {
+        const float ae = sure_alpha(bx, texels, o, D, gs, g, tn, ea, pick3(D, ea) > 0.0f);
+        if (ae < 0.0f) return kShadowUnknown;
+        if (!(ae == 0.0f)) return tn + gn < 1.0f ? kShadowBlocked : kShadowUnknown;
+        if (!(bx.flags & kBoxOuter)) return kShadowLit;
+        const float ax = sure_alpha(bx, texels, o, D, gs, g, tf, xa, xneg);
+        if (ax < 0.0f) return kShadowUnknown;
+        return hit_at_exit(ax > 0.0f);
+    }
+    if (tn + gn < 0.0f && tf - gf > 0.0f) {
+        const float ax = sure_alpha(bx, texels, o, D, gs, g, tf, xa, xneg);
+        if (ax < 0.0f) return kShadowUnknown;
+        return hit_at_exit(!(ax == 0.0f));
+    }
+    return kShadowUnknown;
+}
+__device__ __forceinline__ int shadow_verdict(const SceneView& sc, V3 o, V3 pa, uint32_t allow, float eps, float g) {
+    const V3 D = pa - o;
+    const V3 a = mk3(fabsf(D.x), fabsf(D.y), fabsf(D.z));
+    const float big = fmaxf(a.x, fmaxf(a.y, a.z));
+    if (!(big > 1e-3f) || fminf(a.x, fminf(a.y, a.z)) < 1e-4f * big + 2.0f * eps) return kShadowUnknown;
+    const V3 inv = mk3(rcp_fast(D.x), rcp_fast(D.y), rcp_fast(D.z));
+    const V3 gs = mk3(g * fabsf(inv.x), g * fabsf(inv.y), g * fabsf(inv.z));
+    uint32_t todo = allow & sc.usable_mask;
+    if (sc.n_boxes < 32) todo &= (1u << sc.n_boxes) - 1u;
+    int verdict = kShadowLit;
+    while (todo) {
+        const int i = __ffs(todo) - 1;
+        todo &= todo - 1u;
+        if (kPosedScenes && ((sc.rotated_mask >> i) & 1u)) {
+            const float len2 = fmaf(D.x, D.x, fmaf(D.y, D.y, D.z * D.z));
+            const float rl = rsqrtf(len2);
+            Ray r;
+            r.o = o;
+            r.d = mk3(D.x * rl, D.y * rl, D.z * rl);
+            const int v = posed_box_verdict<true>(sc.boxes[i], r, len2 * rl, (sc.opaque_posed_mask >> i) & 1u, eps);
+            if (v == kPosedHitBeforeLimit) return kShadowBlocked;
+            if (v != kPosedMissed) verdict = kShadowUnknown;
+            continue;
+        }
+        const float4 L = sc.lo[i];
+        const float4 H = sc.hi[i];
+        const float ax = (L.x - o.x) * inv.x, bx = (H.x - o.x) * inv.x;
+        const float ay = (L.y - o.y) * inv.y, by = (H.y - o.y) * inv.y;
+        const float az = (L.z - o.z) * inv.z, bz = (H.z - o.z) * inv.z;
+        const float nx = fminf(ax, bx), fx = fmaxf(ax, bx);
+        const float ny = fminf(ay, by), fy = fmaxf(ay, by);
+        const float nz = fminf(az, bz), fz = fmaxf(az, bz);
+        const float g0 = fmaxf(fmaxf(nx - gs.x, ny - gs.y), fmaxf(nz - gs.z, 0.0f));
+        const float g1 = fminf(fminf(fx + gs.x, fy + gs.y), fz + gs.z);
+        if (g0 > g1 || g0 >= 1.0f) continue;
+        if ((sc.opaque_mask >> i) & 1u) {
+            const float h0 = fmaxf(fmaxf(nx + gs.x, ny + gs.y), fmaxf(nz + gs.z, 0.0f));
+            const float h1 = fminf(fminf(fx - gs.x, fy - gs.y), fz - gs.z);
+            if (h0 < h1 && g1 < 1.0f) return kShadowBlocked;
+            verdict = kShadowUnknown;
+            continue;
+        }
+        const int v = see_through_verdict(sc.boxes[i], sc.texels, o, D, gs, g, mk3(nx, ny, nz), mk3(fx, fy, fz));
+        if (v == kShadowBlocked) return kShadowBlocked;
+        if (v == kShadowUnknown) verdict = kShadowUnknown;
+    }
+    return verdict;
+}
+
 __device__ __forceinline__ bool bundle_clip(V3 a, V3 d, V3 inv, V3 lo, V3 hi, float grow, float* sEnd) {
     const float ax0 = (lo.x - grow - a.x) * inv.x, ax1 = (hi.x + grow - a.x) * inv.x;
     const float ay0 = (lo.y - grow - a.y) * inv.y, ay1 = (hi.y + grow - a.y) * inv.y;
diff --git a/minecraftskin_raytracer_b200/csrc/dev_shade.cuh b/minecraftskin_raytracer_b200/csrc/dev_shade.cuh
--- a/minecraftskin_raytracer_b200/csrc/dev_shade.cuh
+++ b/minecraftskin_raytracer_b200/csrc/dev_shade.cuh
@@ -277,24 +277,44 @@
     return shade_lit(fr, P, normal, tex, viewDir, vis);
 }
 
-template <class Engine>
-__device__ __forceinline__ void soft_shadow_positions(const DevFrame& fr, V3 point, int samples, Engine& rng,
-                                                      float* out ) {
-    const V3 lp = ld3(fr.light_pos);
-    const V3 toPoint = normalize3(point - lp);
-    V3 tangent, bitangent;
-    frame_about(toPoint, &tangent, &bitangent);
-    for (int i = 0; i < samples; ++i) {
-        const float angle = MCSKIN_TWO_PI_F * rng.next();
-        const float r = fr.light_radius * sqrtf(rng.next());
-        float sn, cs;
-        sincos_ref(angle, &sn, &cs);
-        const V3 offset = tangent * (r * cs) + bitangent * (r * sn);
-        const V3 samplePos = lp + offset;
-        out[3 * i] = samplePos.x;
-        out[3 * i + 1] = samplePos.y;
-        out[3 * i + 2] = samplePos.z;
-    }
+__device__ __forceinline__ void light_frame(const DevFrame& fr, V3 point, V3* tangent, V3* bitangent) {
+    frame_about(normalize3(point - ld3(fr.light_pos)), tangent, bitangent);
+}
+__device__ __forceinline__ V3 light_point(const DevFrame& fr, V3 tangent, V3 bitangent, float uAngle, float uRadius) {
+    const float angle = MCSKIN_TWO_PI_F * uAngle;
+    const float r = fr.light_radius * sqrtf(uRadius);
+    float sn, cs;
+    sincos_ref(angle, &sn, &cs);
+    const V3 offset = tangent * (r * cs) + bitangent * (r * sn);
+    return ld3(fr.light_pos) + offset;
+}
+
+constexpr float kLightDrawErr = 2e-6f;
+__device__ __forceinline__ void sincos_2pi_fast(float u, float* sn, float* cs) {
+    __sincosf(MCSKIN_TWO_PI_F * (u < 0.5f ? u : u - 1.0f), sn, cs);
+}
+__device__ __forceinline__ float sqrt_fast(float u) {
+    float r;
+    asm("sqrt.approx.ftz.f32 %0, %1;" : "=f"(r) : "f"(u));
+    return r;
+}
+__device__ __forceinline__ V3 light_point_fast(const DevFrame& fr, V3 tangent, V3 bitangent, float uAngle, float uRadius) {
+    float sn, cs;
+    sincos_2pi_fast(uAngle, &sn, &cs);
+    const float r = fr.light_radius * sqrt_fast(uRadius);
+    const float rc = r * cs, rs = r * sn;
+    return mk3(fmaf(tangent.x, rc, fmaf(bitangent.x, rs, fr.light_pos[0])),
+               fmaf(tangent.y, rc, fmaf(bitangent.y, rs, fr.light_pos[1])),
+               fmaf(tangent.z, rc, fmaf(bitangent.z, rs, fr.light_pos[2])));
+}
+__device__ __forceinline__ float light_point_fast_err(const DevFrame& fr) {
+    const float m = fmaxf(fabsf(fr.light_pos[0]), fmaxf(fabsf(fr.light_pos[1]), fabsf(fr.light_pos[2])));
+    return 8e-6f * fr.light_radius + 0x1p-21f * (m + 2.0f * fr.light_radius);
+}
+__device__ __forceinline__ float shadow_verdict_delta(const DevFrame& fr) {
+    float m = fmaxf(fabsf(fr.light_pos[0]), fmaxf(fabsf(fr.light_pos[1]), fabsf(fr.light_pos[2]))) + fr.light_radius;
+    for (int k = 0; k < 3; ++k) m = fmaxf(m, fmaxf(fabsf(fr.cull_lo[k]), fabsf(fr.cull_hi[k])));
+    return 0x1p-18f * (m + 1.0f);
 }
 
 __device__ __forceinline__ uint32_t shadow_seed(V3 P, int depth) {
diff --git a/minecraftskin_raytracer_b200/csrc/frame.cu b/minecraftskin_raytracer_b200/csrc/frame.cu
--- a/minecraftskin_raytracer_b200/csrc/frame.cu
+++ b/minecraftskin_raytracer_b200/csrc/frame.cu
@@ -187,6 +187,13 @@
     ctx->tileSeedValid = false;
     if (seedTiles) ++ctx->seedGen;
     const bool farOutput = spec.hotF32 || spec.hotU8 || is_far_memory(ctx, outF32) || is_far_memory(ctx, outU8);
+    ShadowVerdicts verdicts;
+    verdicts.fast = ctx->shadowFastVerdict;
+    if (ctx->debugShadowVerdicts && ctx->shadeMode == 0) {
+        CU_TRY(ctx->verdictCounts.reserve(3 * sizeof(unsigned long long)));
+        CU_TRY(cudaMemsetAsync(ctx->verdictCounts.p, 0, 3 * sizeof(unsigned long long), stream));
+        verdicts.counts = static_cast<unsigned long long*>(ctx->verdictCounts.p);
+    }
     for (int c = 0; c < nChunks; ++c) {
         const size_t unit0 = static_cast<size_t>(c) * plan.unitsPerChunk;
         const size_t units = std::min<size_t>(plan.unitsPerChunk, plan.nUnits - unit0);
@@ -241,7 +248,8 @@
         unsigned int* groupCounter = static_cast<unsigned int*>(ctx->countLog.p) + nChunks + c;
         const int shadeGrid = ctx->smCount * ctx->shadeBlocksPerSm;
         if (ctx->shadeMode == 0)
-            build.launch_wavefront(f, fp, band, list, wave, groupCounter, stream, &launches, nullptr, 1, aov ? &aovView : nullptr, nullptr);
+            build.launch_wavefront(f, fp, band, list, wave, groupCounter, stream, &launches, nullptr, 1, aov ? &aovView : nullptr, nullptr,
+                                   verdicts);
         else
             launches += build.launch_shade(f, fp, band, list, shadeGrid, groupCounter, 0u, stream, ctx->shadeMode, &ctx->aov);
         if (!ctx->capturing) CU_TRY(cudaEventRecord(ctx->passEvents[3 * c + 2], stream));
@@ -551,4 +559,19 @@
     return ctx->blockTimesCount;
 }
 
-}
+int32_t mcskin_cuda_context_debug_shadow_verdicts(McContext* ctx, uint64_t* out) {
+    if (!ctx || !out) return fail(MC_ERR_INVALID, "debug_shadow_verdicts: bad argument");
+    CU_TRY(cudaSetDevice(ctx->device));
+    CU_TRY(cudaDeviceSynchronize());
+    out[0] = out[1] = out[2] = 0;
+    for (int k = -1; k < ctx->splitLastRender; ++k) {
+        const McContext* c = k < 0 ? ctx : ctx->lanes[k];
+        if (!c->verdictCounts.p) continue;
+        uint64_t v[3];
+        CU_TRY(cudaMemcpy(v, c->verdictCounts.p, sizeof(v), cudaMemcpyDeviceToHost));
+        for (int i = 0; i < 3; ++i) out[i] += v[i];
+    }
+    return MC_OK;
+}
+
+}
diff --git a/minecraftskin_raytracer_b200/csrc/kernels.cu b/minecraftskin_raytracer_b200/csrc/kernels.cu
--- a/minecraftskin_raytracer_b200/csrc/kernels.cu
+++ b/minecraftskin_raytracer_b200/csrc/kernels.cu
@@ -1149,6 +1149,23 @@
     outCos[i] = cs;
 }
 
+__global__ void k_light_draw_errors(unsigned int* maxErr) {
+    constexpr unsigned int kSmall = 1u << 24, kTotal = kSmall + (8u << 23);
+    float es = 0.0f, ec = 0.0f, er = 0.0f;
+    for (unsigned int i = blockIdx.x * blockDim.x + threadIdx.x; i < kTotal; i += gridDim.x * blockDim.x) {
+        const float u = i < kSmall ? static_cast<float>(i) * 0x1p-32f : __uint_as_float(0x3b800000u + (i - kSmall));
+        float sn, cs, fs, fc;
+        sincos_ref(MCSKIN_TWO_PI_F * u, &sn, &cs);
+        sincos_2pi_fast(u, &fs, &fc);
+        es = fmaxf(es, fabsf(fs - sn));
+        ec = fmaxf(ec, fabsf(fc - cs));
+        er = fmaxf(er, fabsf(sqrt_fast(u) - sqrtf(u)));
+    }
+    atomicMax(&maxErr[0], __float_as_uint(es));
+    atomicMax(&maxErr[1], __float_as_uint(ec));
+    atomicMax(&maxErr[2], __float_as_uint(er));
+}
+
 __global__ void k_aov(const DevFrame fr, const FramePointers fp, int* outTriId) {
     const int px = blockIdx.x * blockDim.x + threadIdx.x;
     const int py = blockIdx.y * blockDim.y + threadIdx.y;
@@ -1374,6 +1391,10 @@
 void launch_powf(const float* x, const float* y, int n, float* out, cudaStream_t stream) {
     if (n > 0) k_powf<<<blocks_for(n), kBlockThreads, 0, stream>>>(x, y, n, out);
 }
+float launch_light_draw_errors(unsigned int* maxErr, cudaStream_t stream) {
+    k_light_draw_errors<<<4 * 148, kBlockThreads, 0, stream>>>(maxErr);
+    return kLightDrawErr;
+}
 void launch_sincos(const float* angles, int n, float* outSin, float* outCos, cudaStream_t stream) {
     if (n > 0) k_sincos<<<blocks_for(n), kBlockThreads, 0, stream>>>(angles, n, outSin, outCos);
 }
diff --git a/minecraftskin_raytracer_b200/csrc/kernels.cuh b/minecraftskin_raytracer_b200/csrc/kernels.cuh
--- a/minecraftskin_raytracer_b200/csrc/kernels.cuh
+++ b/minecraftskin_raytracer_b200/csrc/kernels.cuh
@@ -122,6 +122,7 @@
 void launch_peer_wait(const unsigned int* flags, int n, unsigned int value, unsigned int* timedOut, cudaStream_t stream);
 void launch_powf(const float* x, const float* y, int n, float* out, cudaStream_t stream);
 void launch_sincos(const float* angles, int n, float* outSin, float* outCos, cudaStream_t stream);
+float launch_light_draw_errors(unsigned int* maxErr, cudaStream_t stream);
 void launch_aov(const DevFrame& fr, const FramePointers& fp, int* outTriId, cudaStream_t stream);
 
 struct SkinSliceJob {
diff --git a/minecraftskin_raytracer_b200/csrc/wavefront.cu b/minecraftskin_raytracer_b200/csrc/wavefront.cu
--- a/minecraftskin_raytracer_b200/csrc/wavefront.cu
+++ b/minecraftskin_raytracer_b200/csrc/wavefront.cu
@@ -198,8 +198,10 @@
 }
 
 constexpr int kPendCap = 2 * kWfThreads;
+constexpr int kExactCap = 2 * kWfThreads;
 constexpr int kShadowRound = 8;
-constexpr int kPtStride = kShadowRound * 3 + 1;
+constexpr int kPtFrame = kShadowRound * 2;
+constexpr int kPtStride = kPtFrame + 7;
 struct ShadowSmem {
     float4 pendP[kPendCap];
     float4 pendO[kPendCap];
@@ -207,17 +209,23 @@
     float pts[kWfThreads * kPtStride];
     uint4 engine[kWfThreads];
     unsigned int lit[kWfThreads];
+    unsigned short exact[kExactCap];
+    unsigned int exactTail;
+    unsigned int verdicts[3];
+    float eps, grow;
     unsigned int head, tail;
     unsigned int chunk;
 };
-static_assert((kPendCap & (kPendCap - 1)) == 0, "ring size must be a power of two");
+static_assert((kPendCap & (kPendCap - 1)) == 0 && (kExactCap & (kExactCap - 1)) == 0, "ring sizes must be powers of two");
+static_assert(kExactCap >= 2 * kWfThreads && kWfThreads * kShadowRound <= 65536, "exact ring: a pass adds <= 256 rays");
 
 #ifndef MCSKIN_WF_SOFT_MIN_BLOCKS
 #define MCSKIN_WF_SOFT_MIN_BLOCKS 4
 #endif
 template <bool BATCH>
 __global__ void __launch_bounds__(kWfThreads, MCSKIN_WF_SOFT_MIN_BLOCKS)
-k_wf_softshadow(const DevFrame fr, const FramePointers fp_, const WaveView wv_, const BatchSlice* __restrict__ batch) {
+k_wf_softshadow(const DevFrame fr, const FramePointers fp_, const WaveView wv_, const ShadowVerdicts sv,
+                const BatchSlice* __restrict__ batch) {
     __shared__ __align__(8) uint64_t stageBar;
     const FramePointers& fp = BATCH ? batch[blockIdx.y].fp : fp_;
     const WaveView& wv = BATCH ? batch[blockIdx.y].wave : wv_;
@@ -235,9 +243,14 @@
     const V3 lightCentre = ld3(fr.light_pos);
     const uint32_t one = fr.spp > 0 ? 1u : 0u;
     unsigned int* chunkCounter = wv.qCount + 1;
+    unsigned int exactHead = 0u, exactTail = 0u;
     if (tid == 0) {
         sm->head = 0u;
         sm->tail = 0u;
+        sm->exactTail = 0u;
+        sm->verdicts[0] = sm->verdicts[1] = sm->verdicts[2] = 0u;
+        sm->eps = light_point_fast_err(fr);
+        sm->grow = sm->eps + shadow_verdict_delta(fr);
     }
     for (;;) {
         __syncthreads();
@@ -286,27 +299,71 @@
             for (int round = 0; round < rounds; ++round) {
                 const int ns = min(kShadowRound, N - round * kShadowRound);
                 if (mine) {
-                    const float4 eP = sm->pendP[(head + tid) & (kPendCap - 1)];
-                    const V3 P = mk3(eP.x, eP.y, eP.z);
+                    float* pt = sm->pts + tid * kPtStride;
                     FreshStream rng;
                     if (round == 0) {
+                        const float4 eP = sm->pendP[(head + tid) & (kPendCap - 1)];
                         rng.seed_memo(__float_as_uint(eP.w), one, wv.seedMemo);
+                        V3 t, b;
+                        light_frame(fr, mk3(eP.x, eP.y, eP.z), &t, &b);
+                        pt[kPtFrame] = t.x; pt[kPtFrame + 1] = t.y; pt[kPtFrame + 2] = t.z;
+                        pt[kPtFrame + 3] = b.x; pt[kPtFrame + 4] = b.y; pt[kPtFrame + 5] = b.z;
                     } else {
                         const uint4 e = sm->engine[tid];
                         rng.cur = e.x; rng.nxt = e.y; rng.far = e.z; rng.j = e.w;
                     }
-                    soft_shadow_positions(fr, P, ns, rng, sm->pts + tid * kPtStride);
+                    for (int k = 0; k < ns; ++k) {
+                        pt[2 * k] = rng.next();
+                        pt[2 * k + 1] = rng.next();
+                    }
                     if (round + 1 < rounds) sm->engine[tid] = make_uint4(rng.cur, rng.nxt, rng.far, rng.j);
                 }
                 __syncthreads();
                 const unsigned int nRays = cnt * static_cast<unsigned int>(ns);
-                for (unsigned int r = tid; r < nRays; r += kWfThreads) {
-                    const unsigned int e = ns == kShadowRound ? r >> 3 : r / static_cast<unsigned int>(ns);
-                    const unsigned int k = r - e * static_cast<unsigned int>(ns);
-                    const float4 eO = sm->pendO[(head + e) & (kPendCap - 1)];
-                    const float* pt = sm->pts + e * kPtStride + k * 3u;
-                    if (!in_shadow_from(sc, mk3(eO.x, eO.y, eO.z), mk3(pt[0], pt[1], pt[2]), __float_as_uint(eO.w)))
-                        atomicAdd(&sm->lit[e], 1u);
+                auto hit_of = [&](unsigned int r) { return ns == kShadowRound ? r >> 3 : r / static_cast<unsigned int>(ns); };
+                for (unsigned int r0 = 0; r0 < nRays; r0 += kWfThreads) {
+                    const unsigned int r = r0 + tid;
+                    bool toExact = false;
+                    if (r < nRays) {
+                        const unsigned int e = hit_of(r), k = r - e * static_cast<unsigned int>(ns);
+                        int verdict = kShadowUnknown;
+                        if (sv.fast) {
+                            const float4 eO = sm->pendO[(head + e) & (kPendCap - 1)];
+                            const float* pt = sm->pts + e * kPtStride;
+                            const V3 pa = light_point_fast(fr, mk3(pt[kPtFrame], pt[kPtFrame + 1], pt[kPtFrame + 2]),
+                                                           mk3(pt[kPtFrame + 3], pt[kPtFrame + 4], pt[kPtFrame + 5]),
+                                                           pt[2 * k], pt[2 * k + 1]);
+                            verdict = shadow_verdict(sc, mk3(eO.x, eO.y, eO.z), pa, __float_as_uint(eO.w), sm->eps, sm->grow);
+                        }
+                        if (verdict == kShadowLit) atomicAdd(&sm->lit[e], 1u);
+                        if (sv.counts) atomicAdd(&sm->verdicts[verdict], 1u);
+                        toExact = verdict == kShadowUnknown;
+                    }
+                    const unsigned int m = __ballot_sync(0xffffffffu, toExact);
+                    if (m) {
+                        unsigned int base = 0u;
+                        if (lane == 0) base = atomicAdd(&sm->exactTail, static_cast<unsigned int>(__popc(m)));
+                        base = __shfl_sync(0xffffffffu, base, 0);
+                        if (toExact) sm->exact[(base + __popc(m & ((1u << lane) - 1u))) & (kExactCap - 1)] = static_cast<unsigned short>(r);
+                    }
+                    exactTail += static_cast<unsigned int>(__syncthreads_count(toExact));
+                    const unsigned int flushAt = r0 + kWfThreads >= nRays ? 1u : static_cast<unsigned int>(kWfThreads);
+                    while (exactTail - exactHead >= flushAt) {
+                        const unsigned int take = min(exactTail - exactHead, static_cast<unsigned int>(kWfThreads));
+                        if (static_cast<unsigned int>(tid) < take) {
+                            const unsigned int x = sm->exact[(exactHead + tid) & (kExactCap - 1)];
+                            const unsigned int e = hit_of(x), k = x - e * static_cast<unsigned int>(ns);
+                            const float4 eO = sm->pendO[(head + e) & (kPendCap - 1)];
+                            const float* pt = sm->pts + e * kPtStride;
+                            const V3 p = light_point(fr, mk3(pt[kPtFrame], pt[kPtFrame + 1], pt[kPtFrame + 2]),
+                                                     mk3(pt[kPtFrame + 3], pt[kPtFrame + 4], pt[kPtFrame + 5]), pt[2 * k],
+                                                     pt[2 * k + 1]);
+                            if (!in_shadow_from(sc, mk3(eO.x, eO.y, eO.z), p, __float_as_uint(eO.w)))
+                                atomicAdd(&sm->lit[e], 1u);
+                        }
+                        exactHead += take;
+                        __syncthreads();
+                    }
                 }
                 __syncthreads();
             }
@@ -316,6 +373,11 @@
             __syncthreads();
         }
         if (last) break;
+    }
+    if (sv.counts && tid == 0) {
+        atomicAdd(&sv.counts[0], static_cast<unsigned long long>(sm->verdicts[kShadowLit]));
+        atomicAdd(&sv.counts[1], static_cast<unsigned long long>(sm->verdicts[kShadowBlocked]));
+        atomicAdd(&sv.counts[2], static_cast<unsigned long long>(sm->verdicts[kShadowUnknown]));
     }
 }
 
@@ -586,7 +648,8 @@
 
 void launch_wavefront(const DevFrame& fr, const FramePointers& fp, const BandView& band, const ActiveList& list,
                       const WaveView& wv, unsigned int* groupCounter, cudaStream_t stream, int* launches,
-                      const BatchSlice* batch, int nScenes, const AovView* aovView, const AovView* aovBatch) {
+                      const BatchSlice* batch, int nScenes, const AovView* aovView, const AovView* aovBatch,
+                      ShadowVerdicts verdicts) {
     int n = 0;
     const AovView av = aovView ? *aovView : AovView{};
     const int grid = wv.gridBlocks;
@@ -599,6 +662,7 @@
         else KERNEL<false><<<GRID, kWfThreads, SMEM, stream>>>(__VA_ARGS__, batch);                 \
         ++n;                                                                                        \
     } while (0)
+    verdicts.fast = verdicts.fast && fr.cull_valid && fr.n_boxes <= 32;
     if (wv.shadowMode == kShadowSoft) {
         static SmemOptIn optIn;
         static const void* const fns[] = {reinterpret_cast<const void*>(k_wf_softshadow<false>),
@@ -619,7 +683,7 @@
         if (wv.shadowMode == kShadowSoft) {
             const dim3 gs(std::max(1, std::min<int>(grid, wv.softGrid)), ny);
             const size_t smem = ((blob + 15u) & ~size_t(15)) + sizeof(ShadowSmem);
-            MCSKIN_WF_LAUNCH(k_wf_softshadow, gs, smem, fr, fp, wv);
+            MCSKIN_WF_LAUNCH(k_wf_softshadow, gs, smem, fr, fp, wv, verdicts);
         } else if (wv.shadowMode == kShadowHard) {
             MCSKIN_WF_LAUNCH(k_wf_hardshadow, g, blob, fr, fp, wv);
         }
diff --git a/minecraftskin_raytracer_b200/csrc/wavefront.cuh b/minecraftskin_raytracer_b200/csrc/wavefront.cuh
--- a/minecraftskin_raytracer_b200/csrc/wavefront.cuh
+++ b/minecraftskin_raytracer_b200/csrc/wavefront.cuh
@@ -54,6 +54,11 @@
 bool wavefront_carve(const DevFrame& fr, void* base, size_t bytes, unsigned int pathCapacity, unsigned int entryCapacity,
                      int gridBlocks, WaveView* out, AovView* aov = nullptr);
 
+struct ShadowVerdicts {
+    int fast = 1;
+    unsigned long long* counts = nullptr;
+};
+
 void launch_aov_defaults(const DevFrame& fr, const BandView& band, const McAovTargets& planes, const AovView* aovBatch, int nScenes,
                          cudaStream_t stream);
 
@@ -61,7 +66,7 @@
     void launch_wavefront(const DevFrame& fr, const FramePointers& fp, const BandView& band, const ActiveList& list,    \
                           const WaveView& wave, unsigned int* groupCounter, cudaStream_t stream, int* launches,         \
                           const BatchSlice* batch = nullptr, int nScenes = 1, const AovView* aov = nullptr,             \
-                          const AovView* aovBatch = nullptr);                                                          \
+                          const AovView* aovBatch = nullptr, ShadowVerdicts verdicts = ShadowVerdicts{});             \
     void launch_batch_reset(const BatchSlice* batch, int nScenes, cudaStream_t stream);                                 \
     bool launch_primary_batch(const DevFrame& fr, const BandView& band, uint32_t* tileStates, bool seedTiles,           \
                               const BatchSlice* batch, int nScenes, unsigned int blobBytes, int primaryTargetBlocks,    \
diff --git a/minecraftskin_raytracer_b200/lib.py b/minecraftskin_raytracer_b200/lib.py
--- a/minecraftskin_raytracer_b200/lib.py
+++ b/minecraftskin_raytracer_b200/lib.py
@@ -31,6 +31,7 @@
     "mcskin_cuda_host_register", "mcskin_cuda_host_unregister", "mcskin_cuda_render_batch_multi",
     "mcskin_cuda_enable_peer_access", "mcskin_cuda_context_render_scene_tiles",
     "mcskin_cuda_context_debug_block_times", "mcskin_cuda_context_render_skin_batch",
+    "mcskin_cuda_context_debug_shadow_verdicts", "mcskin_cuda_light_draw_errors",
     "mcskin_skin_layout", "mcskin_cuda_render_aovs", "mcskin_cuda_context_set_aov_targets",
 ]
 
@@ -392,6 +393,11 @@
             _check(min(_lib.mcskin_cuda_context_debug_block_times(self._h, _ptr(out, C.c_uint64), C.c_int32(n)), 0))
         return out
 
+    def debug_shadow_verdicts(self) -> dict:
+        out = np.zeros(3, dtype=np.uint64)
+        _check(_lib.mcskin_cuda_context_debug_shadow_verdicts(self._h, _ptr(out, C.c_uint64)))
+        return {"lit": int(out[0]), "shadowed": int(out[1]), "exact": int(out[2])}
+
     def sync(self) -> dict:
         stats = McRenderStats()
         _check(_lib.mcskin_cuda_context_sync(self._h, C.byref(stats)))
@@ -487,6 +493,12 @@
     _check(_lib.mcskin_cuda_sincos(C.c_int32(device), _ptr(a, C.c_float), C.c_int32(len(a)), _ptr(sn, C.c_float),
                                    _ptr(cs, C.c_float)))
     return sn, cs
+
+
+def light_draw_errors(device: int = 0) -> dict:
+    out = np.zeros(4, dtype=np.float32)
+    _check(_lib.mcskin_cuda_light_draw_errors(C.c_int32(device), _ptr(out, C.c_float)))
+    return {"sin": float(out[0]), "cos": float(out[1]), "sqrt": float(out[2]), "bound": float(out[3])}
 
 
 def powf(x, y, device: int = 0) -> np.ndarray:
```

After: 77120 (median of 6 runs). About the same (-0.1%).
